# dremovd/PPO

Measured on AMD Instinct MI355X. Metric: env-steps/sec (Pong-shaped synthetic, 256 envs/GPU), higher is better.
Workload: dtype f32

## Files before the change

include/ppo_amd.h:

```cpp
#ifndef PPO_AMD_H
#define PPO_AMD_H

#include <stddef.h>
#include <stdint.h>

#ifdef __cplusplus
extern "C" {
#endif

#define PPO_OK 0
#define PPO_E_INVALID (-1)
#define PPO_E_HIP (-2)
#define PPO_E_ALIGN (-3)

#define PPO_TERM_NONE 0
#define PPO_TERM_U8 1
#define PPO_TERM_F32 2

#define PPO_SCAN_AUTO 0
#define PPO_SCAN_COLUMNS 1
#define PPO_SCAN_TILES 2

int ppo_version(void);
const char *ppo_last_error(void);
// ... 33 lines not shown
size_t ppo_conv3x3_packed_floats(int cin, int cout, int transposed);
int ppo_conv3x3_pack_weights_f32(const ppo_pack_job *jobs , int n_jobs, void *stream);
int ppo_conv3x3_forward_packed_f32(const void *in, int in_mode, const float *packed, const float *bias,
                                   const float *residual, float *out, int n, int cin, int cout, int h, int w,
                                   void *stream);
int ppo_conv3x3_backward_data_packed_f32(const float *dy, const float *packed, const float *relu_src,
                                         const float *dres, float *dx, int n, int cin, int cout, int h, int w,
                                         void *stream);
int ppo_conv3x3_pool_forward_packed_f32(const void *in, int in_mode, const float *packed, const float *bias,
                                        float *out, uint8_t *argmax, int n, int cin, int cout, int h, int w,
                                        void *stream);
int ppo_conv3x3_pool_forward_packed_indexed_f32(const void *in, const int32_t *index, int in_mode, const float *packed,
                                                const float *bias, float *out, uint8_t *argmax, int n, int cin, int cout,
                                                int h, int w, void *stream);
int ppo_conv3x3_backward_weight_slabs_pooled_indexed_f32(const void *in, const int32_t *index, int in_mode, const float *g,
                                                         const uint8_t *argmax, void *workspace, size_t workspace_bytes,
                                                         int n, int cin, int cout, int h, int w, int *n_slabs, void *stream);
int ppo_conv1_pool_form(int form);

int ppo_conv3x3_block_supported(int channels, int h, int w);
int ppo_conv3x3_block_forward_packed_f32(const float *in, const float *packed0, const float *bias0, const float *packed1,
                                         const float *bias1, float *out, int n, int channels, int h, int w, void *stream);

size_t ppo_conv3x3_wgrad_workspace_bytes(int cin, int cout);
int ppo_conv3x3_backward_weight_f32(const void *in, int in_mode, const float *dy, float *dweight, float *dbias,
                                    void *workspace, size_t workspace_bytes, int n, int cin, int cout, int h,
                                    int w, int accumulate, void *stream);

typedef struct ppo_wgrad_job {
    const float *slabs;
    float *dweight;
    float *dbias;
    int n_slabs, cin, cout;
    int accumulate;
} ppo_wgrad_job;
int ppo_conv3x3_backward_weight_slabs_f32(const void *in, int in_mode, const float *dy, void *workspace,
                                          size_t workspace_bytes, int n, int cin, int cout, int h, int w,
                                          int *n_slabs, void *stream);
int ppo_conv3x3_backward_weight_slabs_batch_f32(const void *const *ins, int in_mode, const float *const *dys,
                                                void *const *workspaces, size_t workspace_bytes, int count, int n, int cin,
                                                int cout, int h, int w, int *n_slabs, void *stream);
int ppo_conv3x3_backward_weight_slabs_batch_mixed_f32(const void *const *ins, const int *relu, const float *const *dys,
                                                      void *const *workspaces, size_t workspace_bytes, int count, int n,
                                                      int cin, int cout, int h, int w, int *n_slabs, void *stream);
int ppo_conv3x3_backward_weight_bf16x3_supported(int cin, int cout, int h, int w);
int ppo_conv3x3_backward_weight_slabs_batch_bf16x3(const float *const *ins, const int *relu, const float *const *dys,
                                                   void *const *workspaces, size_t workspace_bytes, int count, int n, int cin,
                                                   int cout, int h, int w, int *n_slabs, void *stream);
int ppo_conv3x3_backward_weight_pooled_supported(int cin, int cout, int h, int w);
int ppo_conv3x3_backward_weight_slabs_pooled_f32(const void *in, int in_mode, const float *g, const uint8_t *argmax,
                                                 void *workspace, size_t workspace_bytes, int n, int cin, int cout, int h,
                                                 int w, int *n_slabs, void *stream);
int ppo_conv3x3_wgrad_reduce_f32(const ppo_wgrad_job *jobs, int n_jobs, void *stream);

int ppo_maxpool3x3s2_forward_f32(const float *in, float *out, uint8_t *argmax, int n, int c, int h, int w,
                                 void *stream);
int ppo_maxpool3x3s2_backward_f32(const float *dout, const uint8_t *argmax, float *din, int n, int c, int h, int w,
                                  void *stream);

int ppo_conv2d_strided_supported(int cin, int cout, int kh, int kw, int stride, int h, int w);
int ppo_conv2d_strided_forward_f32(const void *in, int in_mode, const float *weight, const float *bias, float *out,
                                   int relu_out, int n, int cin, int h, int w, int cout, int kh, int kw, int stride,
                                   void *stream);
int ppo_conv2d_strided_backward_data_f32(const float *dy, const float *gate, const float *weight, float *dx, int n,
                                         int cin, int h, int w, int cout, int kh, int kw, int stride, void *stream);
size_t ppo_conv2d_strided_wgrad_workspace_bytes(int n, int cin, int h, int w, int cout, int kh, int kw, int stride);
int ppo_conv2d_strided_backward_weight_f32(const void *in, int in_mode, const float *dy, const float *gate, float *dweight,
                                           float *dbias, void *workspace, size_t workspace_bytes, int n, int cin, int h,
                                           int w, int cout, int kh, int kw, int stride, void *stream);

size_t ppo_gemm_workspace_bytes(int M, int N, int K);
int ppo_gemm_f32(const float *A, int64_t a_sm, int64_t a_sk, int relu_a, const float *B, int64_t b_sk, int64_t b_sn,
                 int relu_b, const float *bias, const float *mask, float *C, int64_t ldc, int M, int N, int K,
                 void *workspace, size_t workspace_bytes, void *stream);

int ppo_dense_heads_forward_f32(const float *x, int relu_x, const float *W, const float *b, const float *Wh, const float *bh,
                                int relu_h, float *h, float *heads, int M, int K, int H, int NH, void *workspace,
                                size_t workspace_bytes, void *stream);

int ppo_dense_heads_act_forward_f32(const float *x, int relu_x, const float *W, const float *b, const float *Wh,
                                    const float *bh, int relu_h, float *h, float *heads, int M, int K, int H, int NH,
                                    void *workspace, size_t workspace_bytes, int n_actions, float temperature,
                                    uint64_t seed, uint64_t offset, float *log_policy, int32_t *actions, float *log_pac,
                                    float *raw_policy, float *values, int n_value_heads, void *stream);
int ppo_dense_heads_loss_forward_f32(const float *x, int relu_x, const float *W, const float *b, const float *Wh, const float *bh,
                                     int relu_h, float *h, float *heads, int M, int K, int H, int NH, void *workspace,
                                     size_t workspace_bytes, int n_actions, int n_value_heads, const int32_t *actions,
                                     const float *old_log_pac, const float *old_log_policy, const float *advantages,
                                     const float *returns, float eps_clip, float ent_coef, float vf_coef, float grad_scale,
                                     float *dheads, float *stats, const int32_t *index, void *stream);

int ppo_heads_backward_f32(const float *dheads, const float *hin, int relu_in, const float *gate, const float *Wh, float *dh,
                           float *dWh, float *dbh, float *db_next, int B, int H, int NH, void *stream);
int ppo_colsum_f32(const float *X, int M, int N, int64_t ldx, float *out, int accumulate, void *stream);

int ppo_policy_act_f32(const float *heads, int B, int ldo, int n_actions, float temperature, const float *uniform,
                       uint64_t seed, uint64_t offset, int greedy, float *log_policy, int32_t *actions,
                       float *log_pac, float *raw_policy, float *values, int n_value_heads, void *stream);

int ppo_ppo_loss_f32(const float *heads, int B, int ldo, int n_actions, int n_value_heads, const int32_t *actions,
                     const float *old_log_pac, const float *old_log_policy, const float *advantages,
                     const float *returns, float eps_clip, float ent_coef, float vf_coef, float grad_scale,
                     float *dheads, float *stats, const int32_t *index, void *stream);

int ppo_tanh_forward_f32(const float *x, float *y, size_t n, void *stream);
int ppo_tanh_backward_f32(const float *dy, const float *y, float *dx, size_t n, void *stream);

int ppo_value_loss_f32(const float *heads, int B, int ldo, int value_col, int n_value_heads, const float *returns,
                       float vf_coef, int tvf_col, int n_tvf, int tvf_stride, const float *tvf_returns,
                       const float *tvf_weights, float tvf_coef, float grad_scale, float *dheads, float *stats,
                       const int32_t *index, float tvf_keep_prob, uint64_t seed, uint64_t offset, void *stream);

int ppo_distil_loss_f32(const float *heads, int B, int ldo, int n_actions, int pred_col, int n_pred, int pred_stride,
                        int vector_targets, const float *targets, const float *weights, const float *old_policy,
                        const float *log_std, float beta, float grad_scale, float *dheads, float *stats,
                        const int32_t *index, void *stream);

int ppo_gaussian_act_f32(const float *heads, int B, int ldo, int n_actions, const float *log_std, const float *normal,
                         uint64_t seed, uint64_t offset, int deterministic, float *actions, float *log_pac,
                         float *raw_policy, float *values, int n_value_heads, void *stream);

int ppo_gaussian_loss_f32(const float *heads, int B, int ldo, int n_actions, int n_value_heads, const float *actions,
                          const float *old_log_pac, const float *advantages, const float *returns,
                          const float *log_std, float eps_clip, float vf_coef, float grad_scale, float *dheads,
                          float *dlog_std_rows, float *stats, const int32_t *index, void *stream);

size_t ppo_adam_workspace_bytes(void);
// ... 161 lines not shown
```

ppo_amd/_lib.py:

```python
import ctypes
import os
import threading

HERE = os.path.dirname(os.path.abspath(__file__))
LIB_PATH = os.environ.get("PPO_AMD_LIB") or os.path.join(HERE, "lib", "libppo_amd.so")

PPO_TERM_NONE, PPO_TERM_U8, PPO_TERM_F32 = 0, 1, 2
PPO_SCAN_AUTO, PPO_SCAN_COLUMNS, PPO_SCAN_TILES = 0, 1, 2
PPO_IN_NONE, PPO_IN_RELU, PPO_IN_U8 = 0, 1, 2

_vp = ctypes.c_void_p
_i = ctypes.c_int
_i64 = ctypes.c_int64
_d = ctypes.c_double
_f = ctypes.c_float
_sz = ctypes.c_size_t
_u64 = ctypes.c_uint64

SIGNATURES = {
    "ppo_version": (_i, []),
    "ppo_last_error": (ctypes.c_char_p, []),
    "ppo_gae_scan_f32": (_i, [_vp, _vp, _vp, _vp, _i, _vp, _vp, _i, _i, _i64, _d, _d, _d, _i, _vp]),
    "ppo_bootstrapped_returns_f32": (_i, [_vp, _vp, _i, _vp, _vp, _d, _vp, _i, _i, _i64, _vp]),
    "ppo_conv3x3_forward_f32": (_i, [_vp, _i, _vp, _vp, _vp, _vp, _i, _i, _i, _i, _i, _vp]),
    "ppo_conv3x3_backward_data_f32": (_i, [_vp, _vp, _vp, _vp, _vp, _i, _i, _i, _i, _i, _vp]),
    "ppo_conv3x3_wgrad_workspace_bytes": (_sz, [_i, _i]),
    "ppo_conv3x3_backward_weight_f32": (_i, [_vp, _i, _vp, _vp, _vp, _vp, _sz, _i, _i, _i, _i, _i, _i, _vp]),
    "ppo_maxpool3x3s2_forward_f32": (_i, [_vp, _vp, _vp, _i, _i, _i, _i, _vp]),
    "ppo_maxpool3x3s2_backward_f32": (_i, [_vp, _vp, _vp, _i, _i, _i, _i, _vp]),
    "ppo_gemm_workspace_bytes": (_sz, [_i, _i, _i]),
    "ppo_gemm_f32": (_i, [_vp, _i64, _i64, _i, _vp, _i64, _i64, _i, _vp, _vp, _vp, _i64, _i, _i, _i, _vp, _sz, _vp]),
    "ppo_colsum_f32": (_i, [_vp, _i, _i, _i64, _vp, _i, _vp]),
    "ppo_heads_backward_f32": (_i, [_vp, _vp, _i, _vp, _vp, _vp, _vp, _vp, _vp, _i, _i, _i, _vp]),
    "ppo_dense_heads_forward_f32": (_i, [_vp, _i, _vp, _vp, _vp, _vp, _i, _vp, _vp, _i, _i, _i, _i, _vp, _sz, _vp]),
    "ppo_dense_heads_act_forward_f32": (_i, [_vp, _i, _vp, _vp, _vp, _vp, _i, _vp, _vp, _i, _i, _i, _i, _vp, _sz, _i, _f, _u64,
                                             _u64, _vp, _vp, _vp, _vp, _vp, _i, _vp]),
    "ppo_dense_heads_loss_forward_f32": (_i, [_vp, _i, _vp, _vp, _vp, _vp, _i, _vp, _vp, _i, _i, _i, _i, _vp, _sz, _i, _i, _vp, _vp, _vp,
                                              _vp, _vp, _f, _f, _f, _f, _vp, _vp, _vp, _vp]),
    "ppo_policy_act_f32": (_i, [_vp, _i, _i, _i, _f, _vp, _u64, _u64, _i, _vp, _vp, _vp, _vp, _vp, _i, _vp]),
    "ppo_gather_rows": (_i, [_vp, _i64, _i64, _vp, _i, _vp, _vp]),
    "ppo_moments_workspace_bytes": (_sz, []),
    "ppo_moments_f64": (_i, [_vp, _i64, _vp, _vp, _vp]),
    "ppo_normalize_f32": (_i, [_vp, _i64, _vp, _f, _vp, _vp, _vp]),
    "ppo_accumulate_f32": (_i, [_vp, _vp, _i64, _vp]),
    "ppo_mask_mul_f32": (_i, [_vp, _vp, _i64, _vp]),
    "ppo_tvf_returns_workspace_bytes": (_sz, [_i, _i, _i, _i, _i]),
    "ppo_tvf_returns_f32": (_i, [_vp, _vp, _vp, _i, _i, _i, _i, _i, _d, _vp, _vp, _vp, _i, _i, _vp, _vp, _vp, _vp, _vp,
                                 _vp, _sz, _vp, _vp]),
    "ppo_synth_env_create": (_vp, [_i, _i64, _u64, _d, _i64, _i]),
    "ppo_synth_env_destroy": (None, [_vp]),
    "ppo_synth_env_reset": (_i, [_vp, _vp]),
    "ppo_synth_env_step": (_i, [_vp, _vp, _vp, _vp, _vp, _vp, _vp, _vp]),
    "ppo_synth_env_step_upload": (_i, [_vp, _vp, _vp, _vp, _vp, _vp, _vp, _vp, _vp, _i, _vp]),
    "ppo_synth_env_get_state": (_i, [_vp, _vp, _vp, _vp]),
    "ppo_synth_env_set_state": (_i, [_vp, _vp, _vp, _vp, _vp]),
    "ppo_ppo_loss_f32": (_i, [_vp, _i, _i, _i, _i, _vp, _vp, _vp, _vp, _vp, _f, _f, _f, _f, _vp, _vp, _vp, _vp]),
    "ppo_conv3x3_pool_forward_f32": (_i, [_vp, _i, _vp, _vp, _vp, _vp, _i, _i, _i, _i, _i, _vp]),
    "ppo_conv3x3_packed_floats": (_sz, [_i, _i, _i]),
    "ppo_conv3x3_pack_weights_f32": (_i, [_vp, _i, _vp]),
    "ppo_conv3x3_forward_packed_f32": (_i, [_vp, _i, _vp, _vp, _vp, _vp, _i, _i, _i, _i, _i, _vp]),
    "ppo_conv3x3_backward_data_packed_f32": (_i, [_vp, _vp, _vp, _vp, _vp, _i, _i, _i, _i, _i, _vp]),
    "ppo_conv3x3_pool_forward_packed_f32": (_i, [_vp, _i, _vp, _vp, _vp, _vp, _i, _i, _i, _i, _i, _vp]),
    "ppo_conv3x3_pool_forward_packed_indexed_f32": (_i, [_vp, _vp, _i, _vp, _vp, _vp, _vp, _i, _i, _i, _i, _i, _vp]),
    "ppo_conv1_pool_form": (_i, [_i]),
    "ppo_conv3x3_block_supported": (_i, [_i, _i, _i]),
    "ppo_conv3x3_block_forward_packed_f32": (_i, [_vp, _vp, _vp, _vp, _vp, _vp, _i, _i, _i, _i, _vp]),
    "ppo_conv3x3_backward_weight_slabs_f32": (_i, [_vp, _i, _vp, _vp, _sz, _i, _i, _i, _i, _i, _vp, _vp]),
    "ppo_conv3x3_backward_weight_pooled_supported": (_i, [_i, _i, _i, _i]),
    "ppo_conv3x3_backward_weight_slabs_pooled_f32": (_i, [_vp, _i, _vp, _vp, _vp, _sz, _i, _i, _i, _i, _i, _vp, _vp]),
    "ppo_conv3x3_backward_weight_slabs_pooled_indexed_f32": (_i, [_vp, _vp, _i, _vp, _vp, _vp, _sz, _i, _i, _i, _i, _i, _vp, _vp]),
    "ppo_conv3x3_backward_weight_slabs_batch_f32": (_i, [_vp, _i, _vp, _vp, _sz, _i, _i, _i, _i, _i, _i, _vp, _vp]),
    "ppo_conv3x3_backward_weight_slabs_batch_mixed_f32": (_i, [_vp, _vp, _vp, _vp, _sz, _i, _i, _i, _i, _i, _i, _vp, _vp]),
    "ppo_conv3x3_backward_weight_bf16x3_supported": (_i, [_i, _i, _i, _i]),
    "ppo_conv3x3_backward_weight_slabs_batch_bf16x3": (_i, [_vp, _vp, _vp, _vp, _sz, _i, _i, _i, _i, _i, _i, _vp, _vp]),
    "ppo_conv3x3_wgrad_reduce_f32": (_i, [_vp, _i, _vp]),
    "ppo_tanh_forward_f32": (_i, [_vp, _vp, _sz, _vp]),
    "ppo_tanh_backward_f32": (_i, [_vp, _vp, _vp, _sz, _vp]),
    "ppo_value_loss_f32": (_i, [_vp, _i, _i, _i, _i, _vp, _f, _i, _i, _i, _vp, _vp, _f, _f, _vp, _vp, _vp, _f, _u64, _u64, _vp]),
    "ppo_distil_loss_f32": (_i, [_vp, _i, _i, _i, _i, _i, _i, _i, _vp, _vp, _vp, _vp, _f, _f, _vp, _vp, _vp, _vp]),
    "ppo_gaussian_act_f32": (_i, [_vp, _i, _i, _i, _vp, _vp, _u64, _u64, _i, _vp, _vp, _vp, _vp, _i, _vp]),
    "ppo_gaussian_loss_f32": (_i, [_vp, _i, _i, _i, _i, _vp, _vp, _vp, _vp, _vp, _f, _f, _f, _vp, _vp, _vp, _vp, _vp]),
    "ppo_impala_stack_tail_supported": (_i, [_i, _i, _i]),
    "ppo_impala_stack_tail_forward_f32": (_i, [_vp, _vp, _vp, _vp, _vp, _vp, _vp, _i, _i, _i, _i, _vp]),
    "ppo_impala_stack_full_supported": (_i, [_i, _i, _i]),
    "ppo_impala_stack_full_backward_f32": (_i, [_vp] * 10 + [_i, _i, _i, _i, _vp]),
    "ppo_impala_stack_chain_forward_f32": (_i, [_vp] * 15 + [_i, _i, _i, _i, _vp]),
    "ppo_impala_stack_chain_split_workspace_bytes": (_sz, [_i, _i, _i, _i]),
    "ppo_impala_stack_chain_split_forward_f32": (_i, [_vp, _vp, _vp, _vp, _vp, _vp, _vp, _sz, _i, _i, _i, _i, _vp]),
    "ppo_impala_stack_full_forward_f32": (_i, [_vp, _vp, _vp, _vp, _vp, _vp, _vp, _vp, _vp, _i, _i, _i, _i, _vp]),
    "ppo_impala_stack_tail_backward_f32": (_i, [_vp, _vp, _vp, _vp, _vp, _vp, _vp, _i, _i, _i, _i, _vp]),
    "ppo_obs_moments_f64": (_i, [_vp, _i, _i, _i, _vp, _vp]),
    "ppo_obs_rms_update_f64": (_i, [_vp, _d, _d, _vp, _vp, _vp, _vp, _i, _vp]),
    "ppo_obs_normalize_f32": (_i, [_vp, _i, _vp, _vp, _f, _vp, _i, _i, _vp]),
    "ppo_adam_workspace_bytes": (_sz, []),
    "ppo_adam_step_f32": (_i, [_vp, _vp, _vp, _vp, _i64, _i64, _d, _d, _d, _d, _f, _f, _vp, _vp, _vp]),
    "ppo_adam_step_presummed_f32": (_i, [_vp, _vp, _vp, _vp, _i64, _i64, _d, _d, _d, _d, _f, _f, _vp, _i, _vp, _vp]),
    "ppo_impala_stack_tail_bf16x3_packed_bytes": (_sz, []),
    "ppo_impala_stack_tail_bf16x3_supported": (_i, [_i, _i, _i]),
    "ppo_impala_stack_tail_pack_bf16x3": (_i, [_vp, _vp, _i, _i, _vp]),
    "ppo_impala_stack_tail_pack_bf16x3_jobs": (_i, [_vp, _i, _vp]),
    "ppo_impala_stack_tail_forward_bf16x3": (_i, [_vp, _vp, _vp, _vp, _vp, _vp, _vp, _i, _i, _i, _i, _vp]),
    "ppo_impala_stack_tail_backward_bf16x3": (_i, [_vp, _vp, _vp, _vp, _vp, _vp, _vp, _i, _i, _i, _i, _vp]),
    "ppo_impala_stack_tail_bf16x3_sign_bytes": (_sz, [_i, _i, _i, _i]),
    "ppo_impala_stack_tail_forward_signs_bf16x3": (_i, [_vp, _vp, _vp, _vp, _vp, _vp, _vp, _vp, _i, _i, _i, _i, _vp]),
    "ppo_impala_stack_tail_backward_signs_bf16x3": (_i, [_vp, _vp, _vp, _vp, _vp, _vp, _vp, _i, _i, _i, _i, _vp]),
    "ppo_conv3x3_bf16x3_supported": (_i, [_i, _i, _i, _i]),
    "ppo_conv3x3_bf16x3_packed_bytes": (_sz, [_i, _i]),
    "ppo_conv3x3_pack_bf16x3_jobs": (_i, [_vp, _i, _vp]),
    "ppo_conv3x3_bf16x3": (_i, [_vp, _i, _vp, _vp, _vp, _i, _i, _i, _i, _i, _vp]),
    "ppo_conv3x3_pool_bf16x3_supported": (_i, [_i, _i, _i, _i]),
    "ppo_conv3x3_backward_weight_slabs_batch_bf16_split": (_i, [_vp, _vp, _vp, _vp, _sz, _i, _i, _i, _i, _i, _i, _i, _vp, _vp]),
    "ppo_conv3x3_bf16_split_packed_bytes": (_sz, [_i, _i, _i]),
    "ppo_conv3x3_pack_bf16_split": (_i, [_vp, _vp, _i, _i, _i, _i, _vp]),
    "ppo_conv3x3_bf16_split": (_i, [_vp, _i, _vp, _vp, _vp, _i, _i, _i, _i, _i, _i, _vp]),
    "ppo_conv3x3_pool_bf16x3": (_i, [_vp, _i, _vp, _vp, _vp, _vp, _i, _i, _i, _i, _i, _vp]),
    "ppo_mlp_supported": (_i, [_i, _i, _i]),
    "ppo_mlp_forward_f32": (_i, [_vp, _vp, _vp, _i, _vp, _vp, _vp, _vp]),
    "ppo_mlp_train_workspace_floats": (_sz, [_i, _i, _i, _i]),
    "ppo_mlp_train_f32": (_i, [_vp, _vp, _vp, _vp, _i64, _i, _vp, _vp, _vp, _vp, _i, _i, _vp, _vp, _vp]),
    "ppo_conv2d_strided_supported": (_i, [_i, _i, _i, _i, _i, _i, _i]),
    "ppo_conv2d_strided_forward_f32": (_i, [_vp, _i, _vp, _vp, _vp, _i, _i, _i, _i, _i, _i, _i, _i, _i, _vp]),
    "ppo_conv2d_strided_backward_data_f32": (_i, [_vp, _vp, _vp, _vp, _i, _i, _i, _i, _i, _i, _i, _i, _vp]),
    "ppo_conv2d_strided_wgrad_workspace_bytes": (_sz, [_i, _i, _i, _i, _i, _i, _i, _i]),
    "ppo_conv2d_strided_backward_weight_f32": (_i, [_vp, _i, _vp, _vp, _vp, _vp, _vp, _sz, _i, _i, _i, _i, _i, _i, _i, _i, _vp]),
    "ppo_adam_step_scatter_f32": (_i, [_vp, _vp, _vp, _vp, _i64, _i64, _d, _d, _d, _d, _f, _f, _vp, _vp, _vp, _i64, _vp, _vp]),
}

class PackJob(ctypes.Structure):
# ... 99 lines not shown
```

ppo_amd/csrc/conv3x3_wgrad.hip:

```cpp
#include "common.h"
#include "conv_stage.h"
#include "mfma.h"

namespace ppo {
namespace {

constexpr int pad_mod32(int v, int target) { return v + ((target - v % 32) + 32) % 32; }

#ifndef PPO_STAMP
#define PPO_STAMP(var)
#define PPO_STAMP_ADD(slot, t1, t0)
#endif
#ifndef PPO_TUNE_WGRAD_NBUF
#define PPO_TUNE_WGRAD_NBUF 2
#endif
#ifndef PPO_TUNE_WGRAD_PERCU
#define PPO_TUNE_WGRAD_PERCU 2
#endif
#ifndef PPO_TUNE_WGRAD_NBUF_ONEBAND
#define PPO_TUNE_WGRAD_NBUF_ONEBAND 1
#endif
template <int IN_MODE, int NBANDS>
constexpr int wgrad_nbuf()
{
    return IN_MODE == IN_U8 ? 1 : (NBANDS == 1 ? PPO_TUNE_WGRAD_NBUF_ONEBAND : PPO_TUNE_WGRAD_NBUF);
}
template <int IN_MODE, bool DY_POOLED>
constexpr bool wgrad_run() { return true; }
constexpr int kWgradWaves = 8;
#ifndef PPO_TUNE_WGRAD_DMA_WAVE
#define PPO_TUNE_WGRAD_DMA_WAVE 4
#endif
template <int IN_MODE, int NBANDS, bool DY_POOLED>
constexpr bool wgrad_dma_wave()
{
    return PPO_TUNE_WGRAD_DMA_WAVE && wgrad_nbuf<IN_MODE, NBANDS>() == 2 && IN_MODE != IN_U8 && !DY_POOLED;
}
constexpr int kWgradDmaWaves = PPO_TUNE_WGRAD_DMA_WAVE;
template <int IN_MODE, int NBANDS, bool DY_POOLED>
constexpr int wgrad_threads() { return (kWgradWaves + (wgrad_dma_wave<IN_MODE, NBANDS, DY_POOLED>() ? kWgradDmaWaves : 0)) * 64; }

template <int CIN, int COUT, int H, int W, int TR, int NBUF_, bool RUN_>
struct WgradCfg {
    static constexpr int CINP = (CIN + 3) / 4 * 4;
    static constexpr int MTC = COUT / 16;
    static constexpr bool BIAS_IN_TILE = (9 * CINP) % 16 != 0;
    static constexpr int NJ = 9 * CINP + (BIAS_IN_TILE ? 1 : 0);
    static constexpr int NTT = (NJ + 15) / 16;
    static constexpr int JP = ((9 * CINP + 1) + 15) / 16 * 16;
    static constexpr int WT = (NTT <= 4 || NTT == 9) ? 1 : ((NTT <= 12 || NTT == 18) ? 2 : 4);
    static constexpr int KG = kWgradWaves / WT;
    static constexpr int NTW_MAX = (NTT + WT - 1) / WT;
    static constexpr int REM = NTT % WT == 0 ? WT : NTT % WT;
    static constexpr int WIDTH = W;
// ... 265 lines not shown
    for (int src = 1; src < C::KG; ++src) {
        float *img = s_red;
        if (kg == src) {
            if (db_lane) {
#pragma unroll
                for (int m = 0; m < C::MTC; ++m) img[(m * 16 + l15) * C::JP + 9 * C::CINP] = asum[m];
            }
#pragma unroll
            for (int m = 0; m < C::MTC; ++m)
#pragma unroll
                for (int t = 0; t < C::NTW_MAX; ++t)
                    if (wt + C::WT * t < C::NTT)
#pragma unroll
                        for (int r = 0; r < 4; ++r)
                            img[(m * 16 + g * 4 + r) * C::JP + (wt + C::WT * t) * 16 + l15] = acc[m][t][r];
        }
        __syncthreads();
        if (kg == 0) {
#pragma unroll
            for (int m = 0; m < C::MTC; ++m)
#pragma unroll
                for (int t = 0; t < C::NTW_MAX; ++t)
                    if (wt + C::WT * t < C::NTT)
#pragma unroll
                        for (int r = 0; r < 4; ++r)
                            acc[m][t][r] += img[(m * 16 + g * 4 + r) * C::JP + (wt + C::WT * t) * 16 + l15];
            if (db_lane) {
#pragma unroll
                for (int m = 0; m < C::MTC; ++m) asum[m] += img[(m * 16 + l15) * C::JP + 9 * C::CINP];
            }
        }
        if (src + 1 < C::KG) __syncthreads();
    }
    if (kg == 0) {
        float *slab = partial + (size_t)blockIdx.x * COUT * C::JP;
#pragma unroll
        for (int m = 0; m < C::MTC; ++m)
#pragma unroll
            for (int t = 0; t < C::NTW_MAX; ++t)
                if (wt + C::WT * t < C::NTT)
#pragma unroll
                    for (int r = 0; r < 4; ++r)
                        slab[(m * 16 + g * 4 + r) * C::JP + (wt + C::WT * t) * 16 + l15] = acc[m][t][r];
        if (db_lane) {
#pragma unroll
            for (int m = 0; m < C::MTC; ++m) slab[(m * 16 + l15) * C::JP + 9 * C::CINP] = asum[m];
        }
    }
    PPO_STAMP(t_k3)
    PPO_STAMP_ADD(7, t_k3, t_k2)
    PPO_STAMP_ADD(3, t_k3, t_k0)
}

__device__ __forceinline__ float4 slab_partition_sum(const float *slabs, int byte_off, int byte_stride, int lo, int hi, bool live)
{
    const __amdgpu_buffer_rsrc_t buf = buffer_of(slabs);
    float4 s0 = make_float4(0.f, 0.f, 0.f, 0.f), s1 = s0;
    for (int q = lo; q < hi; q += 16) {
        float4 v[16];
#pragma unroll
        for (int u = 0; u < 16; ++u) v[u] = buffer_f32x4(buf, (live && q + u < hi) ? byte_off + (q + u) * byte_stride : kOutside);
#pragma unroll
        for (int u = 0; u < 16; u += 2) {
            s0.x += v[u].x; s0.y += v[u].y; s0.z += v[u].z; s0.w += v[u].w;
            s1.x += v[u + 1].x; s1.y += v[u + 1].y; s1.z += v[u + 1].z; s1.w += v[u + 1].w;
        }
    }
    return make_float4(s0.x + s1.x, s0.y + s1.y, s0.z + s1.z, s0.w + s1.w);
}

__global__ __launch_bounds__(256) void conv3x3_wgrad_reduce_kernel(const float *__restrict__ partial, int n_slabs,
                                                                   int cout, int cin, int cinp, int jp,
                                                                   float *__restrict__ dw, float *__restrict__ db,
                                                                   int accumulate)
{
    __shared__ float4 s[256];
    const int q4 = jp / 4;
    const int idx = blockIdx.x * 16 + (threadIdx.x & 15);
    const int part = threadIdx.x >> 4;
    const bool live = idx < cout * q4;
    const int co = live ? idx / q4 : 0;
    const int j0 = live ? (idx % q4) * 4 : 0;
    const size_t stride = (size_t)cout * jp;
    const int per = (n_slabs + 15) / 16;
    const int lo = part * per;
    const int hi = lo + per < n_slabs ? lo + per : n_slabs;
    s[threadIdx.x] = slab_partition_sum(partial, (co * jp + j0) * 4, (int)stride * 4, lo, hi, live);
    __syncthreads();
    if (part == 0 && live) {
        float sum[4] = {0.f, 0.f, 0.f, 0.f};
#pragma unroll
        for (int q = 0; q < 16; ++q) {
            const float4 a = s[q * 16 + threadIdx.x];
            sum[0] += a.x;
            sum[1] += a.y;
            sum[2] += a.z;
            sum[3] += a.w;
        }
#pragma unroll
        for (int e = 0; e < 4; ++e) {
            const int j = j0 + e;
            if (j == 9 * cinp) {
                if (db) db[co] = accumulate ? db[co] + sum[e] : sum[e];
            } else if (j < 9 * cinp) {
                const int tap = j / cinp;
                const int ci = j % cinp;
                if (ci < cin) {
                    float *dst = dw + ((size_t)co * cin + ci) * 9 + tap;
                    *dst = accumulate ? *dst + sum[e] : sum[e];
                }
            }
        }
    }
}

#ifndef PPO_TUNE_WGRAD_MAXSLABS
#define PPO_TUNE_WGRAD_MAXSLABS 512
#endif
constexpr int kWgradMaxSlabs = PPO_TUNE_WGRAD_MAXSLABS;

constexpr int kMaxJobs = 32;
struct ReduceJobs {
    ppo_wgrad_job j[kMaxJobs];
};

__global__ __launch_bounds__(256) void conv3x3_wgrad_reduce_jobs_kernel(ReduceJobs jobs)
{
    __shared__ float4 s[256];
    const ppo_wgrad_job &job = jobs.j[blockIdx.y];
    const int cout = job.cout, cin = job.cin, n_slabs = job.n_slabs, accumulate = job.accumulate;
    const int cinp = (cin + 3) / 4 * 4;
    const int jp = ((9 * cinp + 1) + 15) / 16 * 16;
    const int q4 = jp / 4;
    if ((int)blockIdx.x * 16 >= cout * q4) return;
    const int idx = blockIdx.x * 16 + (threadIdx.x & 15);
    const int part = threadIdx.x >> 4;
    const bool live = idx < cout * q4;
    const int co = live ? idx / q4 : 0;
    const int j0 = live ? (idx % q4) * 4 : 0;
    const size_t stride = (size_t)cout * jp;
    const int per = (n_slabs + 15) / 16;
    const int lo = part * per;
    const int hi = lo + per < n_slabs ? lo + per : n_slabs;
    s[threadIdx.x] = slab_partition_sum(job.slabs, (co * jp + j0) * 4, (int)stride * 4, lo, hi, live);
    __syncthreads();
    if (part == 0 && live) {
        float sum[4] = {0.f, 0.f, 0.f, 0.f};
#pragma unroll
        for (int q = 0; q < 16; ++q) {
            const float4 a = s[q * 16 + threadIdx.x];
            sum[0] += a.x;
            sum[1] += a.y;
            sum[2] += a.z;
            sum[3] += a.w;
        }
#pragma unroll
        for (int e = 0; e < 4; ++e) {
            const int j = j0 + e;
            if (j == 9 * cinp) {
                if (job.dbias) job.dbias[co] = accumulate ? job.dbias[co] + sum[e] : sum[e];
            } else if (j < 9 * cinp) {
                const int tap = j / cinp;
                const int ci = j % cinp;
                if (ci < cin) {
                    float *d = job.dweight + ((size_t)co * cin + ci) * 9 + tap;
                    *d = accumulate ? *d + sum[e] : sum[e];
                }
            }
        }
    }
}

template <int CIN, int COUT, int H, int W, int TR, int IN_MODE, bool DY_POOLED = false>
int launch_wgrad(const void *in, const float *dy, float *dw, float *db, float *workspace, size_t workspace_bytes,
                 int n_images, int accumulate, hipStream_t st, int *n_slabs_out = nullptr,
                 const WgradBatch *more = nullptr, int count = 1, const uint8_t *argmax = nullptr)
{
    using C = WgradCfg<CIN, COUT, H, W, TR, wgrad_nbuf<IN_MODE, (H + TR - 1) / TR>(), wgrad_run<IN_MODE, DY_POOLED>()>;
    auto kern = conv3x3_wgrad_kernel<CIN, COUT, H, W, TR, IN_MODE, DY_POOLED>;
    static bool attr_set = false;
    if (!attr_set) {
        hipError_t e = hipFuncSetAttribute(reinterpret_cast<const void *>(kern),
                                           hipFuncAttributeMaxDynamicSharedMemorySize, (int)C::LDS_BYTES);
        if (e != hipSuccess) return fail(PPO_E_HIP, "conv3x3_wgrad: hipFuncSetAttribute: %s", hipGetErrorString(e));
        attr_set = true;
    }
    const int n_items = n_images * C::NBANDS;
    int per_cu = (int)((160 * 1024) / C::LDS_BYTES);
    per_cu = per_cu < 1 ? 1 : (per_cu > PPO_TUNE_WGRAD_PERCU ? PPO_TUNE_WGRAD_PERCU : per_cu);
#ifndef PPO_TUNE_WGRAD_BIGSLABS
    if ((size_t)COUT * C::JP * sizeof(float) > 16 * 1024) per_cu = 1;
#endif
    int grid = (256 * per_cu) / count;
    if (grid < 1) grid = 1;
    if (grid > kWgradMaxSlabs) grid = kWgradMaxSlabs;
    if (grid > n_items) grid = n_items;
    const size_t need = (size_t)grid * COUT * C::JP * sizeof(float);
    if (need > workspace_bytes)
        return fail(PPO_E_INVALID, "conv3x3_wgrad: workspace too small (%zu < %zu bytes)", workspace_bytes, need);
    WgradBatch batch{};
    if (more) {
        batch = *more;
    } else {
        batch.in[0] = in;
        batch.dy[0] = dy;
        batch.partial[0] = workspace;
    }
    batch.argmax = argmax;
    batch.in_index = IN_MODE == IN_U8 ? t_wgrad_in_index : nullptr;
    hipLaunchKernelGGL(kern, dim3(grid, count), dim3(wgrad_threads<IN_MODE, C::NBANDS, DY_POOLED>()), C::LDS_BYTES, st, batch,
                       n_images);
    int rc = check_launch("conv3x3_wgrad_kernel");
    if (rc) return rc;
    if (n_slabs_out) {
        *n_slabs_out = grid;
        return PPO_OK;
    }
    const int total = COUT * (C::JP / 4);
    hipLaunchKernelGGL(conv3x3_wgrad_reduce_kernel, dim3((total + 15) / 16), dim3(256), 0, st, workspace, grid, COUT,
                       CIN, C::CINP, C::JP, dw, db, accumulate);
    return check_launch("conv3x3_wgrad_reduce_kernel");
}

// ... 201 lines not shown
```

ppo_amd/csrc/gemm.hip:

```cpp
#include <algorithm>

#include "common.h"
#include "loss_rows.h"
#include "policy_act.h"
#include "mfma.h"

namespace ppo {
namespace {

#ifndef PPO_TUNE_GEMM_BK
#define PPO_TUNE_GEMM_BK 32
#endif
constexpr int BM = 64, BN = 64, BK = PPO_TUNE_GEMM_BK;
constexpr int PITCH_M = 80, PITCH_K = BK + 2;
constexpr int TILE_WORDS = BM * PITCH_K > BK * PITCH_M ? BM * PITCH_K : BK * PITCH_M;

struct GemmArgs {
    const float *A;
    const float *B;
    float *C;
    const float *bias;
    const float *mask;
    int M, N, K;
    int64_t a_sm, a_sk, b_sk, b_sn, ldc;
    int relu_a, relu_b;
    int k_per_slice;
    int split;
    int vec_a, vec_b;
    int vec_c;
};

#ifndef PPO_TUNE_GEMM_WAVES
#define PPO_TUNE_GEMM_WAVES 8
#endif
constexpr int kGemmWaves = PPO_TUNE_GEMM_WAVES, kGemmThreads = kGemmWaves * 64;
static_assert(kGemmWaves == 4 || kGemmWaves == 8, "2 x 2 waves of 32 x 32 or 2 x 4 waves of 32 x 16");
constexpr int kWaveN = kGemmWaves == 8 ? 16 : 32, kNJ = kWaveN / 16;
constexpr int kSlabF4 = BM * BK / 4 / kGemmThreads;
struct Slab {
    float4 v[kSlabF4];
};

__device__ __forceinline__ __amdgpu_buffer_rsrc_t operand_rsrc(const float *P) { return buffer_of(P); }

template <bool kfast, bool vec>
__device__ __forceinline__ void slab_load(Slab &s, __amdgpu_buffer_rsrc_t P, int st, int sk, int t0, int rows, int k0,
                                          int kend, int tid)
{
#pragma unroll
    for (int e = 0; e < kSlabF4; ++e) {
        const int q = tid + e * kGemmThreads;
        int tt, kk;
        if (kfast) {
            kk = (q % (BK / 4)) * 4;
            tt = q / (BK / 4);
// ... 46 lines not shown
};
__device__ __forceinline__ TileId tile_of(int id, int gm, int gn, int split)
{
    const int xcd = id % kXcds, slot = id / kXcds;
    TileId t;
    if (split > 1) {
        const int per = (split + kXcds - 1) / kXcds;
        t.z = xcd * per + slot % per;
        const int tile = slot / per;
        t.tn = tile % gn;
        t.tm = tile / gn;
        t.live = t.z < split && t.tm < gm;
    } else if (gn >= gm) {
        t.z = 0;
        t.tm = slot % gm;
        t.tn = xcd + kXcds * (slot / gm);
        t.live = t.tn < gn;
    } else {
        t.z = 0;
        t.tn = slot % gn;
        t.tm = xcd + kXcds * (slot / gn);
        t.live = t.tm < gm;
    }
    return t;
}
inline int tile_grid(int gm, int gn, int split)
{
    if (split > 1) return kXcds * ((split + kXcds - 1) / kXcds) * gm * gn;
    const int lo = gn >= gm ? gm : gn, hi = gn >= gm ? gn : gm;
    return kXcds * ((hi + kXcds - 1) / kXcds) * lo;
}

#ifndef PPO_TUNE_GEMM_DEPTH
#define PPO_TUNE_GEMM_DEPTH 4
#endif
constexpr int DEPTH = PPO_TUNE_GEMM_DEPTH;

#ifdef PPO_TUNE_GEMM_STAMPS
__device__ unsigned long long ppo_gemm_stamps[1024 * 8];
#define PPO_GSTAMP(slot)                                                                          \
    do {                                                                                          \
        unsigned long long t_;                                                                    \
        __builtin_amdgcn_sched_barrier(0);                                                        \
        asm volatile("s_memtime %0\n\ts_waitcnt lgkmcnt(0)" : "=s"(t_)::"memory");               \
        __builtin_amdgcn_sched_barrier(0);                                                        \
        if (threadIdx.x == 0 && blockIdx.x < 1024) ppo_gemm_stamps[blockIdx.x * 8 + (slot)] = t_; \
    } while (0)
#else
#define PPO_GSTAMP(slot)
#endif
static_assert(DEPTH % 2 == 0, "the LDS buffer of a slab is its slot's parity");

template <bool a_kfast, bool b_kfast, bool vec>
__global__ __launch_bounds__(kGemmThreads) void gemm_f32_kernel(GemmArgs p, int gm, int gn)
{
    __shared__ __align__(16) float s_a[2][TILE_WORDS];
    __shared__ __align__(16) float s_b[2][TILE_WORDS];
    const TileId t = tile_of(blockIdx.x, gm, gn, p.split);
    if (!t.live) return;
    const int tid = threadIdx.x;
    const int lane = tid & 63;
    const int wave = tid >> 6;
    const int l15 = lane & 15;
    const int g = lane >> 4;
    const int wm = (wave / (BN / kWaveN)) * 32;
    const int wn = (wave % (BN / kWaveN)) * kWaveN;
    const int m0 = t.tm * BM;
    const int n0 = t.tn * BN;
    const int kbeg = t.z * p.k_per_slice;
    const int kend = min(p.K, kbeg + p.k_per_slice);

    f32x4 acc[2][kNJ];
#pragma unroll
    for (int i = 0; i < 2; ++i)
#pragma unroll
        for (int j = 0; j < kNJ; ++j) acc[i][j] = f32x4{0.f, 0.f, 0.f, 0.f};

    const int nslabs = kbeg < kend ? (kend - kbeg + BK - 1) / BK : 0;
    const int ngroups = (nslabs + DEPTH - 1) / DEPTH;
    const __amdgpu_buffer_rsrc_t bufA = operand_rsrc(p.A), bufB = operand_rsrc(p.B);
    Slab ra[DEPTH], rb[DEPTH];

    auto fetch = [&](int d, int slab) {
        slab_load<a_kfast, vec>(ra[d], bufA, (int)p.a_sm, (int)p.a_sk, m0, p.M, kbeg + slab * BK, kend, tid);
        slab_load<b_kfast, vec>(rb[d], bufB, (int)p.b_sn, (int)p.b_sk, n0, p.N, kbeg + slab * BK, kend, tid);
    };
    auto stage = [&](int d) {
        slab_store(ra[d], s_a[d & 1], a_kfast, p.relu_a, tid);
        slab_store(rb[d], s_b[d & 1], b_kfast, p.relu_b, tid);
        __syncthreads();
    };
    auto multiply = [&](int d) {
        const float *sa = s_a[d & 1], *sb = s_b[d & 1];
        float a[BK / 4][2], b[BK / 4][kNJ];
#pragma unroll
        for (int ks = 0; ks < BK / 4; ++ks) {
#pragma unroll
            for (int i = 0; i < 2; ++i)
                a[ks][i] = a_kfast ? sa[(wm + i * 16 + l15) * PITCH_K + ks * 4 + g]
                                   : sa[(ks * 4 + g) * PITCH_M + wm + i * 16 + l15];
#pragma unroll
            for (int j = 0; j < kNJ; ++j)
                b[ks][j] = b_kfast ? sb[(wn + j * 16 + l15) * PITCH_K + ks * 4 + g]
                                   : sb[(ks * 4 + g) * PITCH_M + wn + j * 16 + l15];
        }
        __builtin_amdgcn_sched_barrier(0);
#pragma unroll
        for (int ks = 0; ks < BK / 4; ++ks)
#pragma unroll
            for (int i = 0; i < 2; ++i)
#pragma unroll
// ... 40 lines not shown
            for (int q = 0; q < kPasses; ++q) {
                const int m = m0 + row0 + kRowsPerPass * q;
                const int off = (m < p.M && col_in) ? (m * (int)p.ldc + n0 + col) * 4 : kOutside;
                gate[q] = buffer_f32x4(bufM, off);
            }
        }
        if (finish && p.bias && col_in) bias4 = *reinterpret_cast<const float4 *>(p.bias + n0 + col);
        __syncthreads();
#pragma unroll
        for (int i = 0; i < 2; ++i)
#pragma unroll
            for (int j = 0; j < kNJ; ++j)
#pragma unroll
                for (int r = 0; r < 4; ++r)
                    sc[(wm + i * 16 + g * 4 + r) * PITCH_C + wn + j * 16 + l15] = acc[i][j][r];
        __syncthreads();
#pragma unroll
        for (int q = 0; q < kPasses; ++q) {
            const int row = row0 + kRowsPerPass * q, m = m0 + row;
            float4 v = *reinterpret_cast<const float4 *>(sc + row * PITCH_C + col);
            if (finish) {
                v.x += bias4.x, v.y += bias4.y, v.z += bias4.z, v.w += bias4.w;
                if (p.mask) {
                    v.x = gate[q].x > 0.f ? v.x : 0.f;
                    v.y = gate[q].y > 0.f ? v.y : 0.f;
                    v.z = gate[q].z > 0.f ? v.z : 0.f;
                    v.w = gate[q].w > 0.f ? v.w : 0.f;
                }
            }
            if (m < p.M && col_in) *reinterpret_cast<float4 *>(C + m * ldc + n0 + col) = v;
        }
    } else {
#pragma unroll
        for (int i = 0; i < 2; ++i)
#pragma unroll
            for (int j = 0; j < kNJ; ++j)
#pragma unroll
                for (int r = 0; r < 4; ++r) {
                    const int m = m0 + wm + i * 16 + g * 4 + r;
                    const int n = n0 + wn + j * 16 + l15;
                    if (m < p.M && n < p.N) {
                        float v = acc[i][j][r];
                        if (finish) {
                            if (p.bias) v += p.bias[n];
                            if (p.mask) v = p.mask[m * p.ldc + n] > 0.f ? v : 0.f;
                        }
                        C[m * ldc + n] = v;
                    }
                }
    }
    PPO_GSTAMP(4);
}

__global__ __launch_bounds__(256) void gemm_finalize_kernel(const float *__restrict__ partial, int split, int M, int N,
                                                            const float *__restrict__ bias,
                                                            const float *__restrict__ mask, float *__restrict__ C,
                                                            int64_t ldc)
{
    const int idx = blockIdx.x * blockDim.x + threadIdx.x;
    if (idx >= M * N) return;
    const int m = idx / N, n = idx % N;
    float v = 0.f;
    const size_t stride = (size_t)M * N;
    int s = 0;
    for (; s + 8 <= split; s += 8) {
        float t[8];
#pragma unroll
        for (int u = 0; u < 8; ++u) t[u] = partial[(size_t)(s + u) * stride + idx];
#pragma unroll
        for (int u = 0; u < 8; ++u) v += t[u];
    }
    for (; s < split; ++s) v += partial[(size_t)s * stride + idx];
    if (bias) v += bias[n];
    if (mask) v = mask[m * ldc + n] > 0.f ? v : 0.f;
    C[m * ldc + n] = v;
}

constexpr int kRowsMaxN = 32, kRowsMaxKPerLane = 8;

template <int NB, int KPL>
__global__ __launch_bounds__(256) void gemm_rows_kernel(GemmArgs p)
{
    const int lane = threadIdx.x & 63;
    const int m = blockIdx.x * 4 + __builtin_amdgcn_readfirstlane(threadIdx.x >> 6);
    if (m >= p.M) return;
    const __amdgpu_buffer_rsrc_t bufA = operand_rsrc(p.A), bufB = operand_rsrc(p.B);
    bool kin[KPL];
#pragma unroll
    for (int i = 0; i < KPL; ++i) kin[i] = lane + 64 * i < p.K;
    float av[KPL];
#pragma unroll
    for (int i = 0; i < KPL; ++i) {
        const int off = kin[i] ? (m * (int)p.a_sm + lane + 64 * i) * 4 : kOutside;
        av[i] = buffer_f32(bufA, off);
    }
    for (int n0 = 0; n0 < p.N; n0 += NB) {
        float bv[NB][KPL];
#pragma unroll
        for (int j = 0; j < NB; ++j) {
            const int row = min(n0 + j, p.N - 1) * (int)p.b_sn;
#pragma unroll
            for (int i = 0; i < KPL; ++i) {
                const int off = kin[i] ? (row + lane + 64 * i) * 4 : kOutside;
                bv[j][i] = buffer_f32(bufB, off);
            }
        }
// ... 25 lines not shown
}

__global__ __launch_bounds__(256) void gemm_small_kernel(GemmArgs p)
{
    __shared__ float s[256];
    const int o = blockIdx.x * 16 + (threadIdx.x & 15);
    const int part = threadIdx.x >> 4;
    const bool live = o < p.M * p.N;
    const int m = live ? o / p.N : 0, n = live ? o - m * p.N : 0;
    const float *a = p.A + m * p.a_sm;
    const float *b = p.B + n * p.b_sn;
    const int per = (p.K + 15) / 16;
    const int k0 = part * per, k1 = min(p.K, k0 + per);
    float acc = 0.f;
    if (live) {
        int k = k0;
        for (; k + 8 <= k1; k += 8) {
            float av[8], bv[8];
#pragma unroll
            for (int u = 0; u < 8; ++u) {
                av[u] = a[(k + u) * p.a_sk];
                bv[u] = b[(k + u) * p.b_sk];
            }
#pragma unroll
            for (int u = 0; u < 8; ++u) {
                if (p.relu_a) av[u] = fmaxf(av[u], 0.f);
                if (p.relu_b) bv[u] = fmaxf(bv[u], 0.f);
                acc = fmaf(av[u], bv[u], acc);
            }
        }
        for (; k < k1; ++k) {
            float a0 = a[k * p.a_sk], b0 = b[k * p.b_sk];
            if (p.relu_a) a0 = fmaxf(a0, 0.f);
            if (p.relu_b) b0 = fmaxf(b0, 0.f);
            acc = fmaf(a0, b0, acc);
        }
    }
    s[threadIdx.x] = acc;
    __syncthreads();
    if (part == 0 && live) {
        float v = 0.f;
#pragma unroll
        for (int q = 0; q < 16; ++q) v += s[q * 16 + threadIdx.x];
        if (p.bias) v += p.bias[n];
        if (p.mask) v = p.mask[m * p.ldc + n] > 0.f ? v : 0.f;
        p.C[m * p.ldc + n] = v;
    }
}

__global__ __launch_bounds__(256) void colsum_kernel(const float *__restrict__ X, int M, int N, int64_t ldx,
                                                     float *__restrict__ out, int accumulate)
{
    __shared__ float s[256];
    const int n = blockIdx.x * 16 + (threadIdx.x & 15);
    const int part = threadIdx.x >> 4;
    float v = 0.f;
    if (n < N) {
        for (int m = part; m < M; m += 16 * 8) {
            float t[8];
#pragma unroll
            for (int u = 0; u < 8; ++u) {
                const int mm = m + 16 * u;
                t[u] = mm < M ? X[mm * ldx + n] : 0.f;
            }
#pragma unroll
            for (int u = 0; u < 8; ++u) v += t[u];
        }
    }
    s[threadIdx.x] = v;
    __syncthreads();
    if (part == 0 && n < N) {
        float t = 0.f;
#pragma unroll
        for (int q = 0; q < 16; ++q) t += s[q * 16 + threadIdx.x];
        out[n] = accumulate ? out[n] + t : t;
    }
}

struct ActTail {
    float temperature;
    uint64_t seed, offset;
    ActOut out;
    int loss;
    PpoLossP lp;
    float *dheads;
    const int32_t *index;
};

template <int KPL, int NA, int NHT>
__global__ __launch_bounds__(256) void finalize_heads_kernel(const float *__restrict__ partial, int split, int M, int H,
                                                            const float *__restrict__ bias, float *__restrict__ h,
                                                            const float *__restrict__ Wh, const float *__restrict__ bh, int NH,
                                                            int relu_h, float *__restrict__ heads, ActTail act)
{
    const int lane = threadIdx.x & 63;
    const int m = blockIdx.x * 4 + __builtin_amdgcn_readfirstlane(threadIdx.x >> 6);
    if (m >= M) return;
    const __amdgpu_buffer_rsrc_t pb = buffer_of(partial), wb = buffer_of(Wh), bb = buffer_of(bias, bias != nullptr);
    const int stride = M * H;
    int off[KPL];
#pragma unroll
    for (int i = 0; i < KPL; ++i) off[i] = lane + 64 * i < H ? m * H + lane + 64 * i : -1;
    float bv[NHT][KPL];
#pragma unroll
    for (int j = 0; j < NHT; ++j) {
        const int row = min(j, NH - 1) * H;
#pragma unroll
        for (int i = 0; i < KPL; ++i) bv[j][i] = buffer_f32(wb, off[i] < 0 ? kOutside : (row + lane + 64 * i) * 4);
    }
    float hv[KPL];
#pragma unroll
    for (int i = 0; i < KPL; ++i) hv[i] = 0.f;
    float bsv[KPL];
#pragma unroll
    for (int i = 0; i < KPL; ++i) bsv[i] = buffer_f32(bb, off[i] < 0 ? kOutside : (lane + 64 * i) * 4);
    int s = 0;
    for (; s + 16 <= split; s += 16) {
        float t[KPL][16];
#pragma unroll
        for (int i = 0; i < KPL; ++i)
#pragma unroll
            for (int u = 0; u < 16; ++u) t[i][u] = buffer_f32(pb, off[i] < 0 ? kOutside : ((s + u) * stride + off[i]) * 4);
#pragma unroll
        for (int i = 0; i < KPL; ++i)
#pragma unroll
            for (int u = 0; u < 16; ++u) hv[i] += t[i][u];
    }
    for (; s + 8 <= split; s += 8) {
        float t[KPL][8];
// ... 124 lines not shown
    }
#pragma unroll
    for (int j = 0; j < 16; ++j) s_red[j][tid] = dW[j];
    s_red[16][tid] = dbn;
    s_red[17][tid] = dbj;
    __syncthreads();
    if (part == 0) {
        float tot[18];
#pragma unroll
        for (int v = 0; v < 18; ++v) {
            float t = 0.f;
#pragma unroll
            for (int q = 0; q < 16; ++q) t += s_red[v][q * 16 + kk];
            tot[v] = t;
        }
        if (col) {
#pragma unroll
            for (int j = 0; j < 16; ++j)
                if (j < a.NH) a.dWh[j * a.H + k] = tot[j];
            if (a.db_next) a.db_next[k] = tot[16];
        }
        if ((int)blockIdx.x == a.xb && a.dbh && kk < a.NH) a.dbh[kk] = tot[17];
    }
}

inline bool vec_ok(const float *P, int64_t s_tile, int64_t s_k, int tile_extent, int k_extent)
{
    const int64_t other = s_k == 1 ? s_tile : s_k;
    const int extent = s_k == 1 ? k_extent : tile_extent;
    return (s_k == 1 || s_tile == 1) && other % 4 == 0 && extent % 4 == 0 && aligned(P, 16);
}

}
}

extern "C" size_t ppo_gemm_workspace_bytes(int M, int N, int K)
{
    (void)K;
    return (size_t)32 * M * N * sizeof(float);
}

namespace ppo {
namespace {
struct HeadsTail {
    const float *Wh, *bh;
    float *heads;
    int NH, relu_h;
    bool fused;
    const ActTail *act = nullptr;
    int act_n = 0;
    bool act_fused = false;
};

int gemm_dispatch(const float *A, int64_t a_sm, int64_t a_sk, int relu_a, const float *B, int64_t b_sk, int64_t b_sn,
                  int relu_b, const float *bias, const float *mask, float *C, int64_t ldc, int M, int N, int K,
                  void *workspace, size_t workspace_bytes, void *stream, HeadsTail *tail)
{
    if (M < 0 || N < 0 || K < 0) return fail(PPO_E_INVALID, "ppo_gemm_f32: negative dimension");
    if (M == 0 || N == 0) return PPO_OK;
    if (!A || !B || !C) return fail(PPO_E_INVALID, "ppo_gemm_f32: null pointer");
    if (ldc < N) return fail(PPO_E_INVALID, "ppo_gemm_f32: ldc < N");
    const int64_t a_last = (int64_t)(M - 1) * a_sm + (int64_t)(K - 1) * a_sk, b_last = (int64_t)(N - 1) * b_sn + (int64_t)(K - 1) * b_sk;
    if (K > 0 && (a_last * 4 + 16 > (int64_t)kBufferBytes || b_last * 4 + 16 > (int64_t)kBufferBytes || a_sm < 0 || a_sk < 0 ||
                  b_sn < 0 || b_sk < 0))
        return fail(PPO_E_INVALID, "ppo_gemm_f32: operand spans 2 GiB or more (or a negative stride); split the batch");
    hipStream_t st = as_stream(stream);
    if ((N <= 16 || K <= 16 || (M <= 16 && a_sm == 1)) && (int64_t)M * N <= (1 << 22)) {
        GemmArgs q{A, B, C, bias, mask, M, N, K, a_sm, a_sk, b_sk, b_sn, ldc, relu_a, relu_b, K, 1, 0, 0, 0};
        if (N <= kRowsMaxN && a_sk == 1 && b_sk == 1 && K <= 64 * kRowsMaxKPerLane) {
            if (K <= 256 && N <= 16)
                hipLaunchKernelGGL((gemm_rows_kernel<16, 4>), dim3((M + 3) / 4), dim3(256), 0, st, q);
            else if (K <= 256)
                hipLaunchKernelGGL((gemm_rows_kernel<8, 4>), dim3((M + 3) / 4), dim3(256), 0, st, q);
            else
                hipLaunchKernelGGL((gemm_rows_kernel<4, kRowsMaxKPerLane>), dim3((M + 3) / 4), dim3(256), 0, st, q);
            return check_launch("gemm_rows_kernel");
        }
        hipLaunchKernelGGL(gemm_small_kernel, dim3((M * N + 15) / 16), dim3(256), 0, st, q);
        return check_launch("gemm_small_kernel");
    }
    const int gm = (M + BM - 1) / BM, gn = (N + BN - 1) / BN;
    constexpr int kSliceK = 256;
    int split = 1;
    const bool few = gn * 4 <= 32;
    if (few && K >= 2 * kSliceK) split = std::min(32, (K + kSliceK - 1) / kSliceK);
    if (split > 1 && (!workspace || workspace_bytes < (size_t)split * M * N * sizeof(float))) split = 1;
    int kps = (K + split - 1) / split;
    kps = (kps + BK - 1) / BK * BK;
    if (split > 1) split = (K + kps - 1) / kps;
    GemmArgs p{A, B, split > 1 ? static_cast<float *>(workspace) : C, bias, mask, M, N, K, a_sm, a_sk, b_sk, b_sn,
               ldc, relu_a, relu_b, kps, split, vec_ok(A, a_sm, a_sk, M, K) ? 1 : 0, vec_ok(B, b_sn, b_sk, N, K) ? 1 : 0, 0};
    p.vec_c = N % 4 == 0 && ldc % 4 == 0 && aligned(C, 16) && aligned(p.C, 16) && (!bias || aligned(bias, 16)) &&
              (!mask || (aligned(mask, 16) && (int64_t)M * ldc * 4 < (int64_t)kBufferBytes));
    const dim3 grid(tile_grid(gm, gn, split));
    const bool vec = p.vec_a && p.vec_b;
    const int variant = (a_sk == 1 ? 4 : 0) | (b_sk == 1 ? 2 : 0) | (vec ? 1 : 0);
#define PPO_GEMM_CASE(v, ak, bk, vc)                                                                  \
    case v:                                                                                           \
        hipLaunchKernelGGL((gemm_f32_kernel<ak, bk, vc>), grid, dim3(kGemmThreads), 0, st, p, gm, gn); \
        break;
    switch (variant) {
        PPO_GEMM_CASE(0, false, false, false)
        PPO_GEMM_CASE(1, false, false, true)
        PPO_GEMM_CASE(2, false, true, false)
        PPO_GEMM_CASE(3, false, true, true)
        PPO_GEMM_CASE(4, true, false, false)
        PPO_GEMM_CASE(5, true, false, true)
        PPO_GEMM_CASE(6, true, true, false)
        PPO_GEMM_CASE(7, true, true, true)
    }
#undef PPO_GEMM_CASE
    int rc = check_launch("gemm_f32_kernel");
    if (rc) return rc;
    if (split > 1) {
        if (tail && !mask && ldc == N && N <= 256 && tail->NH <= 32 && (int64_t)split * M * N * 4 < (int64_t)kBufferBytes) {
#define PPO_FINALIZE(NA, NHT, ACT)                                                                                     \
    hipLaunchKernelGGL((finalize_heads_kernel<4, NA, NHT>), dim3((M + 3) / 4), dim3(256), 0, st,                       \
                       static_cast<const float *>(workspace), split, M, N, bias, C, tail->Wh, tail->bh, tail->NH,      \
                       tail->relu_h, tail->heads, ACT)
            tail->act_fused = tail->act != nullptr;
            const bool wide = tail->NH > 16;
#define PPO_FIN2(NA, ACT)                       \
    do {                                        \
        if (wide) PPO_FINALIZE(NA, 32, ACT);    \
        else PPO_FINALIZE(NA, 16, ACT);         \
    } while (0)
            switch (tail->act ? tail->act_n : 0) {
                case 4: PPO_FIN2(4, *tail->act); break;
                case 6: PPO_FIN2(6, *tail->act); break;
                case 15: PPO_FIN2(15, *tail->act); break;
                case 18: PPO_FIN2(18, *tail->act); break;
                default: PPO_FIN2(0, ActTail{}); tail->act_fused = false;
            }
#undef PPO_FIN2
#undef PPO_FINALIZE
            tail->fused = true;
            return check_launch("finalize_heads_kernel");
        }
        hipLaunchKernelGGL(gemm_finalize_kernel, dim3((M * N + 255) / 256), dim3(256), 0, st,
                           static_cast<const float *>(workspace), split, M, N, bias, mask, C, ldc);
        rc = check_launch("gemm_finalize_kernel");
    }
    return rc;
}
}
}

extern "C" int ppo_gemm_f32(const float *A, int64_t a_sm, int64_t a_sk, int relu_a, const float *B, int64_t b_sk,
                            int64_t b_sn, int relu_b, const float *bias, const float *mask, float *C, int64_t ldc,
                            int M, int N, int K, void *workspace, size_t workspace_bytes, void *stream)
{
    return ppo::gemm_dispatch(A, a_sm, a_sk, relu_a, B, b_sk, b_sn, relu_b, bias, mask, C, ldc, M, N, K, workspace,
                              workspace_bytes, stream, nullptr);
}

extern "C" int ppo_dense_heads_forward_f32(const float *x, int relu_x, const float *W, const float *b, const float *Wh,
                                           const float *bh, int relu_h, float *h, float *heads, int M, int K, int H, int NH,
                                           void *workspace, size_t workspace_bytes, void *stream)
{
    using namespace ppo;
    if (M < 0 || K < 0 || H <= 0 || NH <= 0) return fail(PPO_E_INVALID, "ppo_dense_heads_forward_f32: bad dimension");
    if (M == 0) return PPO_OK;
    if (!x || !W || !Wh || !h || !heads) return fail(PPO_E_INVALID, "ppo_dense_heads_forward_f32: null pointer");
    HeadsTail tail{Wh, bh, heads, NH, relu_h, false};
    int rc = gemm_dispatch(x, K, 1, relu_x, W, 1, K, 0, b, nullptr, h, H, M, H, K, workspace, workspace_bytes, stream, &tail);
    if (rc || tail.fused) return rc;
    return gemm_dispatch(h, H, 1, relu_h, Wh, 1, H, 0, bh, nullptr, heads, NH, M, NH, H, nullptr, 0, stream, nullptr);
}

extern "C" int ppo_policy_act_f32(const float *heads, int B, int ldo, int n_actions, float temperature, const float *uniform,
                                  uint64_t seed, uint64_t offset, int greedy, float *log_policy, int32_t *actions,
                                  float *log_pac, float *raw_policy, float *values, int n_value_heads, void *stream);

extern "C" int ppo_dense_heads_act_forward_f32(const float *x, int relu_x, const float *W, const float *b, const float *Wh,
                                               const float *bh, int relu_h, float *h, float *heads, int M, int K, int H,
                                               int NH, void *workspace, size_t workspace_bytes, int n_actions,
                                               float temperature, uint64_t seed, uint64_t offset, float *log_policy,
                                               int32_t *actions, float *log_pac, float *raw_policy, float *values,
                                               int n_value_heads, void *stream)
{
    using namespace ppo;
    if (M < 0 || K < 0 || H <= 0 || NH <= 0) return fail(PPO_E_INVALID, "ppo_dense_heads_act_forward_f32: bad dimension");
    if (n_actions <= 0 || n_actions > kMaxActions || n_value_heads < 0 || NH < n_actions + n_value_heads)
        return fail(PPO_E_INVALID, "ppo_dense_heads_act_forward_f32: bad head layout (n_actions=%d value heads=%d of %d)",
                    n_actions, n_value_heads, NH);
    if (!(temperature > 0.f)) return fail(PPO_E_INVALID, "ppo_dense_heads_act_forward_f32: temperature must be > 0");
    if (M == 0) return PPO_OK;
    if (!x || !W || !Wh || !h || !heads) return fail(PPO_E_INVALID, "ppo_dense_heads_act_forward_f32: null pointer");
    const ActTail act{temperature, seed, offset, ActOut{log_policy, actions, log_pac, raw_policy, values, n_value_heads}, 0,
                      PpoLossP{}, nullptr, nullptr};
    HeadsTail tail{Wh, bh, heads, NH, relu_h, false};
    tail.act = &act;
    tail.act_n = n_actions;
    int rc = gemm_dispatch(x, K, 1, relu_x, W, 1, K, 0, b, nullptr, h, H, M, H, K, workspace, workspace_bytes, stream, &tail);
    if (rc) return rc;
    if (!tail.fused)
        rc = gemm_dispatch(h, H, 1, relu_h, Wh, 1, H, 0, bh, nullptr, heads, NH, M, NH, H, nullptr, 0, stream, nullptr);
    if (rc || tail.act_fused) return rc;
    return ppo_policy_act_f32(heads, M, NH, n_actions, temperature, nullptr, seed, offset, 0, log_policy, actions, log_pac,
                              raw_policy, values, n_value_heads, stream);
}

extern "C" int ppo_ppo_loss_f32(const float *heads, int B, int ldo, int n_actions, int n_value_heads, const int32_t *actions,
                                const float *old_log_pac, const float *old_log_policy, const float *advantages,
                                const float *returns, float eps_clip, float ent_coef, float vf_coef, float grad_scale,
                                float *dheads, float *stats, const int32_t *index, void *stream);
// ... 54 lines not shown
```

ppo_amd/csrc/optim.hip:

```cpp
#include "common.h"

namespace ppo {
namespace {

constexpr int kPartials = 256;
__device__ __forceinline__ bool aligned16(const void *p) { return (reinterpret_cast<uintptr_t>(p) & 15) == 0; }

__global__ __launch_bounds__(256) void grad_sumsq_kernel(const float *__restrict__ g, int64_t n, float *__restrict__ partials)
{
    __shared__ float s[256];
    const int64_t chunk = (n + gridDim.x - 1) / gridDim.x;
    const int64_t lo = (int64_t)blockIdx.x * chunk;
    const int64_t hi = lo + chunk < n ? lo + chunk : n;
    float acc = 0.f;
    int64_t i = lo + threadIdx.x;
    for (; i + 768 < hi; i += 1024) {
        const float x0 = g[i], x1 = g[i + 256], x2 = g[i + 512], x3 = g[i + 768];
        acc += x0 * x0;
        acc += x1 * x1;
        acc += x2 * x2;
        acc += x3 * x3;
    }
    for (; i < hi; i += 256) {
        const float x = g[i];
        acc += x * x;
    }
    s[threadIdx.x] = acc;
    __syncthreads();
    for (int w = 128; w > 0; w >>= 1) {
        if (threadIdx.x < w) s[threadIdx.x] += s[threadIdx.x + w];
        __syncthreads();
    }
    if (threadIdx.x == 0) partials[blockIdx.x] = s[0];
}

__global__ __launch_bounds__(256) void adam_kernel(float *__restrict__ w, const float *__restrict__ g,
                                                   float *__restrict__ m, float *__restrict__ v, int64_t n,
                                                   const float *__restrict__ partials, int n_partials, float lr,
                                                   float one_minus_beta1, float beta2, float one_minus_beta2,
                                                   float eps, float bias_c1,
                                                   float bias_c2_sqrt, float max_norm, float grad_div,
                                                   float *__restrict__ norm_out, const int32_t *__restrict__ scatter,
                                                   int64_t n_scatter, float *__restrict__ packed)
{
    __shared__ float s_clip;
    __shared__ float s_part[256];
    s_part[threadIdx.x] = (int)threadIdx.x < n_partials ? partials[threadIdx.x] : 0.f;
    __syncthreads();
    for (int w = 128; w > 0; w >>= 1) {
        if ((int)threadIdx.x < w) s_part[threadIdx.x] += s_part[threadIdx.x + w];
        __syncthreads();
    }
    if (threadIdx.x == 0) {
        const float tot = s_part[0];
        const float norm = sqrtf(tot) / grad_div;
        float clip = 1.f;
        if (max_norm > 0.f) {
            clip = max_norm / (norm + 1e-6f);
            clip = clip > 1.f ? 1.f : clip;
        }
        s_clip = clip / grad_div;
        if (norm_out && blockIdx.x == 0) *norm_out = norm;
    }
    __syncthreads();
    const float gscale = s_clip;
    const float step_size = lr / bias_c1;
    auto update = [&](float &wi, float gi, float &mi, float &vi) {
        gi *= gscale;
        mi = mi + (gi - mi) * one_minus_beta1;
        vi = vi * beta2 + one_minus_beta2 * gi * gi;
        const float denom = sqrtf(vi) / bias_c2_sqrt + eps;
        wi = wi - step_size * (mi / denom);
    };
    const bool vec = (n % 4 == 0) && aligned16(w) && aligned16(g) && aligned16(m) && aligned16(v);
    if (vec) {
        const int64_t n4 = n / 4;
        float4 *w4 = reinterpret_cast<float4 *>(w), *m4 = reinterpret_cast<float4 *>(m), *v4 = reinterpret_cast<float4 *>(v);
        const float4 *g4 = reinterpret_cast<const float4 *>(g);
        for (int64_t i = (int64_t)blockIdx.x * blockDim.x + threadIdx.x; i < n4; i += (int64_t)gridDim.x * blockDim.x) {
            float4 ww = w4[i], gg = g4[i], mm = m4[i], vv = v4[i];
            update(ww.x, gg.x, mm.x, vv.x);
            update(ww.y, gg.y, mm.y, vv.y);
            update(ww.z, gg.z, mm.z, vv.z);
            update(ww.w, gg.w, mm.w, vv.w);
            w4[i] = ww;
            m4[i] = mm;
// ... 38 lines not shown

extern "C" int ppo_adam_step_f32(float *params, const float *grads, float *exp_avg, float *exp_avg_sq, int64_t n,
                                 int64_t step, double lr, double beta1, double beta2, double eps, float max_grad_norm,
                                 float grad_div, void *workspace, float *grad_norm_out, void *stream)
{
    return adam_step(params, grads, exp_avg, exp_avg_sq, n, step, lr, beta1, beta2, eps, max_grad_norm, grad_div, workspace,
                     grad_norm_out, nullptr, 0, nullptr, stream);
}

extern "C" int ppo_adam_step_scatter_f32(float *params, const float *grads, float *exp_avg, float *exp_avg_sq, int64_t n,
                                         int64_t step, double lr, double beta1, double beta2, double eps,
                                         float max_grad_norm, float grad_div, void *workspace, float *grad_norm_out,
                                         const int32_t *scatter, int64_t n_scatter, float *packed, void *stream)
{
    if (n_scatter < 0 || n_scatter > n || (n_scatter > 0 && (!scatter || !packed)))
        return ppo::fail(PPO_E_INVALID, "ppo_adam_step_scatter_f32: bad scatter table");
    return adam_step(params, grads, exp_avg, exp_avg_sq, n, step, lr, beta1, beta2, eps, max_grad_norm, grad_div, workspace,
                     grad_norm_out, scatter, n_scatter, packed, stream);
}

extern "C" int ppo_adam_step_presummed_f32(float *params, const float *grads, float *exp_avg, float *exp_avg_sq, int64_t n,
                                           int64_t step, double lr, double beta1, double beta2, double eps,
                                           float max_grad_norm, float grad_div, const float *partials, int n_partials,
                                           float *grad_norm_out, void *stream)
{
    using namespace ppo;
    if (n < 0 || step < 1) return fail(PPO_E_INVALID, "ppo_adam_step_presummed_f32: n < 0 or step < 1");
    if (n == 0) return PPO_OK;
    if (!params || !grads || !exp_avg || !exp_avg_sq || !partials || n_partials < 1 || n_partials > kPartials)
        return fail(PPO_E_INVALID, "ppo_adam_step_presummed_f32: null pointer or partial count outside [1, %d]", kPartials);
    if (!(grad_div > 0.f)) return fail(PPO_E_INVALID, "ppo_adam_step_presummed_f32: grad_div must be > 0");
    const double bc1 = 1.0 - pow(beta1, (double)step);
    const double bc2 = 1.0 - pow(beta2, (double)step);
    int grid = (int)((n + 255) / 256);
    grid = grid > 1024 ? 1024 : grid;
    hipLaunchKernelGGL(adam_kernel, dim3(grid), dim3(256), 0, as_stream(stream), params, grads, exp_avg, exp_avg_sq, n, partials,
                       n_partials, (float)lr, (float)(1.0 - beta1), (float)beta2, (float)(1.0 - beta2), (float)eps, (float)bc1,
                       (float)sqrt(bc2), max_grad_norm, grad_div, grad_norm_out, nullptr, (int64_t)0, nullptr);
    return check_launch("adam_kernel");
}

static int adam_step(float *params, const float *grads, float *exp_avg, float *exp_avg_sq, int64_t n, int64_t step, double lr,
                     double beta1, double beta2, double eps, float max_grad_norm, float grad_div, void *workspace,
                     float *grad_norm_out, const int32_t *scatter, int64_t n_scatter, float *packed, void *stream)
{
    using namespace ppo;
    if (n < 0 || step < 1) return fail(PPO_E_INVALID, "ppo_adam_step_f32: n < 0 or step < 1");
    if (n == 0) return PPO_OK;
    if (!params || !grads || !exp_avg || !exp_avg_sq || !workspace)
        return fail(PPO_E_INVALID, "ppo_adam_step_f32: null pointer");
    if (!(grad_div > 0.f)) return fail(PPO_E_INVALID, "ppo_adam_step_f32: grad_div must be > 0");
    hipStream_t st = as_stream(stream);
    float *partials = static_cast<float *>(workspace);
    int np = (int)((n + 4095) / 4096);
    np = np > kPartials ? kPartials : np;
    hipLaunchKernelGGL(grad_sumsq_kernel, dim3(np), dim3(256), 0, st, grads, n, partials);
    int rc = check_launch("grad_sumsq_kernel");
    if (rc) return rc;
    const double bc1 = 1.0 - pow(beta1, (double)step);
    const double bc2 = 1.0 - pow(beta2, (double)step);
    int grid = (int)((n + 255) / 256);
    grid = grid > 1024 ? 1024 : grid;
    hipLaunchKernelGGL(adam_kernel, dim3(grid), dim3(256), 0, st, params, grads, exp_avg, exp_avg_sq, n, partials, np,
                       (float)lr, (float)(1.0 - beta1), (float)beta2, (float)(1.0 - beta2), (float)eps, (float)bc1,
                       (float)sqrt(bc2), max_grad_norm, grad_div, grad_norm_out, scatter, n_scatter, packed);
    return check_launch("adam_kernel");
}
```

ppo_amd/models.py:

```python
import ctypes
import math
import os
from collections import OrderedDict
from typing import Dict, Optional

import numpy as np
import torch

from . import _lib

IN_NONE, IN_RELU, IN_U8 = _lib.PPO_IN_NONE, _lib.PPO_IN_RELU, _lib.PPO_IN_U8
_ALIGN = 4
FUSE_POOL_STACKS = int(os.environ.get("PPO_AMD_FUSE_POOL", "7"))
WGRAD_SIDE_STREAM = int(os.environ.get("PPO_AMD_WGRAD_STREAM", "0"))
WGRAD_BATCH_REDUCE = int(os.environ.get("PPO_AMD_WGRAD_BATCH_REDUCE", "1"))
WGRAD_BATCH_LAUNCH = int(os.environ.get("PPO_AMD_WGRAD_BATCH_LAUNCH", "1"))
WGRAD_POOLED_DY = int(os.environ.get("PPO_AMD_WGRAD_POOLED_DY", "1"))
WGRAD_RIDE = int(os.environ.get("PPO_AMD_WGRAD_RIDE", "1"))
SPLIT_WGRAD = int(os.environ.get("PPO_AMD_SPLIT_WGRAD", "1"))
SPLIT_CONV = int(os.environ.get("PPO_AMD_SPLIT_CONV", "1"))
SPLIT_CONV_POOL = int(os.environ.get("PPO_AMD_SPLIT_CONV_POOL", "1"))
SPLIT_SIGNS = int(os.environ.get("PPO_AMD_SPLIT_SIGNS", "1"))
PACKED_WEIGHTS = int(os.environ.get("PPO_AMD_PACKED_WEIGHTS", "1"))
ADAM_SCATTER = int(os.environ.get("PPO_AMD_ADAM_SCATTER", "0"))
# ... 249 lines not shown
                 activation_fn: str = "relu", tvf_fixed_head_horizons=None, tvf_feature_sparsity: float = 0.0,
                 tvf_feature_window: int = -1, head_scale: float = 1.0, value_head_names=("ext",),
                 head_bias: bool = False, device="cuda", precision: str = "high", **encoder_args):
        encoder = encoder.lower()
        if precision not in ("low", "medium", "high"):
            raise ValueError(f"Invalid precision mode {precision}")
        if encoder not in ("impala", "mlp", "nature"):
            raise NotImplementedError(f"encoder '{encoder}' has no HIP path (impala | nature | mlp)")
        if activation_fn not in ("relu", "tanh"):
            raise ValueError(f"Invalid activation function {activation_fn}")
        _lib.require_gpu()
        self.lib = _lib.load()
        self.device = torch.device(device)
        if self.device.type != "cuda":
            raise _lib.PpoAmdError(f"device '{device}': the HIP path runs on the GPU only")
        if self.device.index is None:
            self.device = torch.device("cuda", torch.cuda.current_device())
        if encoder == "impala":
            self.spec = ImpalaSpec(input_dims, hidden_units=hidden_units, **encoder_args)
        elif encoder == "nature":
            self.spec = NatureSpec(input_dims, hidden_units=hidden_units, **encoder_args)
            for _name, cin, cout, k, s, h, w, _ho, _wo in self.spec.layers:
                if not self.lib.ppo_conv2d_strided_supported(cin, cout, k, k, s, h, w):
                    raise _lib.PpoAmdError(f"no strided-convolution kernel for {cin}->{cout} {k}x{k}/{s} on {h}x{w}")
        else:
            self.spec = MLPSpec(input_dims, hidden_units=hidden_units, **encoder_args)
        self.encoder_kind = encoder
        self.encoder_activation_fn = activation_fn
        self.n_actions = n_actions
        self.hidden_units = hidden_units
        self.value_head_names = list(value_head_names)
        self.vh = len(self.value_head_names)
        self.head_bias = head_bias
        self.tvf_fixed_head_horizons = None if tvf_fixed_head_horizons is None else list(tvf_fixed_head_horizons)
        self.K = 0 if tvf_fixed_head_horizons is None else len(tvf_fixed_head_horizons)
        self.col_policy, self.col_value = 0, n_actions
        self.col_advantage = n_actions + self.vh
        self.col_tvf = 2 * n_actions + self.vh
        self.nh = self.col_tvf + self.K * self.vh
        self._build_parameters(head_scale)
        self.tvf_feature_sparsity, self.tvf_feature_window = tvf_feature_sparsity, tvf_feature_window
        self.tvf_features_mask = None
        self._build_tvf_feature_mask()
        self._bufs: Dict[tuple, torch.Tensor] = {}
        self._rec = None
        self.act_tail = None
        self._chain_split_usable = None
        self.allow_chain_split = False
        self.obs_index = None
        self.loss_tail = None
        self._tail_ptrs = {}
        self.obs_norm = None
        self.grad_ready_hook = None
        self._split_ws = {}
        self._plans = {}
        self.use_plans = True
        self._build_packed_weights()
        self._build_split_bf16(precision)
        self._build_mlp_fused()
        self._adam_step = 0
        self.exp_avg = None
        self.exp_avg_sq = None

    @property
    def use_tvf(self):
        return self.K > 0

    def _build_parameters(self, head_scale):
        sp = self.spec
        init = init_parameters(sp, self.n_actions, self.vh, head_scale, self.head_bias, self.K)
        head_names = [n for n in HEAD_NAMES if f"{n}.weight" in init]
        order = [(n, t) for n, t in init.items() if n.startswith("encoder.")]
        order += [(f"{n}.weight", init[f"{n}.weight"]) for n in head_names]
        if self.head_bias:
            order += [(f"{n}.bias", init[f"{n}.bias"]) for n in head_names]
        order += [("log_std", init["log_std"])]

        offs, total = OrderedDict(), 0
        for name, t in order:
            offs[name] = (total, tuple(t.shape))
            n = t.numel()
            contiguous_group = name.endswith("_head.weight") or name.endswith("_head.bias")
            total += n if contiguous_group else (n + _ALIGN - 1) // _ALIGN * _ALIGN
        total = (total + _ALIGN - 1) // _ALIGN * _ALIGN
        self.n_params_padded = total
        flat = torch.zeros(total, dtype=torch.float32)
        for name, t in order:
            o, shape = offs[name]
            flat[o:o + t.numel()] = t.reshape(-1)
        self.flat = flat.to(self.device)
        self.grad = torch.zeros_like(self.flat)
        self._offsets = offs
        self._state_order = list(init.keys())
        self.params = OrderedDict((name, self.flat[o:o + int(np.prod(shape))].view(shape)) for name, (o, shape) in offs.items())
        self.grads = OrderedDict((name, self.grad[o:o + int(np.prod(shape))].view(shape)) for name, (o, shape) in offs.items())
        o = offs["policy_head.weight"][0]
        self.w_heads = self.flat[o:o + self.nh * sp.hidden_units].view(self.nh, sp.hidden_units)
        self.g_w_heads = self.grad[o:o + self.nh * sp.hidden_units].view(self.nh, sp.hidden_units)
        if self.head_bias:
            o = offs["policy_head.bias"][0]
            self.b_heads = self.flat[o:o + self.nh]
            self.g_b_heads = self.grad[o:o + self.nh]
        else:
            self.b_heads = self.g_b_heads = None

    def _build_split_bf16(self, precision):
        self.precision = precision
        self.split_bf16, self._pk16, self._split_jobs, self._split_conv_jobs = False, {}, None, None
        if precision == "high" or self.encoder_kind != "impala" or self.spec.n_block != 2:
            return
        jobs = []
        nbytes = int(self.lib.ppo_impala_stack_tail_bf16x3_packed_bytes())
        for si, (_cin, cout, _h, _w, ho, wo) in enumerate(self.spec.stacks):
            if not self.lib.ppo_impala_stack_tail_bf16x3_supported(cout, ho, wo):
                continue
            for tr, order in ((0, ((0, 0), (0, 1), (1, 0), (1, 1))), (1, ((1, 1), (1, 0), (0, 1), (0, 0)))):
                buf = torch.zeros(nbytes, dtype=torch.uint8, device=self.device)
                self._pk16[(si, tr)] = buf
                ws = [self.params[f"encoder.stacks.{si}.blocks.{bi}.conv{ci}.weight"].data_ptr() for bi, ci in order]
                jobs.append(_lib.SplitPackJob((ctypes.c_void_p * 4)(*ws), buf.data_ptr(), cout, tr))
            names = [f"encoder.stacks.{si}.blocks.{bi}.conv{ci}" for bi in range(2) for ci in range(2)]
            self._pk16[(si, "bias")] = (ctypes.c_void_p * 4)(*[self.params[n + ".bias"].data_ptr() for n in names])
        if jobs:
            self._split_jobs = (_lib.SplitPackJob * len(jobs))(*jobs)
            self.split_bf16 = True
            self._packed_dirty = True
        cjobs = []
        self._split_conv_jobs = None
        for si, (cin, cout, h, w, _ho, _wo) in enumerate(self.spec.stacks):
            if not (self.split_bf16 and SPLIT_CONV and si > 0 and cin in (16, 32) and cout in (16, 32)):
                continue
            wname = f"encoder.stacks.{si}.firstconv"
            nb = int(self.lib.ppo_conv3x3_bf16x3_packed_bytes(cin, cout))
            for tr, (ci_op, co_op) in ((0, (cin, cout)), (1, (cout, cin))):
                if not self.lib.ppo_conv3x3_bf16x3_supported(ci_op, co_op, h, w):
                    continue
                buf = torch.zeros(nb, dtype=torch.uint8, device=self.device)
                self._pk16[(wname, tr)] = buf
                cjobs.append(_lib.ConvPackJob(self.params[wname + ".weight"].data_ptr(), buf.data_ptr(), cin, cout, tr))
        if cjobs:
            self._split_conv_jobs = (_lib.ConvPackJob * len(cjobs))(*cjobs)

    def _build_mlp_fused(self):
        self.mlp_fused, self._presummed = False, 0
        sp = self.spec
        if not FUSE_MLP or self.encoder_kind != "mlp" or \
                not self.lib.ppo_mlp_supported(sp.in_features, sp.hidden_units, self.nh):
            return
        P, G = self.params, self.grads
        self._mlp_net = _lib.MlpNet(
            w1=_p(P["encoder.fc1.weight"]), b1=_p(P["encoder.fc1.bias"]), w2=_p(P["encoder.fc2.weight"]),
            b2=_p(P["encoder.fc2.bias"]), wh=_p(self.w_heads), bh=_p(self.b_heads), F=sp.in_features, H=sp.hidden_units,
            NH=self.nh, act=1 if self.encoder_activation_fn == "tanh" else 2)
        self._mlp_grads = _lib.MlpGrads(
            dw1=_p(G["encoder.fc1.weight"]), db1=_p(G["encoder.fc1.bias"]), dw2=_p(G["encoder.fc2.weight"]),
            db2=_p(G["encoder.fc2.bias"]), dwh=_p(self.g_w_heads), dbh=_p(self.g_b_heads), dlog_std=_p(G["log_std"]),
            n_log_std=self.n_actions)
        self._mlp_loss = _lib.MlpLoss()
        self._mlp_npart = ctypes.c_int(0)
        self.mlp_fused = True

    def _mlp_train(self, kind, prev_state, index, stats, n_stats, stat_sums, stat_accumulate, *, obs_indexed=False,
                   **fields):
        B = self._minibatch_rows(prev_state, index, obs_indexed)
        x = prev_state
        if x.dtype != torch.float32 or not x.is_contiguous():
            raise ValueError("the mlp encoder takes contiguous float32 observations")
        x_indexed = int(x.shape[0]) if obs_indexed else 0
        if self.obs_norm is not None:
            if x_indexed:
                raise ValueError("observation normalisation needs the gathered minibatch")
            xn = self._buf("txn", tuple(x.shape))
            self._call("ppo_obs_normalize_f32", _p(x), 0, _p(self.obs_norm.mu), _p(self.obs_norm.std),
                       self.obs_norm.norm_eps, _p(xn), x.shape[0], self.obs_norm.F)
            x = xn
        L = self._mlp_loss
        L.kind, L.stats = kind, _p(stats)
        for k, v in fields.items():
            setattr(L, k, v)
        H = self.hidden_units
        ws = self._buf("mlp_ws", (int(self.lib.ppo_mlp_train_workspace_floats(B, self.spec.in_features, H, self.nh)),))
        partials = self._ws("adam_ws", self.lib.ppo_adam_workspace_bytes())
        self._call("ppo_mlp_train_f32", _p(x), ctypes.addressof(self._mlp_net), ctypes.addressof(self._mlp_grads), _p(index),
                   x_indexed, B, ctypes.addressof(L), _p(ws), None, _p(stat_sums), n_stats, 1 if stat_accumulate else 0,
                   _p(partials), ctypes.addressof(self._mlp_npart))
        self._presummed = self._mlp_npart.value
        return stats

    def _build_tvf_feature_mask(self):
        if not self.use_tvf or (self.tvf_feature_sparsity <= 0 and self.tvf_feature_window <= 0):
            return
        if self.vh != 1:
            raise ValueError("TVF feature masks need a single value head")
        scaled = tvf_feature_mask(self.K, self.hidden_units, self.tvf_feature_sparsity, self.tvf_feature_window)
        w = self.params["tvf_head.weight"]
        w.mul_(scaled.to(self.device))
        self.tvf_features_mask = torch.gt(scaled, 0).to(torch.uint8).to(self.device).contiguous()

    def mask_feature_weights(self):
        if self.tvf_features_mask is not None:
            w = self.params["tvf_head.weight"]
            self._call("ppo_mask_mul_f32", _p(w), _p(self.tvf_features_mask), w.numel())

    @property
    def early_grad_offset(self) -> int:
        return self._offsets["encoder.dense.weight"][0] if self.encoder_kind == "impala" else 0

    def n_parameters(self) -> int:
        return sum(int(np.prod(s)) for _, s in self._offsets.values())

    def state_dict(self) -> "OrderedDict[str, torch.Tensor]":
        names = ["log_std"] + [n for n in self._state_order if n != "log_std"]
        return OrderedDict((n, self.params[n]) for n in names)

    def _build_packed_weights(self):
        self._pk, self._pack_table, self._packed_dirty, self._scatter = {}, None, False, None
        if not PACKED_WEIGHTS or self.encoder_kind != "impala":
            return
        jobs, total = [], 0
        for name, w in self.params.items():
            if not (name.startswith("encoder.stacks.") and name.endswith(".weight")):
                continue
            cout, cin = int(w.shape[0]), int(w.shape[1])
            for transposed in (0, 1):
                if transposed and name == "encoder.stacks.0.firstconv.weight":
                    continue
                n = int(self.lib.ppo_conv3x3_packed_floats(cin, cout, transposed))
                jobs.append((name[:-len(".weight")], transposed, cin, cout, total, n))
                total += n
        self._packed = torch.zeros(total, dtype=torch.float32, device=self.device)
        table = (_lib.PackJob * len(jobs))()
        for k, (wname, transposed, cin, cout, off, n) in enumerate(jobs):
            view = self._packed[off:off + n]
            self._pk[(wname, transposed)] = view
            table[k] = _lib.PackJob(_p(self.params[wname + ".weight"]), _p(view), cin, cout, transposed)
        self._pack_table = table
        self._packed_dirty = True

    def _scatter_table(self):
        if self._scatter is None and self._pack_table is not None:
            n_conv = int(self.early_grad_offset)
            keep = self.flat[:n_conv].clone()
            self.flat[:n_conv] = torch.arange(1, n_conv + 1, dtype=torch.float32, device=self.device)
            self._packed_dirty = True
            self._refresh_packed()
            slots = self._packed.cpu().numpy().astype(np.int64)
            self.flat[:n_conv] = keep
            self._packed_dirty = True
            self._refresh_packed()
            pos = np.flatnonzero(slots > 0)
            src = slots[pos] - 1
            order = np.argsort(src, kind="stable")
            src, pos = src[order], pos[order]
            first = np.r_[True, src[1:] != src[:-1]]
            second = ~first
# ... 16 lines not shown
                    self._call("ppo_conv3x3_pack_weights_f32", ctypes.addressof(self._pack_table), len(self._pack_table))
                if self.split_bf16:
                    self._call("ppo_impala_stack_tail_pack_bf16x3_jobs", ctypes.addressof(self._split_jobs), len(self._split_jobs))
                    if self._split_conv_jobs is not None:
                        self._call("ppo_conv3x3_pack_bf16x3_jobs", ctypes.addressof(self._split_conv_jobs), len(self._split_conv_jobs))
            finally:
                self._rec = rec

    def load_state_dict(self, sd, strict=True):
        self.mark_weights_changed()
        missing = [n for n in self.params if n not in sd]
        unexpected = [n for n in sd if n not in self.params]
        if strict and (missing or unexpected):
            raise KeyError(f"state_dict mismatch: missing {missing}, unexpected {unexpected}")
        with torch.no_grad():
            for n, t in sd.items():
                if n in self.params:
                    self.params[n].copy_(torch.as_tensor(t).to(self.device, torch.float32).reshape(self.params[n].shape))
        self.mask_feature_weights()

    def _buf(self, name, shape, dtype=torch.float32):
        key = (name, tuple(shape), dtype)
        t = self._bufs.get(key)
        if t is None:
            t = torch.empty(shape, dtype=dtype, device=self.device)
            self._bufs[key] = t
        return t

    def _ws(self, name, nbytes):
        return self._buf(name, ((nbytes + 3) // 4,), torch.float32)

    def _call(self, fn_name, *args):
        fn = getattr(self.lib, fn_name)
        if self._rec is not None:
            self._rec.append((fn, fn_name, args))
        rc = fn(*args, _lib.current_stream())
        if rc != 0:
            _lib.check(rc, fn_name)

    def _linear(self, x, k, wname, out, relu_x=0, tag=""):
        w = self.params[wname + ".weight"]
        B, n = x.shape[0], w.shape[0]
        ws_bytes = self.lib.ppo_gemm_workspace_bytes(B, n, k)
        ws = self._ws("gemm_ws" + tag, ws_bytes)
        self._call("ppo_gemm_f32", _p(x), k, 1, relu_x, _p(w), 1, k, 0, _p(self.params[wname + ".bias"]), None,
                   _p(out), n, B, n, k, _p(ws), ws_bytes)

    def _linear_backward(self, x, k, wname, dy, dx, relu_x=0, mask=None, acc=0, side=None):
        w = self.params[wname + ".weight"]
        B, n = dy.shape[0], w.shape[0]

        def param_grads():
            self._call("ppo_gemm_f32", _p(dy), 1, n, 0, _p(x), k, 1, relu_x, None, None,
                       _p(self.grads[wname + ".weight"]), k, n, k, B, None, 0)
            if not (wname == "encoder.dense" and getattr(self, "_dense_bias_done", False)):
                self._call("ppo_colsum_f32", _p(dy), B, n, n, _p(self.grads[wname + ".bias"]), acc)

        if side is None:
            param_grads()
        else:
            with torch.cuda.stream(side):
                param_grads()
        if dx is not None:
            self._call("ppo_gemm_f32", _p(dy), n, 1, 0, _p(w), k, 1, 0, None, _p(mask), _p(dx), k, B, k, n, None, 0)

    def _conv(self, x, mode, wname, out, residual, n, cin, cout, h, w):
        pk = self._pk.get((wname, 0))
        if pk is not None:
            self._call("ppo_conv3x3_forward_packed_f32", _p(x), mode, _p(pk), _p(self.params[wname + ".bias"]),
                       _p(residual), _p(out), n, cin, cout, h, w)
            return
        self._call("ppo_conv3x3_forward_f32", _p(x), mode, _p(self.params[wname + ".weight"]),
                   _p(self.params[wname + ".bias"]), _p(residual), _p(out), n, cin, cout, h, w)

    def encode(self, x: torch.Tensor, train: bool, tag: Optional[str] = None):
        sp = self.spec
        tag = tag or ("t" if train else "i")
        self._refresh_packed()
        if tuple(x.shape[1:]) != sp.input_dims:
            raise ValueError(f"expected input [B, {sp.input_dims}], got {tuple(x.shape)}")
        if x.dtype not in (torch.uint8, torch.float32) or not x.is_contiguous() or x.device != self.device:
            raise ValueError("input must be a contiguous uint8/float32 tensor on the model's device")
        key = (tag, x.shape[0], x.dtype, self.allow_chain_split)
        plan = None if train or not self.use_plans else self._plans.get(key)
        if plan is not None:
            calls, acts, x_slots = plan
            st, xp = _lib.current_stream(), x.data_ptr()
            for k, (fn, fn_name, args) in enumerate(calls):
                if self.act_tail is not None and fn_name == "ppo_dense_heads_forward_f32":
                    fn_name, tail, self.act_tail = "ppo_dense_heads_act_forward_f32", self.act_tail, None
                    rc = self.lib.ppo_dense_heads_act_forward_f32(*args, *tail, st)
                else:
                    rc = fn(xp, *args[1:], st) if k in x_slots else fn(*args, st)
                if rc != 0:
                    _lib.check(rc, fn_name)
            out = dict(acts)
            if self.obs_norm is None:
                for name in plan_input_keys(self.encoder_kind):
                    out[name] = x
            return out
        if not train and self.use_plans:
            self._rec = []
        try:
            x_in = x
            if self.obs_norm is not None:
                x_in = self._buf(tag + "xn", tuple(x.shape))
                self._call("ppo_obs_normalize_f32", _p(x), 1 if x.dtype == torch.uint8 else 0, _p(self.obs_norm.mu),
                           _p(self.obs_norm.std), self.obs_norm.norm_eps, _p(x_in), x.shape[0], self.obs_norm.F)
            acts = (self._encode_mlp(x_in, train, tag) if self.encoder_kind == "mlp"
                    else self._encode_nature(x_in, train, tag) if self.encoder_kind == "nature"
# ... 286 lines not shown
    def heads(self, acts, tag="i"):
        if isinstance(acts, dict):
            if "heads" in acts:
                return acts["heads"]
            h = acts.get("hact", acts["h"])
        else:
            h = acts
            if self.encoder_activation_fn == "tanh":
                raise ValueError("pass encode()'s dict: the tanh activation is computed there")
        B = h.shape[0]
        o = self._buf(f"{tag}heads", (B, self.nh))
        relu = 1 if self.encoder_activation_fn == "relu" else 0
        self._call("ppo_gemm_f32", _p(h), self.hidden_units, 1, relu, _p(self.w_heads), 1, self.hidden_units, 0,
                   _p(self.b_heads), None, _p(o), self.nh, B, self.nh, self.hidden_units, None, 0)
        return o

    def forward(self, x, policy_temperature: float = 1.0, train: bool = False, exclude_value=False,
                exclude_policy=False, exclude_tvf=False, include_features=False,
                required_tvf_heads=None) -> Dict[str, torch.Tensor]:
        acts = self.encode(x, train)
        o = self.heads(acts, "t" if train else "i")
        B, nA = o.shape[0], self.n_actions
        result = {}
        if include_features:
            result["raw_features"] = acts["h"]
            result["features"] = acts["hact"] if "hact" in acts else torch.relu(acts["h"])
        if not exclude_policy:
            logp = self._buf("log_policy", (B, nA))
            result["raw_policy"] = o[:, :nA]
            if nA > 32:
                pass
            elif policy_temperature > 0:
                self._call("ppo_policy_act_f32", _p(o), B, self.nh, nA, float(policy_temperature), None, 0, 0, 1,
                           _p(logp), None, None, None, None, self.vh)
                result["log_policy"] = logp
            else:
                act = self._buf("greedy_actions", (B,), torch.int32)
                self._call("ppo_policy_act_f32", _p(o), B, self.nh, nA, 1.0, None, 0, 0, 1, _p(logp), _p(act), None,
                           None, None, self.vh)
                argmax_policy = torch.zeros_like(logp)
                argmax_policy[torch.arange(B, device=self.device), act.long()] = 1.0
                eps = 1 + policy_temperature
                result["log_policy"] = torch.log(eps * argmax_policy + (1 - eps) * torch.exp(logp) + 1e-8)
                result["argmax_policy"] = argmax_policy
        if not exclude_value:
            result["value"] = o[:, self.col_value:self.col_value + self.vh]
            if self.use_tvf and not exclude_tvf:
                tvf = o[:, self.col_tvf:].view(B, self.K, self.vh)
                result["tvf_value"] = tvf if required_tvf_heads is None else tvf[:, required_tvf_heads]
        result["advantage"] = o[:, self.col_advantage:self.col_advantage + nA]
        result["_heads"], result["_acts"] = o, acts
        return result

    def backward(self, acts, dheads: torch.Tensor, accumulate: bool = False):
        sp = self.spec
        B = dheads.shape[0]
        H = sp.hidden_units
        if accumulate:
            raise NotImplementedError("micro-batch gradient accumulation is not built: with 288 GB of HBM a whole "
                                      "minibatch is one pass (rl/rollout.py:2331-2374 splits only to fit memory)")
        h = acts["h"]
        relu = self.encoder_activation_fn == "relu"
        hin = h if relu else acts["hact"]
        main = torch.cuda.current_stream()
        side = self._wgrad_side_stream() if (WGRAD_SIDE_STREAM and self.encoder_kind == "impala") else None

        dh = self._buf("dh", (B, H))
        self._dense_bias_done = bool(relu and self.encoder_kind == "impala" and self.nh <= 16)
        if self.nh <= 16:
            self._call("ppo_heads_backward_f32", _p(dheads), _p(hin), 1 if relu else 0, _p(h) if relu else None, _p(self.w_heads),
                       _p(dh), _p(self.g_w_heads), _p(self.g_b_heads) if self.head_bias else None,
                       _p(self.grads["encoder.dense.bias"]) if self._dense_bias_done else None, B, H, self.nh)
        else:
            def head_param_grads():
                self._call("ppo_gemm_f32", _p(dheads), 1, self.nh, 0, _p(hin), H, 1, 1 if relu else 0, None, None,
                           _p(self.g_w_heads), H, self.nh, H, B, None, 0)
                if self.head_bias:
                    self._call("ppo_colsum_f32", _p(dheads), B, self.nh, self.nh, _p(self.g_b_heads), 0)

            if side is None:
                head_param_grads()
            else:
                side.wait_stream(main)
                with torch.cuda.stream(side):
                    head_param_grads()
            self._call("ppo_gemm_f32", _p(dheads), self.nh, 1, 0, _p(self.w_heads), H, 1, 0, None, _p(h) if relu else None,
                       _p(dh), H, B, H, self.nh, None, 0)
        if not relu:
            self._call("ppo_tanh_backward_f32", _p(dh), _p(hin), _p(dh), dh.numel())
        if self.encoder_kind == "mlp":
            self._backward_mlp(acts, dh)
        elif self.encoder_kind == "nature":
            self._backward_nature(acts, dh)
        else:
            self._backward_impala(acts, dh)

    def _backward_mlp(self, acts, dh):
        sp = self.spec
        B, H = dh.shape
        da1 = self._buf("da1", (B, H))
        self._linear_backward(acts["a1"], H, "encoder.fc2", dh, da1)
        self._call("ppo_tanh_backward_f32", _p(da1), _p(acts["a1"]), _p(da1), da1.numel())
        self._linear_backward(acts["x"], sp.in_features, "encoder.fc1", da1, None)

    def _backward_nature(self, acts, dh):
        sp = self.spec
        B = dh.shape[0]
        x, flat = acts["x"], acts["flat"]
        g = self._buf("ng_conv3", tuple(acts["conv3"].shape))
        self._linear_backward(flat, sp.flat, "encoder.fc", dh, g.view(B, sp.flat), mask=flat)
        gate = None
        for li in (2, 1, 0):
            name, cin, cout, k, s, h, w, _ho, _wo = sp.layers[li]
            src = acts[sp.layers[li - 1][0]] if li else x
            mode = IN_U8 if src.dtype == torch.uint8 else IN_NONE
            geom = (B, cin, h, w, cout, k, k, s)
            nbytes = int(self.lib.ppo_conv2d_strided_wgrad_workspace_bytes(*geom))
            ws = self._ws("nwgrad_ws_" + name, nbytes)
            self._call("ppo_conv2d_strided_backward_weight_f32", _p(src), mode, _p(g), _p(gate),
                       _p(self.grads[f"encoder.{name}.weight"]), _p(self.grads[f"encoder.{name}.bias"]), _p(ws), nbytes, *geom)
            if li:
                gx = self._buf("ng_" + sp.layers[li - 1][0], tuple(src.shape))
                self._call("ppo_conv2d_strided_backward_data_f32", _p(g), _p(gate), _p(self.params[f"encoder.{name}.weight"]),
                           _p(gx), *geom)
                g, gate = gx, src
        if self.grad_ready_hook is not None:
            self.grad_ready_hook(torch.cuda.current_stream())

    def _backward_impala(self, acts, dh):
        sp, lib = self.spec, self.lib
        B, H = dh.shape
        flat = acts["flat"]
        c_last, h_last, w_last = sp.out_shape
        g = self._buf(f"g{len(sp.stacks) - 1}_top", (B, c_last, h_last, w_last))
        main = torch.cuda.current_stream()
        side = self._wgrad_side_stream() if WGRAD_SIDE_STREAM else None
        if side is not None:
            side.wait_stream(main)
        self._linear_backward(flat, sp.flat, "encoder.dense", dh, g, relu_x=1, mask=flat, side=side)
        if self.grad_ready_hook is not None:
            self.grad_ready_hook(side if side is not None else main)

        n_wgrad = [0]

        jobs = []

        def split_wgrad(mode, cin, cout, hh, ww):
            return self.split_bf16 and SPLIT_WGRAD and WGRAD_BATCH_REDUCE and mode in (IN_NONE, IN_RELU) \
                and lib.ppo_conv3x3_backward_weight_bf16x3_supported(cin, cout, hh, ww)

        def wgrad(x, mode, dy, wname, n, cin, cout, hh, ww, argmax=None):
            nbytes = lib.ppo_conv3x3_wgrad_workspace_bytes(cin, cout)
            if WGRAD_BATCH_REDUCE:
                ws = self._ws("wgrad_ws_" + wname, nbytes)
                n_slabs = ctypes.c_int(0)
                if argmax is not None and acts.get("in0_index") is not None and wname == "encoder.stacks.0.firstconv":
                    args_ = ("ppo_conv3x3_backward_weight_slabs_pooled_indexed_f32", _p(x), _p(acts["in0_index"]), mode, _p(dy),
                             _p(argmax), _p(ws), nbytes, n, cin, cout, hh, ww, ctypes.addressof(n_slabs))
                elif argmax is not None:
                    args_ = ("ppo_conv3x3_backward_weight_slabs_pooled_f32", _p(x), mode, _p(dy), _p(argmax), _p(ws),
                             nbytes, n, cin, cout, hh, ww, ctypes.addressof(n_slabs))
                elif split_wgrad(mode, cin, cout, hh, ww):
                    keep = ((ctypes.c_void_p * 1)(x.data_ptr()), (ctypes.c_int * 1)(int(mode == IN_RELU)),
                            (ctypes.c_void_p * 1)(dy.data_ptr()), (ctypes.c_void_p * 1)(ws.data_ptr()))
                    args_ = ("ppo_conv3x3_backward_weight_slabs_batch_bf16x3", keep[0], keep[1], keep[2], keep[3], nbytes, 1, n,
                             cin, cout, hh, ww, ctypes.addressof(n_slabs))
                else:
                    args_ = ("ppo_conv3x3_backward_weight_slabs_f32", _p(x), mode, _p(dy), _p(ws), nbytes, n, cin, cout,
                             hh, ww, ctypes.addressof(n_slabs))
            else:
                ws = self._ws("wgrad_ws", nbytes)
                args_ = ("ppo_conv3x3_backward_weight_f32", _p(x), mode, _p(dy), _p(self.grads[wname + ".weight"]),
                         _p(self.grads[wname + ".bias"]), _p(ws), nbytes, n, cin, cout, hh, ww, 0)
            if side is None:
                self._call(*args_)
            else:
                ev = self._wgrad_events[n_wgrad[0]]
                n_wgrad[0] += 1
                ev.record(main)
                side.wait_event(ev)
                with torch.cuda.stream(side):
                    self._call(*args_)
            if WGRAD_BATCH_REDUCE:
                jobs.append(_lib.WgradJob(_p(ws), _p(self.grads[wname + ".weight"]), _p(self.grads[wname + ".bias"]),
                                          n_slabs.value, cin, cout, 0))

        carry = []

        def flush_carry():
            while carry:
                x, dy, wname, n, c, hh, ww = carry.pop()
                wgrad(x, IN_NONE, dy, wname, n, c, c, hh, ww)

        def wgrad_blocks(problems, n, c, hh, ww):
            if not (WGRAD_BATCH_LAUNCH and WGRAD_BATCH_REDUCE) or len(problems) > 4:
                flush_carry()
                for x, dy, wname in problems:
                    wgrad(x, IN_RELU, dy, wname, n, c, c, hh, ww)
                return
            relu = [1] * len(problems)
            if carry and carry[-1][3:] == (n, c, hh, ww):
                x, dy, wname = carry.pop()[:3]
                problems = list(problems) + [(x, dy, wname)]
                relu.append(0)
            flush_carry()
            nbytes = lib.ppo_conv3x3_wgrad_workspace_bytes(c, c)
            wss = [self._ws("wgrad_ws_" + wname, nbytes) for _x, _dy, wname in problems]
            k = len(problems)
            n_slabs = ctypes.c_int(0)
            ins = (ctypes.c_void_p * k)(*[x.data_ptr() for x, _d, _w in problems])
            dys = (ctypes.c_void_p * k)(*[dy.data_ptr() for _x, dy, _w in problems])
            wsp = (ctypes.c_void_p * k)(*[ws.data_ptr() for ws in wss])
            if split_wgrad(IN_RELU, c, c, hh, ww):
                args_ = ("ppo_conv3x3_backward_weight_slabs_batch_bf16x3", ins, (ctypes.c_int * k)(*relu), dys, wsp, nbytes, k, n,
                         c, c, hh, ww, ctypes.addressof(n_slabs))
            elif k > 4:
                args_ = ("ppo_conv3x3_backward_weight_slabs_batch_mixed_f32", ins, (ctypes.c_int * k)(*relu), dys, wsp, nbytes, k, n,
                         c, c, hh, ww, ctypes.addressof(n_slabs))
            else:
                args_ = ("ppo_conv3x3_backward_weight_slabs_batch_f32", ins, IN_RELU, dys, wsp, nbytes, k, n, c, c, hh, ww,
                         ctypes.addressof(n_slabs))
            if side is None:
                self._call(*args_)
            else:
                ev = self._wgrad_events[n_wgrad[0]]
                n_wgrad[0] += 1
                ev.record(main)
                side.wait_event(ev)
                with torch.cuda.stream(side):
                    self._call(*args_)
            for (_x, _dy, wname), ws in zip(problems, wss):
                jobs.append(_lib.WgradJob(_p(ws), _p(self.grads[wname + ".weight"]), _p(self.grads[wname + ".bias"]),
                                          n_slabs.value, c, c, 0))

        for si in reversed(range(len(sp.stacks))):
            cin, cout, hh, ww, ho, wo = sp.stacks[si]
            full_w = self._stack_full_bwd_ptrs(si, cin, cout, hh, ww) if si > 0 else None
            if full_w is not None:
                b0, b1 = f"encoder.stacks.{si}.blocks.0", f"encoder.stacks.{si}.blocks.1"
                p_in, a0, q0, a1 = acts[f"q{si}_0_in"], acts[f"a{si}_0"], acts[f"q{si}_1_in"], acts[f"a{si}_1"]
                da1, g1, da0, g0 = (self._buf(nm, (B, cout, ho, wo)) for nm in
                                    (f"g{si}_1_da", f"g{si}_1_in", f"g{si}_0_da", f"g{si}_0_in"))
                dc = self._buf(f"g{si}_dc", (B, cout, hh, ww))
                g_prev = self._buf(f"g{si - 1}_top", (B, cin, hh, ww))
                masks = (ctypes.c_void_p * 4)(a1.data_ptr(), q0.data_ptr(), a0.data_ptr(), p_in.data_ptr())
                self._call("ppo_impala_stack_full_backward_f32", _p(g), full_w, masks, _p(acts[f"idx{si}"]), _p(da1), _p(g1),
                           _p(da0), _p(g0), _p(dc), _p(g_prev), B, cout, hh, ww)
                wgrad_blocks([(a1, g, b1 + ".conv1"), (q0, da1, b1 + ".conv0"), (a0, g1, b0 + ".conv1"),
                              (p_in, da0, b0 + ".conv0")], B, cout, ho, wo)
                wgrad(acts[f"in{si}"], IN_NONE, dc, f"encoder.stacks.{si}.firstconv", B, cin, cout, hh, ww)
                g = g_prev
                continue
            tail_w = self._stack_tail_bwd_ptrs(si, cout, ho, wo)
            split = self.split_bf16 and (si, 1) in self._pk16
            if split:
                tail_w = True
            if tail_w is not None:
                b0, b1 = f"encoder.stacks.{si}.blocks.0", f"encoder.stacks.{si}.blocks.1"
                p_in, a0, q0, a1 = acts[f"q{si}_0_in"], acts[f"a{si}_0"], acts[f"q{si}_1_in"], acts[f"a{si}_1"]
                da1, g1, da0, g0 = (self._buf(nm, (B, cout, ho, wo)) for nm in
                                    (f"g{si}_1_da", f"g{si}_1_in", f"g{si}_0_da", f"g{si}_0_in"))
                masks = (ctypes.c_void_p * 4)(a1.data_ptr(), q0.data_ptr(), a0.data_ptr(), p_in.data_ptr())
                if split and acts.get(f"signs{si}") is not None:
                    self._call("ppo_impala_stack_tail_backward_signs_bf16x3", _p(g), _p(self._pk16[(si, 1)]), acts[f"signs{si}"],
                               _p(da1), _p(g1), _p(da0), _p(g0), B, cout, ho, wo)
                elif split:
                    self._call("ppo_impala_stack_tail_backward_bf16x3", _p(g), _p(self._pk16[(si, 1)]), masks, _p(da1), _p(g1),
                               _p(da0), _p(g0), B, cout, ho, wo)
                else:
                    self._call("ppo_impala_stack_tail_backward_f32", _p(g), tail_w, masks, _p(da1), _p(g1), _p(da0), _p(g0),
                               B, cout, ho, wo)
                wgrad_blocks([(a1, g, b1 + ".conv1"), (q0, da1, b1 + ".conv0"), (a0, g1, b0 + ".conv1"),
                              (p_in, da0, b0 + ".conv0")], B, cout, ho, wo)
                g = g0
            defer = WGRAD_BATCH_LAUNCH and WGRAD_BATCH_REDUCE and sp.n_block * 2 <= 4
            problems = []
            for bi in (reversed(range(sp.n_block)) if tail_w is None else ()):
                base = f"encoder.stacks.{si}.blocks.{bi}"
                q_in, a = acts[f"q{si}_{bi}_in"], acts[f"a{si}_{bi}"]
                if defer:
                    problems.append((a, g, base + ".conv1"))
                else:
                    wgrad(a, IN_RELU, g, base + ".conv1", B, cout, cout, ho, wo)
                da = self._buf(f"g{si}_{bi}_da", (B, cout, ho, wo))
                self._call(self._bwd_data_fn(base + ".conv1"), _p(g), _p(self._bwd_w(base + ".conv1")), _p(a), None,
                           _p(da), B, cout, cout, ho, wo)
                if defer:
                    problems.append((q_in, da, base + ".conv0"))
                else:
                    wgrad(q_in, IN_RELU, da, base + ".conv0", B, cout, cout, ho, wo)
                gn = self._buf(f"g{si}_{bi}_in", (B, cout, ho, wo))
                self._call(self._bwd_data_fn(base + ".conv0"), _p(da), _p(self._bwd_w(base + ".conv0")), _p(q_in),
                           _p(g), _p(gn), B, cout, cout, ho, wo)
                g = gn
            if problems:
                wgrad_blocks(problems, B, cout, ho, wo)
            x_in = acts[f"in{si}"]
            mode = IN_NONE if si > 0 else (IN_U8 if x_in.dtype == torch.uint8 else IN_NONE)
            if si == 0 and WGRAD_POOLED_DY and WGRAD_BATCH_REDUCE \
                    and lib.ppo_conv3x3_backward_weight_pooled_supported(cin, cout, hh, ww):
                wgrad(x_in, mode, g, f"encoder.stacks.{si}.firstconv", B, cin, cout, hh, ww, argmax=acts[f"idx{si}"])
                continue
            dc = self._buf(f"g{si}_dc", (B, cout, hh, ww))
            self._call("ppo_maxpool3x3s2_backward_f32", _p(g), _p(acts[f"idx{si}"]), _p(dc), B, cout, hh, ww)
            if WGRAD_RIDE and WGRAD_BATCH_LAUNCH and WGRAD_BATCH_REDUCE and side is None and si > 0 and cin == cout \
                    and mode == IN_NONE and sp.n_block == 2 and sp.stacks[si - 1][1] == cin \
                    and tuple(sp.stacks[si - 1][4:6]) == (hh, ww):
                carry.append((x_in, dc, f"encoder.stacks.{si}.firstconv", B, cin, hh, ww))
            else:
                wgrad(x_in, mode, dc, f"encoder.stacks.{si}.firstconv", B, cin, cout, hh, ww)
            if si > 0:
                g = self._buf(f"g{si - 1}_top", (B, cin, hh, ww))
                fc = f"encoder.stacks.{si}.firstconv"
                if self.split_bf16 and (fc, 1) in self._pk16:
                    self._call("ppo_conv3x3_bf16x3", _p(dc), 0, _p(self._pk16[(fc, 1)]), None, _p(g), B, cout, cin, hh, ww)
                else:
                    self._call(self._bwd_data_fn(fc), _p(dc), _p(self._bwd_w(fc)),
                               None, None, _p(g), B, cin, cout, hh, ww)
        flush_carry()
        if jobs:
            table = (_lib.WgradJob * len(jobs))(*jobs)
            if side is None:
                self._call("ppo_conv3x3_wgrad_reduce_f32", ctypes.addressof(table), len(jobs))
            else:
                with torch.cuda.stream(side):
                    self._call("ppo_conv3x3_wgrad_reduce_f32", ctypes.addressof(table), len(jobs))
        if side is not None:
            main.wait_stream(side)

    def _stack_full_bwd_ptrs(self, si, cin, cout, h, w):
        if not (FUSE_STACK_FULL_BWD and FUSE_STACK_TAIL) or self.spec.n_block != 2 or cin != cout \
                or not self.lib.ppo_impala_stack_full_supported(cout, h, w):
            return None
        cached = self._tail_ptrs.get(("full_bwd", si))
        if cached is None:
            names = [f"encoder.stacks.{si}.blocks.{bi}.conv{ci}" for bi in (1, 0) for ci in (1, 0)]
            names.append(f"encoder.stacks.{si}.firstconv")
            pks = [self._pk.get((n, 1)) for n in names]
            if any(pk is None for pk in pks):
                return None
            cached = (ctypes.c_void_p * 5)(*[pk.data_ptr() for pk in pks])
            self._tail_ptrs[("full_bwd", si)] = cached
        return cached

    def _stack_tail_bwd_ptrs(self, si, cout, ho, wo):
        if not (FUSE_STACK_TAIL and FUSE_STACK_TAIL_BWD >> si & 1) or self.spec.n_block != 2 \
                or not self.lib.ppo_impala_stack_tail_supported(cout, ho, wo) or (cout == 16 and not FUSE_STACK16):
            return None
        cached = self._tail_ptrs.get(("bwd", si))
        if cached is None:
            names = [f"encoder.stacks.{si}.blocks.{bi}.conv{ci}" for bi in (1, 0) for ci in (1, 0)]
            pks = [self._pk.get((n, 1)) for n in names]
            if any(pk is None for pk in pks):
                return None
            cached = (ctypes.c_void_p * 4)(*[pk.data_ptr() for pk in pks])
            self._tail_ptrs[("bwd", si)] = cached
        return cached

    def _bwd_data_fn(self, wname):
        return "ppo_conv3x3_backward_data_packed_f32" if (wname, 1) in self._pk else "ppo_conv3x3_backward_data_f32"

    def _bwd_w(self, wname):
        return self._pk.get((wname, 1), self.params[wname + ".weight"])

    def _wgrad_side_stream(self):
        if getattr(self, "_wgrad_stream", None) is None:
            self._wgrad_stream = torch.cuda.Stream(device=self.device)
            n = len(self.spec.stacks) * (1 + 2 * self.spec.n_block)
            self._wgrad_events = [torch.cuda.Event() for _ in range(n)]
        return self._wgrad_stream

    def takes_obs_index(self, obs) -> bool:
        if self.encoder_kind != "impala" or obs.dtype != torch.uint8 or self.obs_norm is not None or not GATHER_IN_CONV:
            return False
        cin, cout, h, w, _ho, _wo = self.spec.stacks[0]
        return bool(FUSE_POOL_STACKS & 1) and self._pk.get(("encoder.stacks.0.firstconv", 0)) is not None \
            and bool(WGRAD_POOLED_DY and WGRAD_BATCH_REDUCE) \
            and bool(self.lib.ppo_conv3x3_backward_weight_pooled_supported(cin, cout, h, w))

    @staticmethod
    def _minibatch_rows(prev_state, index, obs_indexed) -> int:
        if obs_indexed:
            if index is None:
                raise ValueError("obs_indexed=True needs the index that prev_state is read through")
            return int(index.shape[0])
        B = int(prev_state.shape[0])
        if index is not None and int(index.shape[0]) != B:
            raise ValueError(f"prev_state holds {B} rows for a minibatch of {int(index.shape[0])}: pass the gathered "
                             "minibatch, or the array the index points into with obs_indexed=True")
        return B

    def _train_forward(self, prev_state, index=None, obs_indexed=False):
        self._minibatch_rows(prev_state, index, obs_indexed)
        if obs_indexed:
            if not self.takes_obs_index(prev_state):
                raise ValueError("this net needs the gathered minibatch of observations (takes_obs_index is False)")
            self.obs_index = index
        try:
            acts = self.encode(prev_state, train=True)
        finally:
            self.obs_index = None
        o = self.heads(acts, "t")
        B = o.shape[0]
        return acts, o, B, self._buf("dheads", (B, self.nh))

    def ppo_minibatch(self, prev_state, actions, old_log_pac, old_log_policy, advantages, returns,
                      eps_clip=0.2, ent_coef=0.01, vf_coef=0.5, loss_scale=1.0, index=None, stat_sums=None,
                      stat_accumulate=False, obs_indexed=False):
        if self.mlp_fused:
            B = self._minibatch_rows(prev_state, index, obs_indexed)
            return self._mlp_train(
                _lib.MLP_LOSS_PPO, prev_state, index, self._buf("loss_stats", (B, 8)), 8, stat_sums, stat_accumulate,
                obs_indexed=obs_indexed, grad_scale=float(loss_scale) / B, n_actions=self.n_actions,
                n_value_heads=self.vh if returns is not None else 0,
                returns=_p(returns), vf_coef=float(vf_coef), actions_i=_p(actions), old_log_pac=_p(old_log_pac),
                old_log_policy=_p(old_log_policy), advantages=_p(advantages), eps_clip=float(eps_clip), ent_coef=float(ent_coef))
        B = self._minibatch_rows(prev_state, index, obs_indexed)
        stats = self._buf("loss_stats", (B, 8))
        vh = self.vh if returns is not None else 0
        loss_args = (self.n_actions, vh, _p(actions), _p(old_log_pac), _p(old_log_policy), _p(advantages), _p(returns),
                     float(eps_clip), float(ent_coef), float(vf_coef), float(loss_scale) / B,
                     _p(self._buf("dheads", (B, self.nh))), _p(stats), _p(index))
        self.loss_tail = loss_args if FUSE_LOSS else None
        try:
            acts, o, B, dheads = self._train_forward(prev_state, index, obs_indexed)
            fused = FUSE_LOSS and self.loss_tail is None
        finally:
            self.loss_tail = None
        if not fused:
            self._call("ppo_ppo_loss_f32", _p(o), B, self.nh, *loss_args)
        self.backward(acts, dheads)
        return stats

    def gaussian_minibatch(self, prev_state, actions, old_log_pac, advantages, returns, eps_clip=0.2, vf_coef=0.5,
                           loss_scale=1.0, index=None, stat_sums=None, stat_accumulate=False, obs_indexed=False):
        if self.mlp_fused:
            B = self._minibatch_rows(prev_state, index, obs_indexed)
            return self._mlp_train(
                _lib.MLP_LOSS_GAUSSIAN, prev_state, index, self._buf("loss_stats", (B, 8)), 8, stat_sums, stat_accumulate,
                obs_indexed=obs_indexed, grad_scale=float(loss_scale) / B, n_actions=self.n_actions,
                n_value_heads=self.vh if returns is not None else 0,
                returns=_p(returns), vf_coef=float(vf_coef), actions_f=_p(actions), old_log_pac=_p(old_log_pac),
                advantages=_p(advantages), log_std=_p(self.params["log_std"]), eps_clip=float(eps_clip),
                dlog_std_rows=_p(self._buf("dlog_std_rows", (B, self.n_actions))))
        acts, o, B, dheads = self._train_forward(prev_state, index, obs_indexed)
        stats = self._buf("loss_stats", (B, 8))
        rows = self._buf("dlog_std_rows", (B, self.n_actions))
        vh = self.vh if returns is not None else 0
        self._call("ppo_gaussian_loss_f32", _p(o), B, self.nh, self.n_actions, vh, _p(actions), _p(old_log_pac),
                   _p(advantages), _p(returns), _p(self.params["log_std"]), float(eps_clip), float(vf_coef),
                   float(loss_scale) / B, _p(dheads), _p(rows), _p(stats), _p(index))
        self._call("ppo_colsum_f32", _p(rows), B, self.n_actions, self.n_actions, _p(self.grads["log_std"]), 0)
        self.backward(acts, dheads)
        return stats

    def value_minibatch(self, prev_state, returns=None, tvf_returns=None, tvf_weights=None, vf_coef=0.5,
                        tvf_coef=1.0, loss_scale=1.0, index=None, tvf_keep_prob=1.0, dropout_seed=0, dropout_offset=0,
                        stat_sums=None, stat_accumulate=False, obs_indexed=False):
        if self.mlp_fused:
            B = self._minibatch_rows(prev_state, index, obs_indexed)
            return self._mlp_train(
                _lib.MLP_LOSS_VALUE, prev_state, index, self._buf("value_stats", (B, 4)), 4, stat_sums, stat_accumulate,
                obs_indexed=obs_indexed, grad_scale=float(loss_scale) / B, value_col=self.col_value,
                n_value_heads=self.vh if returns is not None else 0,
                returns=_p(returns), vf_coef=float(vf_coef), tvf_col=self.col_tvf if self.K else 0,
                n_tvf=self.K if tvf_returns is not None else 0, tvf_stride=max(self.vh, 1), tvf_returns=_p(tvf_returns),
                tvf_weights=_p(tvf_weights), tvf_coef=float(tvf_coef), tvf_keep_prob=float(tvf_keep_prob),
                seed=int(dropout_seed) & (2**64 - 1), offset=int(dropout_offset) & (2**64 - 1))
        acts, o, B, dheads = self._train_forward(prev_state, index, obs_indexed)
        stats = self._buf("value_stats", (B, 4))
        self._call("ppo_value_loss_f32", _p(o), B, self.nh, self.col_value, self.vh if returns is not None else 0,
                   _p(returns), float(vf_coef), self.col_tvf if self.K else 0, self.K if tvf_returns is not None else 0,
                   max(self.vh, 1), _p(tvf_returns), _p(tvf_weights), float(tvf_coef), float(loss_scale) / B, _p(dheads),
                   _p(stats), _p(index), float(tvf_keep_prob), int(dropout_seed) & (2**64 - 1),
                   int(dropout_offset) & (2**64 - 1))
        self.backward(acts, dheads)
        return stats

    def distil_minibatch(self, prev_state, targets, old_policy, beta=1.0, use_tvf=False, weights=None, gaussian=False,
                         loss_scale=1.0, index=None, stat_sums=None, stat_accumulate=False, obs_indexed=False):
        col, n_pred, stride = (self.col_tvf, self.K, self.vh) if use_tvf else (self.col_value, 1, 1)
        if self.mlp_fused:
            B = self._minibatch_rows(prev_state, index, obs_indexed)
            return self._mlp_train(
                _lib.MLP_LOSS_DISTIL, prev_state, index, self._buf("distil_stats", (B, 4)), 4, stat_sums, stat_accumulate,
                obs_indexed=obs_indexed, grad_scale=float(loss_scale) / B, n_actions=self.n_actions, pred_col=col,
                n_pred=n_pred, pred_stride=stride,
                vector_targets=1 if use_tvf else 0, targets=_p(targets), weights=_p(weights), old_policy=_p(old_policy),
                log_std=_p(self.params["log_std"]) if gaussian else None, beta=float(beta))
        acts, o, B, dheads = self._train_forward(prev_state, index, obs_indexed)
        stats = self._buf("distil_stats", (B, 4))
        self._call("ppo_distil_loss_f32", _p(o), B, self.nh, self.n_actions, col, n_pred, stride, 1 if use_tvf else 0,
                   _p(targets), _p(weights), _p(old_policy), _p(self.params["log_std"]) if gaussian else None,
                   float(beta), float(loss_scale) / B, _p(dheads), _p(stats), _p(index))
        self.backward(acts, dheads)
        return stats

    def last_dheads(self, B):
        if self.mlp_fused:
            ws = self._buf("mlp_ws", (int(self.lib.ppo_mlp_train_workspace_floats(B, self.spec.in_features, self.hidden_units,
                                                                                   self.nh)),))
            return ws[4 * B * self.hidden_units:4 * B * self.hidden_units + B * self.nh].view(B, self.nh)
        return self._buf("dheads", (B, self.nh))

    def zero_untouched_grads(self):
        self.grads["log_std"].zero_()

    def adam_step(self, lr=2.5e-4, beta1=0.9, beta2=0.999, eps=1e-5, max_grad_norm=20.0, grad_div=1.0,
                  grad_norm_out: Optional[torch.Tensor] = None, state: Optional["AdamState"] = None):
        ws = self._ws("adam_ws", self.lib.ppo_adam_workspace_bytes())
        scatter = self._scatter_table() if ADAM_SCATTER else None
        if scatter is None:
            self.mark_weights_changed()
        elif self._packed_dirty:
            self._refresh_packed()
        if state is not None:
            state.ensure(self.flat)
            state.step += 1
            m, v, step = state.exp_avg, state.exp_avg_sq, state.step
        else:
            if self.exp_avg is None:
                self.exp_avg = torch.zeros_like(self.flat)
                self.exp_avg_sq = torch.zeros_like(self.flat)
            self._adam_step += 1
            m, v, step = self.exp_avg, self.exp_avg_sq, self._adam_step
        n_part, self._presummed = self._presummed, 0
        if n_part and scatter is None and grad_div == 1.0:
            self._call("ppo_adam_step_presummed_f32", _p(self.flat), _p(self.grad), _p(m), _p(v), self.flat.numel(), step,
                       float(lr), float(beta1), float(beta2), float(eps), float(max_grad_norm), float(grad_div), _p(ws),
                       n_part, _p(grad_norm_out))
            self.mask_feature_weights()
            return
        if scatter is not None:
            self._call("ppo_adam_step_scatter_f32", _p(self.flat), _p(self.grad), _p(m), _p(v), self.flat.numel(), step,
                       float(lr), float(beta1), float(beta2), float(eps), float(max_grad_norm), float(grad_div), _p(ws),
                       _p(grad_norm_out), _p(scatter[0]), scatter[1], _p(self._packed))
            self.mask_feature_weights()
            return
        self._call("ppo_adam_step_f32", _p(self.flat), _p(self.grad), _p(m), _p(v), self.flat.numel(), step, float(lr),
                   float(beta1), float(beta2), float(eps), float(max_grad_norm), float(grad_div), _p(ws),
                   _p(grad_norm_out))
        self.mask_feature_weights()

    def parameter_order(self):
        return list(self.state_dict().keys())

    def adam_state_dict(self, exp_avg, exp_avg_sq, step, cfg=None):
        names = self.parameter_order()
        state = {}
        if exp_avg is not None and step > 0:
            touched = {}
            for i, name in enumerate(names):
                o, shape = self._offsets[name]
                n = int(np.prod(shape))
                touched[i] = (exp_avg_sq[o:o + n], exp_avg[o:o + n], shape)
            flags = torch.stack([(v != 0).any() | (m != 0).any() for v, m, _ in touched.values()]).cpu().tolist()
            for (i, (v, m, shape)), hit in zip(touched.items(), flags):
                if hit:
                    state[i] = {"step": torch.tensor(float(step), dtype=torch.float32),
                                "exp_avg": m.view(shape).clone(), "exp_avg_sq": v.view(shape).clone()}
        group = {"lr": float(cfg.lr) if cfg is not None else 0.0,
                 "betas": (float(cfg.adam_beta1), float(cfg.adam_beta2)) if cfg is not None else (0.9, 0.999),
                 "eps": float(cfg.adam_epsilon) if cfg is not None else 1e-8, "weight_decay": 0, "amsgrad": False,
                 "maximize": False, "foreach": None, "capturable": False, "params": list(range(len(names)))}
        return {"state": state, "param_groups": [group]}

    def read_adam_state_dict(self, sd):
        if "flat" in sd:
            return (sd["flat"]["exp_avg"].to(self.device).clone(), sd["flat"]["exp_avg_sq"].to(self.device).clone(),
                    int(sd["step"]))
        state = sd.get("state") or {}
        if not state:
            return None, None, int(sd.get("step", 0)) if not isinstance(sd.get("step"), torch.Tensor) else 0
        names = self.parameter_order()
        m, v, step = torch.zeros_like(self.flat), torch.zeros_like(self.flat), int(sd.get("step", 0) or 0)
        for key, st in state.items():
            name = names[int(key)] if not isinstance(key, str) or key.isdigit() else key
            o, shape = self._offsets[name]
            n = int(np.prod(shape))
            m[o:o + n].copy_(torch.as_tensor(st["exp_avg"]).reshape(-1))
            v[o:o + n].copy_(torch.as_tensor(st["exp_avg_sq"]).reshape(-1))
            if "step" in st:
                step = max(step, int(float(st["step"])))
        return m, v, step

    def optimizer_state_dict(self, cfg=None):
        return self.adam_state_dict(self.exp_avg, self.exp_avg_sq, self._adam_step, cfg)

    def load_optimizer_state_dict(self, sd):
        self.exp_avg, self.exp_avg_sq, self._adam_step = self.read_adam_state_dict(sd)


# ... 134 lines not shown
```

ppo_amd/rollout.py:

```python
import copy
import math
import os

import numpy as np
import torch

from . import _lib, parallel, value_quality
from .config import args
from .models import AdamState
from .returns import calculate_bootstrapped_returns


ROLLOUT_GRAPH = int(os.environ.get("PPO_AMD_ROLLOUT_GRAPH", "0"))
UPLOAD_CHUNKS = int(os.environ.get("PPO_AMD_UPLOAD_CHUNKS", "2"))
FUSE_ACT = int(os.environ.get("PPO_AMD_FUSE_ACT", "1"))


def _p(t):
    return None if t is None else t.data_ptr()


class Optimizer:

    def __init__(self, net, cfg, state=None):
# ... 564 lines not shown
        if not args.disable_logging:
            self.log_returns(value)

    @property
    def reward_scale(self):
        if args.env.reward_normalization == "off":
            return 1.0
        if args.env.reward_normalization != "rms":
            raise ValueError(f"Invalid reward normalization {args.env.reward_normalization}")
        from . import wrappers
        norm = wrappers.get_wrapper(self.vec_env, wrappers.VecNormalizeRewardWrapper)
        return 1.0 if norm is None else float(1.0 / norm.std)

    def log_returns(self, value_estimate):
        N = self.N
        head0 = self.value_heads[0]
        named = [("*ext_value_estimates", value_estimate, {}), ("adv_ext", self.advantage, {"display_width": 0})]
        for i, head in enumerate(self.value_heads):
            named.append((f"*return_{head}", self.returns[..., i], {"display_width": 0}))
            named.append((f"value_{head}", self.value[..., i], {"display_name": "v_" + head}))
        value_quality.log_batch_moments(self.log, named)
        self.log.watch_mean("reward_scale", self.reward_scale, display_width=0, history_length=1)
        self.log.watch_mean("entropy_bonus", self.current_entropy_bonus, display_width=0, history_length=1)
        self.log.watch("*gamma", args.gamma)
        if self.tvf is not None:
            self.log.watch("*tvf_gamma", args.tvf.gamma)
            self.log.watch_stats("*tvf_return_ext", self.tvf.tvf_returns[:, :, -1].cpu().numpy())
        if args.disable_ev or self.batch_counter % 4 != 3:
            return
        value_quality.log_feature_statistics(
            self.log, self.detached_batch_forward(self.all_obs[0], output="full", include_features=True))
        ext_value = self.value[..., self.value_heads.index("ext")] if "ext" in self.value_heads else self.value[..., 0]
        targets = calculate_bootstrapped_returns(self.ext_rewards, self.terminals, ext_value[N], float(args.gamma))
        if self.tvf is not None:
            self.tvf.log_tvf_curve_quality(ext_value[:N], targets)
        else:
            value_quality.log_dna_value_quality(self.log, ext_value[:N], targets)

    def _normalize_advantages(self):
        n = self.N * self.A
        self._call("ppo_moments_f64", _p(self.advantage), n, _p(self._moments), _p(self._moments_ws))
        parallel.allreduce_sum_(self._moments)
        self._call("ppo_normalize_f32", _p(self.advantage), n, _p(self._moments), float(self.current_advantage_epsilon),
                   _p(self.norm_advantage), _p(self._mean_std))
        if args.advantage_clipping is not None:
            self.norm_advantage.clamp_(-args.advantage_clipping, args.advantage_clipping)

    def optimizer_step(self, optimizer=None, label="policy", norm_out=None):
        opt = optimizer or self.policy_optimizer
        net, cfg = opt.net, opt.cfg
        red = self._reducers.get(id(net))
        if red is not None:
            red.finish()
        net.adam_step(lr=self._lr(cfg), beta1=cfg.adam_beta1, beta2=cfg.adam_beta2, eps=cfg.adam_epsilon,
                      max_grad_norm=args.max_grad_norm if args.grad_clip_mode == "global_norm" else 0.0,
                      grad_div=float(self.world), grad_norm_out=self._grad_norm if norm_out is None else norm_out,
                      state=opt.state)
        return self._grad_norm if norm_out is None else norm_out

    def _micro_batches(self, mb, force_micro_batch_size=None):
        micro = force_micro_batch_size if force_micro_batch_size is not None else min(args.max_micro_batch_size, mb)
        if micro <= 0 or mb % micro:
            raise ValueError(f"minibatch {mb} is not a multiple of the micro-batch size {micro}")
        return micro, mb // micro

    class _Accumulator:

        def __init__(self, runner, net, count):
            self.r, self.net, self.count, self.k = runner, net, count, 0
            self.hook = net.grad_ready_hook
            if count > 1:
                net.grad_ready_hook = None
                self.acc = net._buf("grad_accum", tuple(net.grad.shape))

        def after_backward(self):
            if self.count > 1:
                if self.k == 0:
                    self.acc.copy_(self.net.grad)
                else:
                    self.r._call("ppo_accumulate_f32", _p(self.acc), _p(self.net.grad), self.net.grad.numel())
            self.k += 1

        def finish(self):
            if self.count > 1:
                self.net.grad.copy_(self.acc)
                self.net._presummed = 0
            self.restore_hook()

        def restore_hook(self):
            self.net.grad_ready_hook = self.hook

    def _run_epochs(self, label, optimizer, epochs, mini_batch_size, step_fn, n_stats):
        B = self.N * self.A
        net = optimizer.net
        mb = parallel.local_minibatch(mini_batch_size)
        if B % mb:
            raise ValueError(f"batch {B} is not a multiple of the per-rank minibatch {mb}")
        n_mb = B // mb
        micro, n_micro = self._micro_batches(mb)
        obs_rows = self.all_obs[:self.N].view(B, -1)
        row_bytes = obs_rows.shape[1] * obs_rows.element_size()
        fused = bool(getattr(net, "mlp_fused", False)) and net.obs_norm is None and self.all_obs.dtype == torch.float32
        in_conv = not fused and hasattr(net, "takes_obs_index") and net.takes_obs_index(self.all_obs)
        obs_all = self.all_obs[:self.N].view(B, *self.state_shape)
        mb_obs = None if (fused or in_conv) else net._buf("mb_obs", (micro, *self.state_shape), self.all_obs.dtype)
        stat_rows = net._buf(f"stat_rows_{label}", (epochs * n_mb, n_stats))
        norm_rows = net._buf(f"norm_rows_{label}", (epochs * n_mb,))
        k = 0
        for _epoch in range(epochs):
            ordering = np.arange(B, dtype=np.int32)
            np.random.shuffle(ordering)
            order_dev = torch.from_numpy(ordering).to(self.device, non_blocking=True)
            for j in range(n_mb):
                acc = self._Accumulator(self, net, n_micro)
                try:
                    for u in range(n_micro):
                        idx = order_dev[j * mb + u * micro:j * mb + (u + 1) * micro]
                        if fused:
                            step_fn(obs_rows, idx, 1.0 / n_micro, stat_sums=stat_rows[k], stat_accumulate=bool(u),
                                    obs_indexed=True)
                            acc.after_backward()
                            continue
                        if in_conv:
                            stats = step_fn(obs_all, idx, 1.0 / n_micro, obs_indexed=True)
                        else:
                            self._call("ppo_gather_rows", _p(obs_rows), row_bytes, B, _p(idx), micro, _p(mb_obs))
                            stats = step_fn(mb_obs, idx, 1.0 / n_micro)
                        acc.after_backward()
                        self._call("ppo_colsum_f32", _p(stats), micro, n_stats, n_stats, _p(stat_rows[k]), 1 if u else 0)
                    acc.finish()
                finally:
                    acc.restore_hook()
                self.optimizer_step(optimizer, label, norm_out=norm_rows[k:k + 1])
                k += 1
        self._phase_stats[label] = (stat_rows, norm_rows, mb)

    def train_policy(self):
        if args.policy_opt.epochs == 0:
            return
        B = self.N * self.A
        net = self.policy_net
        self._normalize_advantages()
        returns = None if self.dual else self.returns
        net.zero_untouched_grads()
        if self.action_dist == "discrete":
            def step(mb_obs, idx, loss_scale, **kw):
                return net.ppo_minibatch(mb_obs, self.actions, self.log_pac, self.log_policy, self.norm_advantage,
                                         returns, eps_clip=self.ppo_epsilon, ent_coef=self.current_entropy_bonus,
                                         vf_coef=args.ppo_vf_coef, loss_scale=loss_scale, index=idx, **kw)
        else:
            actions, log_pac = self.actions.view(B, self.n_actions), self.log_pac.view(B, self.n_actions)

            def step(mb_obs, idx, loss_scale, **kw):
                return net.gaussian_minibatch(mb_obs, actions, log_pac, self.norm_advantage, returns,
                                              eps_clip=self.ppo_epsilon, vf_coef=args.ppo_vf_coef, loss_scale=loss_scale,
                                              index=idx, **kw)
        self._run_epochs("policy", self.policy_optimizer, args.policy_opt.epochs, args.policy_opt.mini_batch_size,
                         step, 8)

    def train_value(self):
        if args.value_opt.epochs == 0:
            return
        B = self.N * self.A
        net = self.value_net
        use_ext = self.tvf is None or args.tvf.include_ext
        returns = self.returns.view(B, self.VH) if use_ext else None
        tvf_returns = self.tvf.tvf_returns[:, :, :, -1].reshape(B, self.K) if self.tvf is not None else None
        weights = self._tvf_value_weights_dev if self.tvf is not None else None
        net.zero_untouched_grads()

        keep = 1.0 - args.tvf.horizon_dropout if self.tvf is not None else 1.0
        seed = self._device_seed * 1000003 + 7919 * (self.rank + 1)

        def step(mb_obs, idx, loss_scale, **kw):
            off = self.tvf.next_dropout_offset(idx.shape[0] * self.K) if keep < 1.0 else 0
            return net.value_minibatch(mb_obs, returns=returns, tvf_returns=tvf_returns, tvf_weights=weights,
                                       vf_coef=args.ppo_vf_coef, tvf_coef=args.tvf.coef, loss_scale=loss_scale, index=idx,
                                       tvf_keep_prob=keep, dropout_seed=seed, dropout_offset=off, **kw)
        self._run_epochs("value", self.value_optimizer, args.value_opt.epochs, args.value_opt.mini_batch_size, step, 4)

    def wants_distil_update(self, location=None):
        return (self.dual and args.distil_opt.epochs > 0 and self.step >= args.distil.delay * 1e6
# ... 255 lines not shown
```

Measured before the change: 97070.

## Fuse backward tail: paired dense-backward GEMMs and single grad-finish kernel

Adds a paired GEMM kernel that runs the dense layer's weight-grad and data-grad GEMMs in one launch, and a new grad-finish kernel that merges the conv wgrad slab reduction, the sum-of-squares partials for Adam, and the per-minibatch stats column sum. The Python training loop now passes stat sums into the minibatch step instead of issuing a separate colsum call, and tracks partial-grad state so the presummed norm path stays correct. The aim is to cut kernel launches and host overhead in the backward/optimizer tail. The trade-off is more complex bookkeeping, with a risk of stale presummed partials when microbatch accumulation is used.

After: 96080. 0.99x the previous value.

```diff
diff --git a/include/ppo_amd.h b/include/ppo_amd.h
--- a/include/ppo_amd.h
+++ b/include/ppo_amd.h
@@ -109,6 +109,9 @@
                                                  void *workspace, size_t workspace_bytes, int n, int cin, int cout, int h,
                                                  int w, int *n_slabs, void *stream);
 int ppo_conv3x3_wgrad_reduce_f32(const ppo_wgrad_job *jobs, int n_jobs, void *stream);
+size_t ppo_grad_finish_workspace_bytes(void);
+int ppo_grad_finish_f32(const ppo_wgrad_job *jobs, int n_jobs, float *grads, int64_t n, void *workspace, int *n_partials,
+                        const float *X, int M, int N, int64_t ldx, float *out, int accumulate, void *stream);
 
 int ppo_maxpool3x3s2_forward_f32(const float *in, float *out, uint8_t *argmax, int n, int c, int h, int w,
                                  void *stream);
@@ -130,6 +133,8 @@
 int ppo_gemm_f32(const float *A, int64_t a_sm, int64_t a_sk, int relu_a, const float *B, int64_t b_sk, int64_t b_sn,
                  int relu_b, const float *bias, const float *mask, float *C, int64_t ldc, int M, int N, int K,
                  void *workspace, size_t workspace_bytes, void *stream);
+int ppo_dense_backward_f32(const float *dy, const float *x, int relu_x, const float *W, const float *mask, float *dW,
+                           float *dx, int B, int K, int H, void *stream);
 
 int ppo_dense_heads_forward_f32(const float *x, int relu_x, const float *W, const float *b, const float *Wh, const float *bh,
                                 int relu_h, float *h, float *heads, int M, int K, int H, int NH, void *workspace,
diff --git a/ppo_amd/_lib.py b/ppo_amd/_lib.py
--- a/ppo_amd/_lib.py
+++ b/ppo_amd/_lib.py
@@ -31,6 +31,7 @@
     "ppo_gemm_workspace_bytes": (_sz, [_i, _i, _i]),
     "ppo_gemm_f32": (_i, [_vp, _i64, _i64, _i, _vp, _i64, _i64, _i, _vp, _vp, _vp, _i64, _i, _i, _i, _vp, _sz, _vp]),
     "ppo_colsum_f32": (_i, [_vp, _i, _i, _i64, _vp, _i, _vp]),
+    "ppo_dense_backward_f32": (_i, [_vp, _vp, _i, _vp, _vp, _vp, _vp, _i, _i, _i, _vp]),
     "ppo_heads_backward_f32": (_i, [_vp, _vp, _i, _vp, _vp, _vp, _vp, _vp, _vp, _i, _i, _i, _vp]),
     "ppo_dense_heads_forward_f32": (_i, [_vp, _i, _vp, _vp, _vp, _vp, _i, _vp, _vp, _i, _i, _i, _i, _vp, _sz, _vp]),
     "ppo_dense_heads_act_forward_f32": (_i, [_vp, _i, _vp, _vp, _vp, _vp, _i, _vp, _vp, _i, _i, _i, _i, _vp, _sz, _i, _f, _u64,
@@ -74,6 +75,8 @@
     "ppo_conv3x3_backward_weight_bf16x3_supported": (_i, [_i, _i, _i, _i]),
     "ppo_conv3x3_backward_weight_slabs_batch_bf16x3": (_i, [_vp, _vp, _vp, _vp, _sz, _i, _i, _i, _i, _i, _i, _vp, _vp]),
     "ppo_conv3x3_wgrad_reduce_f32": (_i, [_vp, _i, _vp]),
+    "ppo_grad_finish_workspace_bytes": (_sz, []),
+    "ppo_grad_finish_f32": (_i, [_vp, _i, _vp, _i64, _vp, _vp, _vp, _i, _i, _i64, _vp, _i, _vp]),
     "ppo_tanh_forward_f32": (_i, [_vp, _vp, _sz, _vp]),
     "ppo_tanh_backward_f32": (_i, [_vp, _vp, _vp, _sz, _vp]),
     "ppo_value_loss_f32": (_i, [_vp, _i, _i, _i, _i, _vp, _f, _i, _i, _i, _vp, _vp, _f, _f, _vp, _vp, _vp, _f, _u64, _u64, _vp]),
diff --git a/ppo_amd/csrc/conv3x3_wgrad.hip b/ppo_amd/csrc/conv3x3_wgrad.hip
--- a/ppo_amd/csrc/conv3x3_wgrad.hip
+++ b/ppo_amd/csrc/conv3x3_wgrad.hip
@@ -1,5 +1,6 @@
 #include "common.h"
 #include "conv_stage.h"
+#include "grad_tail.h"
 #include "mfma.h"
 
 namespace ppo {
@@ -371,23 +372,6 @@
     PPO_STAMP_ADD(3, t_k3, t_k0)
 }
 
-__device__ __forceinline__ float4 slab_partition_sum(const float *slabs, int byte_off, int byte_stride, int lo, int hi, bool live)
-{
-    const __amdgpu_buffer_rsrc_t buf = buffer_of(slabs);
-    float4 s0 = make_float4(0.f, 0.f, 0.f, 0.f), s1 = s0;
-    for (int q = lo; q < hi; q += 16) {
-        float4 v[16];
-#pragma unroll
-        for (int u = 0; u < 16; ++u) v[u] = buffer_f32x4(buf, (live && q + u < hi) ? byte_off + (q + u) * byte_stride : kOutside);
-#pragma unroll
-        for (int u = 0; u < 16; u += 2) {
-            s0.x += v[u].x; s0.y += v[u].y; s0.z += v[u].z; s0.w += v[u].w;
-            s1.x += v[u + 1].x; s1.y += v[u + 1].y; s1.z += v[u + 1].z; s1.w += v[u + 1].w;
-        }
-    }
-    return make_float4(s0.x + s1.x, s0.y + s1.y, s0.z + s1.z, s0.w + s1.w);
-}
-
 __global__ __launch_bounds__(256) void conv3x3_wgrad_reduce_kernel(const float *__restrict__ partial, int n_slabs,
                                                                    int cout, int cin, int cinp, int jp,
                                                                    float *__restrict__ dw, float *__restrict__ db,
@@ -447,47 +431,8 @@
 {
     __shared__ float4 s[256];
     const ppo_wgrad_job &job = jobs.j[blockIdx.y];
-    const int cout = job.cout, cin = job.cin, n_slabs = job.n_slabs, accumulate = job.accumulate;
-    const int cinp = (cin + 3) / 4 * 4;
-    const int jp = ((9 * cinp + 1) + 15) / 16 * 16;
-    const int q4 = jp / 4;
-    if ((int)blockIdx.x * 16 >= cout * q4) return;
-    const int idx = blockIdx.x * 16 + (threadIdx.x & 15);
-    const int part = threadIdx.x >> 4;
-    const bool live = idx < cout * q4;
-    const int co = live ? idx / q4 : 0;
-    const int j0 = live ? (idx % q4) * 4 : 0;
-    const size_t stride = (size_t)cout * jp;
-    const int per = (n_slabs + 15) / 16;
-    const int lo = part * per;
-    const int hi = lo + per < n_slabs ? lo + per : n_slabs;
-    s[threadIdx.x] = slab_partition_sum(job.slabs, (co * jp + j0) * 4, (int)stride * 4, lo, hi, live);
-    __syncthreads();
-    if (part == 0 && live) {
-        float sum[4] = {0.f, 0.f, 0.f, 0.f};
-#pragma unroll
-        for (int q = 0; q < 16; ++q) {
-            const float4 a = s[q * 16 + threadIdx.x];
-            sum[0] += a.x;
-            sum[1] += a.y;
-            sum[2] += a.z;
-            sum[3] += a.w;
-        }
-#pragma unroll
-        for (int e = 0; e < 4; ++e) {
-            const int j = j0 + e;
-            if (j == 9 * cinp) {
-                if (job.dbias) job.dbias[co] = accumulate ? job.dbias[co] + sum[e] : sum[e];
-            } else if (j < 9 * cinp) {
-                const int tap = j / cinp;
-                const int ci = j % cinp;
-                if (ci < cin) {
-                    float *d = job.dweight + ((size_t)co * cin + ci) * 9 + tap;
-                    *d = accumulate ? *d + sum[e] : sum[e];
-                }
-            }
-        }
-    }
+    if ((int)blockIdx.x >= wgrad_reduce_blocks(job.cin, job.cout)) return;
+    wgrad_reduce_body<false>(job, blockIdx.x, s);
 }
 
 template <int CIN, int COUT, int H, int W, int TR, int IN_MODE, bool DY_POOLED = false>
diff --git a/ppo_amd/csrc/gemm.hip b/ppo_amd/csrc/gemm.hip
--- a/ppo_amd/csrc/gemm.hip
+++ b/ppo_amd/csrc/gemm.hip
@@ -1,6 +1,7 @@
 #include <algorithm>
 
 #include "common.h"
+#include "grad_tail.h"
 #include "loss_rows.h"
 #include "policy_act.h"
 #include "mfma.h"
@@ -153,11 +154,10 @@
 static_assert(DEPTH % 2 == 0, "the LDS buffer of a slab is its slot's parity");
 
 template <bool a_kfast, bool b_kfast, bool vec>
-__global__ __launch_bounds__(kGemmThreads) void gemm_f32_kernel(GemmArgs p, int gm, int gn)
-{
-    __shared__ __align__(16) float s_a[2][TILE_WORDS];
-    __shared__ __align__(16) float s_b[2][TILE_WORDS];
-    const TileId t = tile_of(blockIdx.x, gm, gn, p.split);
+__device__ __forceinline__ void gemm_tile(const GemmArgs &p, int gm, int gn, int id, float (*s_a)[TILE_WORDS],
+                                          float (*s_b)[TILE_WORDS])
+{
+    const TileId t = tile_of(id, gm, gn, p.split);
     if (!t.live) return;
     const int tid = threadIdx.x;
     const int lane = tid & 63;
@@ -304,6 +304,25 @@
     PPO_GSTAMP(4);
 }
 
+template <bool a_kfast, bool b_kfast, bool vec>
+__global__ __launch_bounds__(kGemmThreads) void gemm_f32_kernel(GemmArgs p, int gm, int gn)
+{
+    __shared__ __align__(16) float s_a[2][TILE_WORDS];
+    __shared__ __align__(16) float s_b[2][TILE_WORDS];
+    gemm_tile<a_kfast, b_kfast, vec>(p, gm, gn, blockIdx.x, s_a, s_b);
+}
+
+__global__ __launch_bounds__(kGemmThreads) void gemm_pair_f32_kernel(GemmArgs p0, int gm0, int gn0, int first, GemmArgs p1,
+                                                                     int gm1, int gn1)
+{
+    __shared__ __align__(16) float s_a[2][TILE_WORDS];
+    __shared__ __align__(16) float s_b[2][TILE_WORDS];
+    if ((int)blockIdx.x < first)
+        gemm_tile<false, false, true>(p0, gm0, gn0, blockIdx.x, s_a, s_b);
+    else
+        gemm_tile<true, false, true>(p1, gm1, gn1, (int)blockIdx.x - first, s_a, s_b);
+}
+
 __global__ __launch_bounds__(256) void gemm_finalize_kernel(const float *__restrict__ partial, int split, int M, int N,
                                                             const float *__restrict__ bias,
                                                             const float *__restrict__ mask, float *__restrict__ C,
@@ -435,29 +454,7 @@
                                                      float *__restrict__ out, int accumulate)
 {
     __shared__ float s[256];
-    const int n = blockIdx.x * 16 + (threadIdx.x & 15);
-    const int part = threadIdx.x >> 4;
-    float v = 0.f;
-    if (n < N) {
-        for (int m = part; m < M; m += 16 * 8) {
-            float t[8];
-#pragma unroll
-            for (int u = 0; u < 8; ++u) {
-                const int mm = m + 16 * u;
-                t[u] = mm < M ? X[mm * ldx + n] : 0.f;
-            }
-#pragma unroll
-            for (int u = 0; u < 8; ++u) v += t[u];
-        }
-    }
-    s[threadIdx.x] = v;
-    __syncthreads();
-    if (part == 0 && n < N) {
-        float t = 0.f;
-#pragma unroll
-        for (int q = 0; q < 16; ++q) t += s[q * 16 + threadIdx.x];
-        out[n] = accumulate ? out[n] + t : t;
-    }
+    colsum_body(X, M, N, ldx, out, accumulate, blockIdx.x, s);
 }
 
 struct ActTail {
@@ -688,32 +685,32 @@
     bool act_fused = false;
 };
 
-int gemm_dispatch(const float *A, int64_t a_sm, int64_t a_sk, int relu_a, const float *B, int64_t b_sk, int64_t b_sn,
-                  int relu_b, const float *bias, const float *mask, float *C, int64_t ldc, int M, int N, int K,
-                  void *workspace, size_t workspace_bytes, void *stream, HeadsTail *tail)
-{
+struct GemmPlan {
+    bool empty, skinny;
+    GemmArgs p;
+    int gm, gn;
+};
+
+int gemm_plan(const float *A, int64_t a_sm, int64_t a_sk, int relu_a, const float *B, int64_t b_sk, int64_t b_sn, int relu_b,
+              const float *bias, const float *mask, float *C, int64_t ldc, int M, int N, int K, void *workspace,
+              size_t workspace_bytes, GemmPlan &pl)
+{
+    pl.empty = pl.skinny = false;
     if (M < 0 || N < 0 || K < 0) return fail(PPO_E_INVALID, "ppo_gemm_f32: negative dimension");
-    if (M == 0 || N == 0) return PPO_OK;
+    if (M == 0 || N == 0) {
+        pl.empty = true;
+        return PPO_OK;
+    }
     if (!A || !B || !C) return fail(PPO_E_INVALID, "ppo_gemm_f32: null pointer");
     if (ldc < N) return fail(PPO_E_INVALID, "ppo_gemm_f32: ldc < N");
     const int64_t a_last = (int64_t)(M - 1) * a_sm + (int64_t)(K - 1) * a_sk, b_last = (int64_t)(N - 1) * b_sn + (int64_t)(K - 1) * b_sk;
     if (K > 0 && (a_last * 4 + 16 > (int64_t)kBufferBytes || b_last * 4 + 16 > (int64_t)kBufferBytes || a_sm < 0 || a_sk < 0 ||
                   b_sn < 0 || b_sk < 0))
         return fail(PPO_E_INVALID, "ppo_gemm_f32: operand spans 2 GiB or more (or a negative stride); split the batch");
-    hipStream_t st = as_stream(stream);
     if ((N <= 16 || K <= 16 || (M <= 16 && a_sm == 1)) && (int64_t)M * N <= (1 << 22)) {
-        GemmArgs q{A, B, C, bias, mask, M, N, K, a_sm, a_sk, b_sk, b_sn, ldc, relu_a, relu_b, K, 1, 0, 0, 0};
-        if (N <= kRowsMaxN && a_sk == 1 && b_sk == 1 && K <= 64 * kRowsMaxKPerLane) {
-            if (K <= 256 && N <= 16)
-                hipLaunchKernelGGL((gemm_rows_kernel<16, 4>), dim3((M + 3) / 4), dim3(256), 0, st, q);
-            else if (K <= 256)
-                hipLaunchKernelGGL((gemm_rows_kernel<8, 4>), dim3((M + 3) / 4), dim3(256), 0, st, q);
-            else
-                hipLaunchKernelGGL((gemm_rows_kernel<4, kRowsMaxKPerLane>), dim3((M + 3) / 4), dim3(256), 0, st, q);
-            return check_launch("gemm_rows_kernel");
-        }
-        hipLaunchKernelGGL(gemm_small_kernel, dim3((M * N + 15) / 16), dim3(256), 0, st, q);
-        return check_launch("gemm_small_kernel");
+        pl.skinny = true;
+        pl.p = GemmArgs{A, B, C, bias, mask, M, N, K, a_sm, a_sk, b_sk, b_sn, ldc, relu_a, relu_b, K, 1, 0, 0, 0};
+        return PPO_OK;
     }
     const int gm = (M + BM - 1) / BM, gn = (N + BN - 1) / BN;
     constexpr int kSliceK = 256;
@@ -728,6 +725,34 @@
                ldc, relu_a, relu_b, kps, split, vec_ok(A, a_sm, a_sk, M, K) ? 1 : 0, vec_ok(B, b_sn, b_sk, N, K) ? 1 : 0, 0};
     p.vec_c = N % 4 == 0 && ldc % 4 == 0 && aligned(C, 16) && aligned(p.C, 16) && (!bias || aligned(bias, 16)) &&
               (!mask || (aligned(mask, 16) && (int64_t)M * ldc * 4 < (int64_t)kBufferBytes));
+    pl.p = p, pl.gm = gm, pl.gn = gn;
+    return PPO_OK;
+}
+
+int gemm_dispatch(const float *A, int64_t a_sm, int64_t a_sk, int relu_a, const float *B, int64_t b_sk, int64_t b_sn,
+                  int relu_b, const float *bias, const float *mask, float *C, int64_t ldc, int M, int N, int K,
+                  void *workspace, size_t workspace_bytes, void *stream, HeadsTail *tail)
+{
+    GemmPlan pl;
+    int rc = gemm_plan(A, a_sm, a_sk, relu_a, B, b_sk, b_sn, relu_b, bias, mask, C, ldc, M, N, K, workspace, workspace_bytes, pl);
+    if (rc || pl.empty) return rc;
+    hipStream_t st = as_stream(stream);
+    if (pl.skinny) {
+        const GemmArgs &q = pl.p;
+        if (N <= kRowsMaxN && a_sk == 1 && b_sk == 1 && K <= 64 * kRowsMaxKPerLane) {
+            if (K <= 256 && N <= 16)
+                hipLaunchKernelGGL((gemm_rows_kernel<16, 4>), dim3((M + 3) / 4), dim3(256), 0, st, q);
+            else if (K <= 256)
+                hipLaunchKernelGGL((gemm_rows_kernel<8, 4>), dim3((M + 3) / 4), dim3(256), 0, st, q);
+            else
+                hipLaunchKernelGGL((gemm_rows_kernel<4, kRowsMaxKPerLane>), dim3((M + 3) / 4), dim3(256), 0, st, q);
+            return check_launch("gemm_rows_kernel");
+        }
+        hipLaunchKernelGGL(gemm_small_kernel, dim3((M * N + 15) / 16), dim3(256), 0, st, q);
+        return check_launch("gemm_small_kernel");
+    }
+    const GemmArgs &p = pl.p;
+    const int gm = pl.gm, gn = pl.gn, split = p.split;
     const dim3 grid(tile_grid(gm, gn, split));
     const bool vec = p.vec_a && p.vec_b;
     const int variant = (a_sk == 1 ? 4 : 0) | (b_sk == 1 ? 2 : 0) | (vec ? 1 : 0);
@@ -746,7 +771,7 @@
         PPO_GEMM_CASE(7, true, true, true)
     }
 #undef PPO_GEMM_CASE
-    int rc = check_launch("gemm_f32_kernel");
+    rc = check_launch("gemm_f32_kernel");
     if (rc) return rc;
     if (split > 1) {
         if (tail && !mask && ldc == N && N <= 256 && tail->NH <= 32 && (int64_t)split * M * N * 4 < (int64_t)kBufferBytes) {
@@ -788,6 +813,28 @@
 {
     return ppo::gemm_dispatch(A, a_sm, a_sk, relu_a, B, b_sk, b_sn, relu_b, bias, mask, C, ldc, M, N, K, workspace,
                               workspace_bytes, stream, nullptr);
+}
+
+extern "C" int ppo_dense_backward_f32(const float *dy, const float *x, int relu_x, const float *W, const float *mask, float *dW,
+                                      float *dx, int B, int K, int H, void *stream)
+{
+    using namespace ppo;
+    if (B <= 0 || K <= 0 || H <= 0) return fail(PPO_E_INVALID, "ppo_dense_backward_f32: needs B, K, H > 0");
+    if (!dy || !x || !W || !dW || !dx) return fail(PPO_E_INVALID, "ppo_dense_backward_f32: null pointer");
+    GemmPlan w, d;
+    int rc = gemm_plan(dy, 1, H, 0, x, K, 1, relu_x, nullptr, nullptr, dW, K, H, K, B, nullptr, 0, w);
+    if (!rc) rc = gemm_plan(dy, H, 1, 0, W, K, 1, 0, nullptr, mask, dx, K, B, K, H, nullptr, 0, d);
+    if (rc) return rc;
+    const auto paired = [](const GemmPlan &pl) { return !pl.skinny && pl.p.split == 1 && pl.p.vec_a && pl.p.vec_b; };
+    if (!paired(w) || !paired(d)) {
+        rc = gemm_dispatch(dy, 1, H, 0, x, K, 1, relu_x, nullptr, nullptr, dW, K, H, K, B, nullptr, 0, stream, nullptr);
+        if (rc) return rc;
+        return gemm_dispatch(dy, H, 1, 0, W, K, 1, 0, nullptr, mask, dx, K, B, K, H, nullptr, 0, stream, nullptr);
+    }
+    const int first = tile_grid(w.gm, w.gn, 1), second = tile_grid(d.gm, d.gn, 1);
+    hipLaunchKernelGGL(gemm_pair_f32_kernel, dim3(first + second), dim3(kGemmThreads), 0, as_stream(stream), w.p, w.gm, w.gn,
+                       first, d.p, d.gm, d.gn);
+    return check_launch("gemm_pair_f32_kernel");
 }
 
 extern "C" int ppo_dense_heads_forward_f32(const float *x, int relu_x, const float *W, const float *b, const float *Wh,
diff --git a/ppo_amd/csrc/grad_finish.hip b/ppo_amd/csrc/grad_finish.hip
--- /dev/null
+++ b/ppo_amd/csrc/grad_finish.hip
@@ -0,0 +1,153 @@
+#include "grad_tail.h"
+
+namespace ppo {
+namespace {
+
+constexpr int kMaxJobs = 32;
+constexpr int kMaxLast = 500;
+
+struct FinishArgs {
+    ppo_wgrad_job j[kMaxJobs];
+    int start[kMaxJobs + 1];
+    int64_t woff[kMaxJobs];
+    int64_t boff[kMaxJobs];
+    uint16_t expected[kSumsqPartials];
+    int n_jobs, np, stat_blocks;
+    float *grads;
+    int64_t n;
+    float *partials;
+    unsigned *counters;
+    const float *X;
+    int M, N;
+    int64_t ldx;
+    float *out;
+    int accumulate;
+};
+
+template <class F>
+__host__ __device__ inline void for_touched_chunks(int cin, int cout, int bx, int64_t woff, int64_t boff, int64_t chunk, F f)
+{
+    const int q4 = wgrad_slab_row(cin) / 4;
+    const int co_lo = bx * 16 / q4;
+    int co_hi = (bx * 16 + 15) / q4;
+    co_hi = co_hi < cout ? co_hi : cout - 1;
+    int64_t c0 = 0, c1 = -1;
+    if (woff >= 0) {
+        c0 = (woff + (int64_t)co_lo * cin * 9) / chunk;
+        c1 = (woff + (int64_t)(co_hi + 1) * cin * 9 - 1) / chunk;
+        for (int64_t c = c0; c <= c1; ++c) f((int)c);
+    }
+    if (boff >= 0)
+        for (int64_t c = (boff + co_lo) / chunk; c <= (boff + co_hi) / chunk; ++c)
+            if (c < c0 || c > c1) f((int)c);
+}
+
+__global__ __launch_bounds__(256) void grad_finish_kernel(FinishArgs a)
+{
+    __shared__ float4 s4[256];
+    float *s = reinterpret_cast<float *>(s4);
+    int *si = reinterpret_cast<int *>(s4);
+    const int id = blockIdx.x, R = a.start[a.n_jobs];
+    if (id >= R + a.np) {
+        colsum_body(a.X, a.M, a.N, a.ldx, a.out, a.accumulate, id - R - a.np, s);
+        return;
+    }
+    if (id >= R) {
+        const int c = id - R;
+        if (a.expected[c] == 0) grad_sumsq_body(a.grads, a.n, a.np, c, a.partials, s);
+        return;
+    }
+    int k = 0;
+    while (id >= a.start[k + 1]) ++k;
+    const int bx = id - a.start[k];
+    wgrad_reduce_body<true>(a.j[k], bx, s4);
+    if (a.np == 0) return;
+    asm volatile("s_waitcnt vmcnt(0)" ::: "memory");
+    __syncthreads();
+    if (threadIdx.x == 0) {
+        const int64_t chunk = (a.n + a.np - 1) / a.np;
+        int n_last = 0;
+        for_touched_chunks(a.j[k].cin, a.j[k].cout, bx, a.woff[k], a.boff[k], chunk, [&](int c) {
+            global_u32 *cnt = (global_u32 *)(a.counters + c);
+            const unsigned seen = __hip_atomic_fetch_add(cnt, 1u, __ATOMIC_RELAXED, __HIP_MEMORY_SCOPE_AGENT);
+            if (seen + 1 == a.expected[c]) {
+                __hip_atomic_store(cnt, 0u, __ATOMIC_RELAXED, __HIP_MEMORY_SCOPE_AGENT);
+                if (n_last < kMaxLast) si[1 + n_last++] = c;
+            }
+        });
+        si[0] = n_last;
+        if (n_last) {
+            __builtin_amdgcn_fence(__ATOMIC_ACQUIRE, "agent");
+            asm volatile("s_waitcnt vmcnt(0)" ::: "memory");
+        }
+    }
+    __syncthreads();
+    const int n_last = si[0];
+    for (int q = 0; q < n_last; ++q) {
+        grad_sumsq_body(a.grads, a.n, a.np, si[1 + q], a.partials, s + 512);
+        __syncthreads();
+    }
+}
+
+}
+}
+
+extern "C" size_t ppo_grad_finish_workspace_bytes(void)
+{
+    return ppo::kSumsqPartials * (sizeof(float) + sizeof(unsigned));
+}
+
+extern "C" int ppo_grad_finish_f32(const ppo_wgrad_job *jobs, int n_jobs, float *grads, int64_t n, void *workspace,
+                                   int *n_partials, const float *X, int M, int N, int64_t ldx, float *out, int accumulate,
+                                   void *stream)
+{
+    using namespace ppo;
+    if (n_partials) *n_partials = 0;
+    if (n_jobs < 0 || n_jobs > kMaxJobs) return fail(PPO_E_INVALID, "ppo_grad_finish_f32: 0..%d jobs per call", kMaxJobs);
+    if (n_jobs > 0 && !jobs) return fail(PPO_E_INVALID, "ppo_grad_finish_f32: null jobs");
+    if (grads && (n <= 0 || !workspace || !n_partials))
+        return fail(PPO_E_INVALID, "ppo_grad_finish_f32: the sums of g^2 need n > 0, the workspace and n_partials");
+    if (X && (M < 0 || N <= 0 || !out)) return fail(PPO_E_INVALID, "ppo_grad_finish_f32: bad column-sum job");
+    FinishArgs a{};
+    a.n_jobs = n_jobs;
+    a.np = grads ? sumsq_partials(n) : 0;
+    a.grads = grads, a.n = n;
+    a.partials = static_cast<float *>(workspace);
+    a.counters = reinterpret_cast<unsigned *>(a.partials + kSumsqPartials);
+    a.X = X, a.M = M, a.N = N, a.ldx = ldx, a.out = out, a.accumulate = accumulate;
+    a.stat_blocks = X ? (N + 15) / 16 : 0;
+    const int64_t chunk = a.np ? (n + a.np - 1) / a.np : 1;
+    int expected[kSumsqPartials] = {0};
+    for (int i = 0; i < n_jobs; ++i) {
+        const ppo_wgrad_job &j = jobs[i];
+        if (!j.slabs || !j.dweight || j.n_slabs <= 0 || j.cin <= 0 || j.cout <= 0 || j.cout % 16)
+            return fail(PPO_E_INVALID, "ppo_grad_finish_f32: bad job %d", i);
+        a.j[i] = j;
+        a.start[i + 1] = a.start[i] + wgrad_reduce_blocks(j.cin, j.cout);
+        a.woff[i] = a.boff[i] = -1;
+        if (!grads) continue;
+        const int64_t nw = (int64_t)j.cout * j.cin * 9;
+        if (j.dweight + nw > grads && j.dweight < grads + n) {
+            if (j.dweight < grads || j.dweight + nw > grads + n)
+                return fail(PPO_E_INVALID, "ppo_grad_finish_f32: job %d's dweight straddles the end of the flat gradient", i);
+            a.woff[i] = j.dweight - grads;
+        }
+        if (j.dbias && j.dbias + j.cout > grads && j.dbias < grads + n) {
+            if (j.dbias < grads || j.dbias + j.cout > grads + n)
+                return fail(PPO_E_INVALID, "ppo_grad_finish_f32: job %d's dbias straddles the end of the flat gradient", i);
+            a.boff[i] = j.dbias - grads;
+        }
+        const int blocks = a.start[i + 1] - a.start[i];
+        for (int bx = 0; bx < blocks; ++bx)
+            for_touched_chunks(j.cin, j.cout, bx, a.woff[i], a.boff[i], chunk, [&](int c) { ++expected[c]; });
+    }
+    for (int c = 0; c < a.np; ++c) {
+        if (expected[c] > 0xffff) return fail(PPO_E_INVALID, "ppo_grad_finish_f32: too many reductions write into one chunk");
+        a.expected[c] = (uint16_t)expected[c];
+    }
+    const int grid = a.start[n_jobs] + a.np + a.stat_blocks;
+    if (grid == 0) return PPO_OK;
+    hipLaunchKernelGGL(grad_finish_kernel, dim3(grid), dim3(256), 0, as_stream(stream), a);
+    if (n_partials) *n_partials = a.np;
+    return check_launch("grad_finish_kernel");
+}
diff --git a/ppo_amd/csrc/grad_tail.h b/ppo_amd/csrc/grad_tail.h
--- /dev/null
+++ b/ppo_amd/csrc/grad_tail.h
@@ -0,0 +1,146 @@
+#pragma once
+#include "common.h"
+
+namespace ppo {
+
+typedef __attribute__((address_space(1))) float global_f32;
+typedef __attribute__((address_space(1))) unsigned global_u32;
+
+__device__ __forceinline__ float4 slab_partition_sum(const float *slabs, int byte_off, int byte_stride, int lo, int hi, bool live)
+{
+    const __amdgpu_buffer_rsrc_t buf = buffer_of(slabs);
+    float4 s0 = make_float4(0.f, 0.f, 0.f, 0.f), s1 = s0;
+    for (int q = lo; q < hi; q += 16) {
+        float4 v[16];
+#pragma unroll
+        for (int u = 0; u < 16; ++u) v[u] = buffer_f32x4(buf, (live && q + u < hi) ? byte_off + (q + u) * byte_stride : kOutside);
+#pragma unroll
+        for (int u = 0; u < 16; u += 2) {
+            s0.x += v[u].x; s0.y += v[u].y; s0.z += v[u].z; s0.w += v[u].w;
+            s1.x += v[u + 1].x; s1.y += v[u + 1].y; s1.z += v[u + 1].z; s1.w += v[u + 1].w;
+        }
+    }
+    return make_float4(s0.x + s1.x, s0.y + s1.y, s0.z + s1.z, s0.w + s1.w);
+}
+
+__host__ __device__ inline int wgrad_slab_row(int cin)
+{
+    const int cinp = (cin + 3) / 4 * 4;
+    return ((9 * cinp + 1) + 15) / 16 * 16;
+}
+__host__ __device__ inline int wgrad_reduce_blocks(int cin, int cout) { return (cout * (wgrad_slab_row(cin) / 4) + 15) / 16; }
+
+template <bool PUBLISH>
+__device__ __forceinline__ void wgrad_reduce_body(const ppo_wgrad_job &job, int bx, float4 *s)
+{
+    const int cout = job.cout, cin = job.cin, n_slabs = job.n_slabs, accumulate = job.accumulate;
+    const int cinp = (cin + 3) / 4 * 4;
+    const int jp = ((9 * cinp + 1) + 15) / 16 * 16;
+    const int q4 = jp / 4;
+    const int idx = bx * 16 + (threadIdx.x & 15);
+    const int part = threadIdx.x >> 4;
+    const bool live = idx < cout * q4;
+    const int co = live ? idx / q4 : 0;
+    const int j0 = live ? (idx % q4) * 4 : 0;
+    const size_t stride = (size_t)cout * jp;
+    const int per = (n_slabs + 15) / 16;
+    const int lo = part * per;
+    const int hi = lo + per < n_slabs ? lo + per : n_slabs;
+    s[threadIdx.x] = slab_partition_sum(job.slabs, (co * jp + j0) * 4, (int)stride * 4, lo, hi, live);
+    __syncthreads();
+    auto put = [](float *d, float v) {
+        if (PUBLISH)
+            __hip_atomic_store((global_f32 *)d, v, __ATOMIC_RELAXED, __HIP_MEMORY_SCOPE_AGENT);
+        else
+            *d = v;
+    };
+    if (part == 0 && live) {
+        float sum[4] = {0.f, 0.f, 0.f, 0.f};
+#pragma unroll
+        for (int q = 0; q < 16; ++q) {
+            const float4 a = s[q * 16 + threadIdx.x];
+            sum[0] += a.x;
+            sum[1] += a.y;
+            sum[2] += a.z;
+            sum[3] += a.w;
+        }
+#pragma unroll
+        for (int e = 0; e < 4; ++e) {
+            const int j = j0 + e;
+            if (j == 9 * cinp) {
+                if (job.dbias) put(job.dbias + co, accumulate ? job.dbias[co] + sum[e] : sum[e]);
+            } else if (j < 9 * cinp) {
+                const int tap = j / cinp;
+                const int ci = j % cinp;
+                if (ci < cin) {
+                    float *d = job.dweight + ((size_t)co * cin + ci) * 9 + tap;
+                    put(d, accumulate ? *d + sum[e] : sum[e]);
+                }
+            }
+        }
+    }
+}
+
+__device__ __forceinline__ void grad_sumsq_body(float *g, int64_t n, int np, int c, float *partials, float *s)
+{
+    const int64_t chunk = (n + np - 1) / np;
+    const int64_t lo = (int64_t)c * chunk;
+    const int64_t hi = lo + chunk < n ? lo + chunk : n;
+    float acc = 0.f;
+    int64_t i = lo + threadIdx.x;
+    for (; i + 768 < hi; i += 1024) {
+        const float x0 = g[i], x1 = g[i + 256], x2 = g[i + 512], x3 = g[i + 768];
+        acc += x0 * x0;
+        acc += x1 * x1;
+        acc += x2 * x2;
+        acc += x3 * x3;
+    }
+    for (; i < hi; i += 256) {
+        const float x = g[i];
+        acc += x * x;
+    }
+    s[threadIdx.x] = acc;
+    __syncthreads();
+    for (int w = 128; w > 0; w >>= 1) {
+        if (threadIdx.x < w) s[threadIdx.x] += s[threadIdx.x + w];
+        __syncthreads();
+    }
+    if (threadIdx.x == 0) partials[c] = s[0];
+}
+
+__device__ __forceinline__ void colsum_body(const float *__restrict__ X, int M, int N, int64_t ldx, float *__restrict__ out,
+                                            int accumulate, int bx, float *s)
+{
+    const int n = bx * 16 + (threadIdx.x & 15);
+    const int part = threadIdx.x >> 4;
+    float v = 0.f;
+    if (n < N) {
+        for (int m = part; m < M; m += 16 * 8) {
+            float t[8];
+#pragma unroll
+            for (int u = 0; u < 8; ++u) {
+                const int mm = m + 16 * u;
+                t[u] = mm < M ? X[mm * ldx + n] : 0.f;
+            }
+#pragma unroll
+            for (int u = 0; u < 8; ++u) v += t[u];
+        }
+    }
+    s[threadIdx.x] = v;
+    __syncthreads();
+    if (part == 0 && n < N) {
+        float t = 0.f;
+#pragma unroll
+        for (int q = 0; q < 16; ++q) t += s[q * 16 + threadIdx.x];
+        out[n] = accumulate ? out[n] + t : t;
+    }
+}
+
+constexpr int kSumsqPartials = 256;
+inline int sumsq_partials(int64_t n)
+{
+    const int64_t np = (n + 4095) / 4096;
+    return (int)(np > kSumsqPartials ? kSumsqPartials : np);
+}
+
+}
diff --git a/ppo_amd/csrc/optim.hip b/ppo_amd/csrc/optim.hip
--- a/ppo_amd/csrc/optim.hip
+++ b/ppo_amd/csrc/optim.hip
@@ -1,37 +1,16 @@
 #include "common.h"
+#include "grad_tail.h"
 
 namespace ppo {
 namespace {
 
-constexpr int kPartials = 256;
+constexpr int kPartials = kSumsqPartials;
 __device__ __forceinline__ bool aligned16(const void *p) { return (reinterpret_cast<uintptr_t>(p) & 15) == 0; }
 
-__global__ __launch_bounds__(256) void grad_sumsq_kernel(const float *__restrict__ g, int64_t n, float *__restrict__ partials)
+__global__ __launch_bounds__(256) void grad_sumsq_kernel(float *g, int64_t n, float *__restrict__ partials)
 {
     __shared__ float s[256];
-    const int64_t chunk = (n + gridDim.x - 1) / gridDim.x;
-    const int64_t lo = (int64_t)blockIdx.x * chunk;
-    const int64_t hi = lo + chunk < n ? lo + chunk : n;
-    float acc = 0.f;
-    int64_t i = lo + threadIdx.x;
-    for (; i + 768 < hi; i += 1024) {
-        const float x0 = g[i], x1 = g[i + 256], x2 = g[i + 512], x3 = g[i + 768];
-        acc += x0 * x0;
-        acc += x1 * x1;
-        acc += x2 * x2;
-        acc += x3 * x3;
-    }
-    for (; i < hi; i += 256) {
-        const float x = g[i];
-        acc += x * x;
-    }
-    s[threadIdx.x] = acc;
-    __syncthreads();
-    for (int w = 128; w > 0; w >>= 1) {
-        if (threadIdx.x < w) s[threadIdx.x] += s[threadIdx.x + w];
-        __syncthreads();
-    }
-    if (threadIdx.x == 0) partials[blockIdx.x] = s[0];
+    grad_sumsq_body(g, n, gridDim.x, blockIdx.x, partials, s);
 }
 
 __global__ __launch_bounds__(256) void adam_kernel(float *__restrict__ w, const float *__restrict__ g,
@@ -176,9 +155,8 @@
     if (!(grad_div > 0.f)) return fail(PPO_E_INVALID, "ppo_adam_step_f32: grad_div must be > 0");
     hipStream_t st = as_stream(stream);
     float *partials = static_cast<float *>(workspace);
-    int np = (int)((n + 4095) / 4096);
-    np = np > kPartials ? kPartials : np;
-    hipLaunchKernelGGL(grad_sumsq_kernel, dim3(np), dim3(256), 0, st, grads, n, partials);
+    const int np = sumsq_partials(n);
+    hipLaunchKernelGGL(grad_sumsq_kernel, dim3(np), dim3(256), 0, st, const_cast<float *>(grads), n, partials);
     int rc = check_launch("grad_sumsq_kernel");
     if (rc) return rc;
     const double bc1 = 1.0 - pow(beta1, (double)step);
diff --git a/ppo_amd/models.py b/ppo_amd/models.py
--- a/ppo_amd/models.py
+++ b/ppo_amd/models.py
@@ -325,6 +325,7 @@
         self._tail_ptrs = {}
         self.obs_norm = None
         self.grad_ready_hook = None
+        self.grad_is_partial = False
         self._split_ws = {}
         self._plans = {}
         self.use_plans = True
@@ -362,18 +363,18 @@
             o, shape = offs[name]
             flat[o:o + t.numel()] = t.reshape(-1)
         self.flat = flat.to(self.device)
-        self.grad = torch.zeros_like(self.flat)
+        self._grad = torch.zeros_like(self.flat)
         self._offsets = offs
         self._state_order = list(init.keys())
         self.params = OrderedDict((name, self.flat[o:o + int(np.prod(shape))].view(shape)) for name, (o, shape) in offs.items())
-        self.grads = OrderedDict((name, self.grad[o:o + int(np.prod(shape))].view(shape)) for name, (o, shape) in offs.items())
+        self._grads = OrderedDict((name, self._grad[o:o + int(np.prod(shape))].view(shape)) for name, (o, shape) in offs.items())
         o = offs["policy_head.weight"][0]
         self.w_heads = self.flat[o:o + self.nh * sp.hidden_units].view(self.nh, sp.hidden_units)
-        self.g_w_heads = self.grad[o:o + self.nh * sp.hidden_units].view(self.nh, sp.hidden_units)
+        self.g_w_heads = self._grad[o:o + self.nh * sp.hidden_units].view(self.nh, sp.hidden_units)
         if self.head_bias:
             o = offs["policy_head.bias"][0]
             self.b_heads = self.flat[o:o + self.nh]
-            self.g_b_heads = self.grad[o:o + self.nh]
+            self.g_b_heads = self._grad[o:o + self.nh]
         else:
             self.b_heads = self.g_b_heads = None
 
@@ -420,7 +421,7 @@
         if not FUSE_MLP or self.encoder_kind != "mlp" or \
                 not self.lib.ppo_mlp_supported(sp.in_features, sp.hidden_units, self.nh):
             return
-        P, G = self.params, self.grads
+        P, G = self.params, self._grads
         self._mlp_net = _lib.MlpNet(
             w1=_p(P["encoder.fc1.weight"]), b1=_p(P["encoder.fc1.bias"]), w2=_p(P["encoder.fc2.weight"]),
             b2=_p(P["encoder.fc2.bias"]), wh=_p(self.w_heads), bh=_p(self.b_heads), F=sp.in_features, H=sp.hidden_units,
@@ -453,7 +454,7 @@
             setattr(L, k, v)
         H = self.hidden_units
         ws = self._buf("mlp_ws", (int(self.lib.ppo_mlp_train_workspace_floats(B, self.spec.in_features, H, self.nh)),))
-        partials = self._ws("adam_ws", self.lib.ppo_adam_workspace_bytes())
+        partials = self._adam_ws()
         self._call("ppo_mlp_train_f32", _p(x), ctypes.addressof(self._mlp_net), ctypes.addressof(self._mlp_grads), _p(index),
                    x_indexed, B, ctypes.addressof(L), _p(ws), None, _p(stat_sums), n_stats, 1 if stat_accumulate else 0,
                    _p(partials), ctypes.addressof(self._mlp_npart))
@@ -474,6 +475,28 @@
         if self.tvf_features_mask is not None:
             w = self.params["tvf_head.weight"]
             self._call("ppo_mask_mul_f32", _p(w), _p(self.tvf_features_mask), w.numel())
+
+    _presummed = 0
+
+    @property
+    def grad(self) -> torch.Tensor:
+        self._presummed = 0
+        return self._grad
+
+    @property
+    def grads(self) -> "OrderedDict[str, torch.Tensor]":
+        self._presummed = 0
+        return self._grads
+
+    def mark_grads_changed(self):
+        self._presummed = 0
+
+    def _adam_ws(self):
+        ws = self._bufs.get("adam_ws")
+        if ws is None:
+            nbytes = max(int(self.lib.ppo_adam_workspace_bytes()), int(self.lib.ppo_grad_finish_workspace_bytes()))
+            ws = self._bufs["adam_ws"] = torch.zeros((nbytes + 3) // 4, dtype=torch.float32, device=self.device)
+        return ws
 
     @property
     def early_grad_offset(self) -> int:
@@ -596,10 +619,16 @@
 
         def param_grads():
             self._call("ppo_gemm_f32", _p(dy), 1, n, 0, _p(x), k, 1, relu_x, None, None,
-                       _p(self.grads[wname + ".weight"]), k, n, k, B, None, 0)
+                       _p(self._grads[wname + ".weight"]), k, n, k, B, None, 0)
             if not (wname == "encoder.dense" and getattr(self, "_dense_bias_done", False)):
-                self._call("ppo_colsum_f32", _p(dy), B, n, n, _p(self.grads[wname + ".bias"]), acc)
-
+                self._call("ppo_colsum_f32", _p(dy), B, n, n, _p(self._grads[wname + ".bias"]), acc)
+
+        if side is None and dx is not None:
+            self._call("ppo_dense_backward_f32", _p(dy), _p(x), relu_x, _p(w), _p(mask), _p(self._grads[wname + ".weight"]),
+                       _p(dx), B, k, n)
+            if not (wname == "encoder.dense" and getattr(self, "_dense_bias_done", False)):
+                self._call("ppo_colsum_f32", _p(dy), B, n, n, _p(self._grads[wname + ".bias"]), acc)
+            return
         if side is None:
             param_grads()
         else:
@@ -992,7 +1021,7 @@
         result["_heads"], result["_acts"] = o, acts
         return result
 
-    def backward(self, acts, dheads: torch.Tensor, accumulate: bool = False):
+    def backward(self, acts, dheads: torch.Tensor, accumulate: bool = False, stat_job=None):
         sp = self.spec
         B = dheads.shape[0]
         H = sp.hidden_units
@@ -1010,7 +1039,7 @@
         if self.nh <= 16:
             self._call("ppo_heads_backward_f32", _p(dheads), _p(hin), 1 if relu else 0, _p(h) if relu else None, _p(self.w_heads),
                        _p(dh), _p(self.g_w_heads), _p(self.g_b_heads) if self.head_bias else None,
-                       _p(self.grads["encoder.dense.bias"]) if self._dense_bias_done else None, B, H, self.nh)
+                       _p(self._grads["encoder.dense.bias"]) if self._dense_bias_done else None, B, H, self.nh)
         else:
             def head_param_grads():
                 self._call("ppo_gemm_f32", _p(dheads), 1, self.nh, 0, _p(hin), H, 1, 1 if relu else 0, None, None,
@@ -1028,12 +1057,16 @@
                        _p(dh), H, B, H, self.nh, None, 0)
         if not relu:
             self._call("ppo_tanh_backward_f32", _p(dh), _p(hin), _p(dh), dh.numel())
+        self._presummed = 0
         if self.encoder_kind == "mlp":
             self._backward_mlp(acts, dh)
         elif self.encoder_kind == "nature":
             self._backward_nature(acts, dh)
-        else:
-            self._backward_impala(acts, dh)
+        elif self._backward_impala(acts, dh, stat_job):
+            return
+        if stat_job is not None:
+            stats, out, acc = stat_job
+            self._call("ppo_colsum_f32", _p(stats), stats.shape[0], stats.shape[1], stats.shape[1], _p(out), 1 if acc else 0)
 
     def _backward_mlp(self, acts, dh):
         sp = self.spec
@@ -1058,7 +1091,7 @@
             nbytes = int(self.lib.ppo_conv2d_strided_wgrad_workspace_bytes(*geom))
             ws = self._ws("nwgrad_ws_" + name, nbytes)
             self._call("ppo_conv2d_strided_backward_weight_f32", _p(src), mode, _p(g), _p(gate),
-                       _p(self.grads[f"encoder.{name}.weight"]), _p(self.grads[f"encoder.{name}.bias"]), _p(ws), nbytes, *geom)
+                       _p(self._grads[f"encoder.{name}.weight"]), _p(self._grads[f"encoder.{name}.bias"]), _p(ws), nbytes, *geom)
             if li:
                 gx = self._buf("ng_" + sp.layers[li - 1][0], tuple(src.shape))
                 self._call("ppo_conv2d_strided_backward_data_f32", _p(g), _p(gate), _p(self.params[f"encoder.{name}.weight"]),
@@ -1067,7 +1100,7 @@
         if self.grad_ready_hook is not None:
             self.grad_ready_hook(torch.cuda.current_stream())
 
-    def _backward_impala(self, acts, dh):
+    def _backward_impala(self, acts, dh, stat_job=None):
         sp, lib = self.spec, self.lib
         B, H = dh.shape
         flat = acts["flat"]
@@ -1110,8 +1143,8 @@
                              hh, ww, ctypes.addressof(n_slabs))
             else:
                 ws = self._ws("wgrad_ws", nbytes)
-                args_ = ("ppo_conv3x3_backward_weight_f32", _p(x), mode, _p(dy), _p(self.grads[wname + ".weight"]),
-                         _p(self.grads[wname + ".bias"]), _p(ws), nbytes, n, cin, cout, hh, ww, 0)
+                args_ = ("ppo_conv3x3_backward_weight_f32", _p(x), mode, _p(dy), _p(self._grads[wname + ".weight"]),
+                         _p(self._grads[wname + ".bias"]), _p(ws), nbytes, n, cin, cout, hh, ww, 0)
             if side is None:
                 self._call(*args_)
             else:
@@ -1122,7 +1155,7 @@
                 with torch.cuda.stream(side):
                     self._call(*args_)
             if WGRAD_BATCH_REDUCE:
-                jobs.append(_lib.WgradJob(_p(ws), _p(self.grads[wname + ".weight"]), _p(self.grads[wname + ".bias"]),
+                jobs.append(_lib.WgradJob(_p(ws), _p(self._grads[wname + ".weight"]), _p(self._grads[wname + ".bias"]),
                                           n_slabs.value, cin, cout, 0))
 
         carry = []
@@ -1170,7 +1203,7 @@
                 with torch.cuda.stream(side):
                     self._call(*args_)
             for (_x, _dy, wname), ws in zip(problems, wss):
-                jobs.append(_lib.WgradJob(_p(ws), _p(self.grads[wname + ".weight"]), _p(self.grads[wname + ".bias"]),
+                jobs.append(_lib.WgradJob(_p(ws), _p(self._grads[wname + ".weight"]), _p(self._grads[wname + ".bias"]),
                                           n_slabs.value, c, c, 0))
 
         for si in reversed(range(len(sp.stacks))):
@@ -1258,15 +1291,24 @@
                     self._call(self._bwd_data_fn(fc), _p(dc), _p(self._bwd_w(fc)),
                                None, None, _p(g), B, cin, cout, hh, ww)
         flush_carry()
+        if jobs and side is None:
+            table = (_lib.WgradJob * len(jobs))(*jobs)
+            whole = self.grad_ready_hook is None and not self.grad_is_partial
+            stats, out, acc = stat_job if stat_job is not None else (None, None, False)
+            n_part = ctypes.c_int(0)
+            self._call("ppo_grad_finish_f32", ctypes.addressof(table), len(jobs), _p(self._grad) if whole else None,
+                       self._grad.numel(), _p(self._adam_ws()), ctypes.addressof(n_part), _p(stats),
+                       stats.shape[0] if stats is not None else 0, stats.shape[1] if stats is not None else 0,
+                       stats.shape[1] if stats is not None else 0, _p(out), 1 if acc else 0)
+            self._presummed = n_part.value
+            return True
         if jobs:
             table = (_lib.WgradJob * len(jobs))(*jobs)
-            if side is None:
+            with torch.cuda.stream(side):
                 self._call("ppo_conv3x3_wgrad_reduce_f32", ctypes.addressof(table), len(jobs))
-            else:
-                with torch.cuda.stream(side):
-                    self._call("ppo_conv3x3_wgrad_reduce_f32", ctypes.addressof(table), len(jobs))
         if side is not None:
             main.wait_stream(side)
+        return False
 
     def _stack_full_bwd_ptrs(self, si, cin, cout, h, w):
         if not (FUSE_STACK_FULL_BWD and FUSE_STACK_TAIL) or self.spec.n_block != 2 or cin != cout \
@@ -1369,7 +1411,7 @@
             self.loss_tail = None
         if not fused:
             self._call("ppo_ppo_loss_f32", _p(o), B, self.nh, *loss_args)
-        self.backward(acts, dheads)
+        self.backward(acts, dheads, stat_job=None if stat_sums is None else (stats, stat_sums, stat_accumulate))
         return stats
 
     def gaussian_minibatch(self, prev_state, actions, old_log_pac, advantages, returns, eps_clip=0.2, vf_coef=0.5,
@@ -1390,8 +1432,8 @@
         self._call("ppo_gaussian_loss_f32", _p(o), B, self.nh, self.n_actions, vh, _p(actions), _p(old_log_pac),
                    _p(advantages), _p(returns), _p(self.params["log_std"]), float(eps_clip), float(vf_coef),
                    float(loss_scale) / B, _p(dheads), _p(rows), _p(stats), _p(index))
-        self._call("ppo_colsum_f32", _p(rows), B, self.n_actions, self.n_actions, _p(self.grads["log_std"]), 0)
-        self.backward(acts, dheads)
+        self._call("ppo_colsum_f32", _p(rows), B, self.n_actions, self.n_actions, _p(self._grads["log_std"]), 0)
+        self.backward(acts, dheads, stat_job=None if stat_sums is None else (stats, stat_sums, stat_accumulate))
         return stats
 
     def value_minibatch(self, prev_state, returns=None, tvf_returns=None, tvf_weights=None, vf_coef=0.5,
@@ -1414,7 +1456,7 @@
                    max(self.vh, 1), _p(tvf_returns), _p(tvf_weights), float(tvf_coef), float(loss_scale) / B, _p(dheads),
                    _p(stats), _p(index), float(tvf_keep_prob), int(dropout_seed) & (2**64 - 1),
                    int(dropout_offset) & (2**64 - 1))
-        self.backward(acts, dheads)
+        self.backward(acts, dheads, stat_job=None if stat_sums is None else (stats, stat_sums, stat_accumulate))
         return stats
 
     def distil_minibatch(self, prev_state, targets, old_policy, beta=1.0, use_tvf=False, weights=None, gaussian=False,
@@ -1433,7 +1475,7 @@
         self._call("ppo_distil_loss_f32", _p(o), B, self.nh, self.n_actions, col, n_pred, stride, 1 if use_tvf else 0,
                    _p(targets), _p(weights), _p(old_policy), _p(self.params["log_std"]) if gaussian else None,
                    float(beta), float(loss_scale) / B, _p(dheads), _p(stats), _p(index))
-        self.backward(acts, dheads)
+        self.backward(acts, dheads, stat_job=None if stat_sums is None else (stats, stat_sums, stat_accumulate))
         return stats
 
     def last_dheads(self, B):
@@ -1444,11 +1486,12 @@
         return self._buf("dheads", (B, self.nh))
 
     def zero_untouched_grads(self):
-        self.grads["log_std"].zero_()
+        self._grads["log_std"].zero_()
+        self._presummed = 0
 
     def adam_step(self, lr=2.5e-4, beta1=0.9, beta2=0.999, eps=1e-5, max_grad_norm=20.0, grad_div=1.0,
                   grad_norm_out: Optional[torch.Tensor] = None, state: Optional["AdamState"] = None):
-        ws = self._ws("adam_ws", self.lib.ppo_adam_workspace_bytes())
+        ws = self._adam_ws()
         scatter = self._scatter_table() if ADAM_SCATTER else None
         if scatter is None:
             self.mark_weights_changed()
@@ -1466,18 +1509,18 @@
             m, v, step = self.exp_avg, self.exp_avg_sq, self._adam_step
         n_part, self._presummed = self._presummed, 0
         if n_part and scatter is None and grad_div == 1.0:
-            self._call("ppo_adam_step_presummed_f32", _p(self.flat), _p(self.grad), _p(m), _p(v), self.flat.numel(), step,
+            self._call("ppo_adam_step_presummed_f32", _p(self.flat), _p(self._grad), _p(m), _p(v), self.flat.numel(), step,
                        float(lr), float(beta1), float(beta2), float(eps), float(max_grad_norm), float(grad_div), _p(ws),
                        n_part, _p(grad_norm_out))
             self.mask_feature_weights()
             return
         if scatter is not None:
-            self._call("ppo_adam_step_scatter_f32", _p(self.flat), _p(self.grad), _p(m), _p(v), self.flat.numel(), step,
+            self._call("ppo_adam_step_scatter_f32", _p(self.flat), _p(self._grad), _p(m), _p(v), self.flat.numel(), step,
                        float(lr), float(beta1), float(beta2), float(eps), float(max_grad_norm), float(grad_div), _p(ws),
                        _p(grad_norm_out), _p(scatter[0]), scatter[1], _p(self._packed))
             self.mask_feature_weights()
             return
-        self._call("ppo_adam_step_f32", _p(self.flat), _p(self.grad), _p(m), _p(v), self.flat.numel(), step, float(lr),
+        self._call("ppo_adam_step_f32", _p(self.flat), _p(self._grad), _p(m), _p(v), self.flat.numel(), step, float(lr),
                    float(beta1), float(beta2), float(eps), float(max_grad_norm), float(grad_div), _p(ws),
                    _p(grad_norm_out))
         self.mask_feature_weights()
diff --git a/ppo_amd/rollout.py b/ppo_amd/rollout.py
--- a/ppo_amd/rollout.py
+++ b/ppo_amd/rollout.py
@@ -640,6 +640,7 @@
         red = self._reducers.get(id(net))
         if red is not None:
             red.finish()
+            net.mark_grads_changed()
         net.adam_step(lr=self._lr(cfg), beta1=cfg.adam_beta1, beta2=cfg.adam_beta2, eps=cfg.adam_epsilon,
                       max_grad_norm=args.max_grad_norm if args.grad_clip_mode == "global_norm" else 0.0,
                       grad_div=float(self.world), grad_norm_out=self._grad_norm if norm_out is None else norm_out,
@@ -659,6 +660,7 @@
             self.hook = net.grad_ready_hook
             if count > 1:
                 net.grad_ready_hook = None
+                net.grad_is_partial = True
                 self.acc = net._buf("grad_accum", tuple(net.grad.shape))
 
         def after_backward(self):
@@ -672,11 +674,12 @@
         def finish(self):
             if self.count > 1:
                 self.net.grad.copy_(self.acc)
-                self.net._presummed = 0
+                self.net.mark_grads_changed()
             self.restore_hook()
 
         def restore_hook(self):
             self.net.grad_ready_hook = self.hook
+            self.net.grad_is_partial = False
 
     def _run_epochs(self, label, optimizer, epochs, mini_batch_size, step_fn, n_stats):
         B = self.N * self.A
@@ -710,12 +713,12 @@
                             acc.after_backward()
                             continue
                         if in_conv:
-                            stats = step_fn(obs_all, idx, 1.0 / n_micro, obs_indexed=True)
+                            step_fn(obs_all, idx, 1.0 / n_micro, obs_indexed=True, stat_sums=stat_rows[k],
+                                    stat_accumulate=bool(u))
                         else:
                             self._call("ppo_gather_rows", _p(obs_rows), row_bytes, B, _p(idx), micro, _p(mb_obs))
-                            stats = step_fn(mb_obs, idx, 1.0 / n_micro)
+                            step_fn(mb_obs, idx, 1.0 / n_micro, stat_sums=stat_rows[k], stat_accumulate=bool(u))
                         acc.after_backward()
-                        self._call("ppo_colsum_f32", _p(stats), micro, n_stats, n_stats, _p(stat_rows[k]), 1 if u else 0)
                     acc.finish()
                 finally:
                     acc.restore_hook()
```
